# CIawevy/FreeFine

Measured on AMD Instinct MI355X. Metric: edited images/sec/GPU @512px 50-step DDIM, higher is better.
Workload: dtype bf16x3

## Files before the change

freefine_amd/_lib.py:

```python
import ctypes as C
import os

_HERE = os.path.dirname(os.path.abspath(__file__))
LIB_PATH = os.environ.get("FREEFINE_HIP_LIB") or os.path.join(_HERE, "libfreefine_hip.so")

FFN_F32, FFN_BF16, FFN_BF16X3, FFN_FP8 = 0, 1, 2, 3
IG_OUT_SILU, IG_OUT_F32, IG_GEGLU, IG_OUT_TRANSPOSED, IG_OUT_PAIR, IG_OUT_GELU, IG_OUT_RELU, IG_OUT_KV64 = 1, 2, 4, 8, 16, 32, 64, 128
IG_OUT_QGELU = 256
ELT_RELU, ELT_ADD = 0, 1
ATT_MAXP, ATT_MAXB = 4, 16
ATT_HEAD_RULE, ATT_UNIFORM_SEL1, ATT_UNIFORM_SEL0, ATT_CAUSAL = 1, 2, 4, 8
NORM_SILU, NORM_OUT_PAIR = 1, 2


class IgemmDesc(C.Structure):
    _fields_ = [
        ("A", C.c_void_p), ("W", C.c_void_p), ("out", C.c_void_p),
        ("bias", C.c_void_p), ("rowbias", C.c_void_p), ("residual", C.c_void_p),
        ("M", C.c_int), ("N", C.c_int), ("K", C.c_int), ("Kpad", C.c_int),
        ("lda", C.c_int), ("ldo", C.c_int), ("ldr", C.c_int), ("ldrb", C.c_int),
        ("rows_per_batch", C.c_int),
        ("Hin", C.c_int), ("Win", C.c_int), ("Cin", C.c_int), ("Hout", C.c_int), ("Wout", C.c_int),
        ("stride", C.c_int), ("pad", C.c_int), ("upsample", C.c_int),
        ("flags", C.c_int), ("alpha", C.c_float), ("conv", C.c_int),
        ("splitk", C.c_int), ("ws", C.c_void_p), ("ws_bytes", C.c_long),
        ("a_lo", C.c_int), ("x3", C.c_int), ("f8", C.c_int), ("kv64_from", C.c_int),
    ]


class AttnEntry(C.Structure):
    _fields_ = [
        ("q_row", C.c_int), ("kv_row", C.c_int),
        ("w_const", C.c_float), ("w_slope", C.c_float),
        ("wq", C.c_void_p), ("kmask", C.c_void_p), ("qsel", C.c_void_p),
        ("flags", C.c_int), ("hr_row", C.c_int),
    ]


class AttnDesc(C.Structure):
    _fields_ = [
        ("q", C.c_void_p), ("k", C.c_void_p), ("vt", C.c_void_p), ("out", C.c_void_p), ("w_dev", C.c_void_p),
        ("Bo", C.c_int), ("S", C.c_int), ("Sk", C.c_int), ("heads", C.c_int), ("D", C.c_int),
        ("ldq", C.c_int), ("ldk", C.c_int), ("ldvt", C.c_int), ("ldo", C.c_int),
        ("scale", C.c_float), ("npass", C.c_int), ("out_pair", C.c_int), ("kv_pair", C.c_int),
        ("e", AttnEntry * (ATT_MAXP * ATT_MAXB)),
    ]


class CtrlStepDesc(C.Structure):
    _fields_ = [
        ("eps", C.c_void_p), ("x", C.c_void_p), ("noise", C.c_void_p), ("m", C.c_void_p), ("om", C.c_void_p),
        ("x_prev", C.c_void_p), ("pred_x0", C.c_void_p),
        ("c_bt", C.c_float), ("c_at", C.c_float), ("c_ap", C.c_float), ("c_dir", C.c_float),
        ("c_dirm", C.c_float * 8), ("stdv", C.c_float * 8), ("row_masked", C.c_int * 8),
        ("rows", C.c_int), ("CHW", C.c_int), ("HW", C.c_int),
    ]


class SplatXform(C.Structure):
    _fields_ = [("center", C.c_float * 3), ("translate", C.c_float * 3), ("rotate", C.c_float * 9), ("scale", C.c_float * 3),
                ("tan_half_fov", C.c_float)]


class PackDesc(C.Structure):
    _fields_ = [
        ("src", C.c_void_p), ("dst", C.c_void_p), ("src_row", C.c_int * 16),
        ("B", C.c_int), ("Cl", C.c_int), ("CP", C.c_int), ("HW", C.c_int),
    ]


_vp, _i, _f, _l = C.c_void_p, C.c_int, C.c_float, C.c_long
SYMBOLS = {
    "ffn_version": (_i, []),
    "ffn_last_error": (C.c_char_p, []),
    "ffn_device_info": (_i, [_i, C.c_char_p, _i]),
    "ffn_graph_launch": (_i, [_vp, _vp]),
    "ffn_igemm": (_i, [_vp, _i, C.POINTER(IgemmDesc)]),
    "ffn_conv3x3_n4": (_i, [_vp, _i, _vp, _vp, _vp, _vp, _i, _i, _i, _i]),
    "ffn_split_pair": (_i, [_vp, _vp, _vp, _l, _i, _i]),
    "ffn_groupnorm_f8": (_i, [_vp, _vp, _vp, _vp, _vp, _i, _i, _i, _i, _i, _f, _i, _f, _vp, _vp, _vp]),
    "ffn_attn": (_i, [_vp, _i, C.POINTER(AttnDesc)]),
    "ffn_attn_kernel_name": (_i, [_i, C.POINTER(AttnDesc), C.c_char_p, _i]),
    "ffn_igemm_tune": (_i, [_vp, _i, C.POINTER(IgemmDesc)]),
    "ffn_igemm_tune_entry_ints": (_i, []),
    "ffn_igemm_tune_export": (_i, [C.POINTER(C.c_int), _i]),
    "ffn_igemm_tune_import": (_i, [C.POINTER(C.c_int), _i]),
    "ffn_igemm_tune_stamp": (_i, []),
    "ffn_igemm_tune_clear": (_i, []),
    "ffn_igemm_tune_enable": (_i, [_i]),
    "ffn_igemm_num_configs": (_i, []),
    "ffn_igemm_force_config": (_i, [_i]),
    "ffn_igemm_variant": (_i, [C.POINTER(IgemmDesc), C.POINTER(C.c_int), C.POINTER(C.c_int)]),
    "ffn_igemm_kernel_name": (_i, [_i, C.POINTER(IgemmDesc), C.c_char_p, _i]),
    "ffn_attn_presplit": (_i, [_vp, _vp, _vp, _vp, _vp, _i, _i, _i, _i, _i]),
    "ffn_attn_variant": (_i, [_i, _i, C.POINTER(C.c_int), C.POINTER(C.c_int)]),
    "ffn_gn_nchunk": (_i, [_i]),
    "ffn_gn_fused": (_i, [_i, _i, _i, _i]),
    "ffn_gn_stats": (_i, [_vp, _i, _vp, _vp, _vp, _i, _i, _i, _i, _f, _vp, _vp, _vp]),
    "ffn_gn_apply": (_i, [_vp, _i, _vp, _vp, _vp, _vp, _i, _i, _i, _i]),
    "ffn_groupnorm": (_i, [_vp, _i, _vp, _vp, _vp, _vp, _i, _i, _i, _i, _f, _i, _vp, _vp, _vp]),
    "ffn_groupnorm_pair_raw": (_i, [_vp, _vp, _vp, _vp, _vp, _vp, _i, _i, _i, _i, _f, _i, _vp, _vp, _vp]),
    "ffn_layernorm": (_i, [_vp, _i, _vp, _vp, _vp, _vp, _i, _i, _f]),
    "ffn_layernorm_pair": (_i, [_vp, _vp, _vp, _vp, _vp, _i, _i, _f]),
    "ffn_softmax_rows": (_i, [_vp, _i, _vp, _vp, _l, _i, _f]),
    "ffn_cfg_masked": (_i, [_vp, _vp, _vp, _vp, _f, _vp, _l, _i]),
    "ffn_ddim_inv_step": (_i, [_vp, _vp, _vp, _f, _f, _f, _f, _vp, _vp, _l]),
    "ffn_ddim_ctrl_step": (_i, [_vp, C.POINTER(CtrlStepDesc)]),
    "ffn_pack_nchw": (_i, [_vp, _i, C.POINTER(PackDesc)]),
    "ffn_nhwc_to_nchw_f32": (_i, [_vp, _vp, _vp, _i, _i, _i, _i]),
    "ffn_concat": (_i, [_vp, _i, _vp, _vp, _vp, _l, _i, _i]),
    "ffn_timestep_embed": (_i, [_vp, _i, _vp, _vp, _vp, _i, _i, _i]),
    "ffn_transpose": (_i, [_vp, _i, _vp, _vp, _i, _i, _i, _i, _i]),
    "ffn_cast": (_i, [_vp, _i, _i, _vp, _vp, _l]),
    "ffn_eltwise": (_i, [_vp, _i, _i, _vp, _vp, _vp, _l]),
    "ffn_resize_bilinear": (_i, [_vp, _i, _vp, _vp, _i, _i, _i, _i, _i, _i, _i]),
    "ffn_splat_lift": (_i, [_vp, _vp, _vp, _vp, _i, _i, _i, _f, _f]),
    "ffn_splat_project": (_i, [_vp, _vp, _vp, _i, C.POINTER(SplatXform)]),
    "ffn_splat_bin": (_i, [_vp, _i, _vp, _i, _f, _i, _i, _vp, _vp, _vp]),
    "ffn_splat_render": (_i, [_vp, _vp, _vp, _vp, _vp, _f, _i, _i, _i, _vp, _vp, _vp]),
    "ffn_embed_tokens": (_i, [_vp, _i, _vp, _vp, _vp, _vp, _l, _i, _i, _i]),
    "ffn_image_to_nhwc": (_i, [_vp, _i, _vp, _vp, _l, _i]),
    "ffn_nhwc_to_image": (_i, [_vp, _i, _vp, _vp, _i, _i, _i]),
}

_lib = None


class FreeFineHipError(RuntimeError):
    pass


def load():
    global _lib
    if _lib is None:
        if not os.path.exists(LIB_PATH):
            raise FreeFineHipError(
                f"{LIB_PATH} not found: build it with `python -c 'import __graft_entry__ as g; g.build()'` "
                "(hipcc --offload-arch=gfx950). There is no CPU fallback for the product path.")
        import torch
        lib = C.CDLL(LIB_PATH)
        for name, (res, args) in SYMBOLS.items():
            fn = getattr(lib, name)
            fn.restype = res
            fn.argtypes = args
        _lib = lib
    return _lib


def check(rc, what=""):
    if rc != 0:
        msg = load().ffn_last_error()
        raise FreeFineHipError(f"{what} failed rc={rc}: {msg.decode() if msg else ''}")
```

freefine_amd/csrc/capi.hip:

```cpp
#include <hip/hip_runtime.h>
#include <stdarg.h>
#include <stdio.h>
#include <mutex>
#include <unordered_map>
#include <stdlib.h>
#include <string.h>

#include "../../include/freefine_hip.h"
#include "attention.h"
#include "attention_pp.h"
#include "attention_x.h"
#include "attention_x3.h"
#include "attention_x3p.h"
#include "attention_xx3.h"
#include "conv_small.h"
#include "elementwise.h"
#include "igemm.h"
#include "igemm_p8.h"
#include "norms.h"
#include "splat.h"

static thread_local char g_err[512] = "";
static int fail(int code, const char* fmt, ...) {
    va_list ap;
    va_start(ap, fmt);
    vsnprintf(g_err, sizeof(g_err), fmt, ap);
    va_end(ap);
    return code;
}
static int check_launch(const char* what) {
    hipError_t e = hipGetLastError();
    if (e != hipSuccess) return fail(FFN_EHIP, "%s: %s", what, hipGetErrorString(e));
    return FFN_OK;
}
#define LAUNCH(...)                  \
    do {                             \
        (void)hipGetLastError();     \
        hipLaunchKernelGGL(__VA_ARGS__); \
    } while (0)
#define REQUIRE(cond, ...) \
    do {                   \
        if (!(cond)) return fail(FFN_EINVAL, __VA_ARGS__); \
    } while (0)

static inline bool aligned16(const void* p) { return (reinterpret_cast<uintptr_t>(p) & 15) == 0; }
static inline int grid_for(long n, int per_block = 256, int cap = 4096) {
    long g = (n + per_block - 1) / per_block;
    if (g < 1) g = 1;
    if (g > cap) g = cap;
    return (int)g;
}

template <typename K>
static int set_lds(K kernel, int bytes) {
    static std::mutex mu;
    static std::unordered_map<const void*, int> done;
    if (bytes > 48 * 1024) {
        std::lock_guard<std::mutex> lk(mu);
        int& have = done[reinterpret_cast<const void*>(kernel)];
        if (have >= bytes) return FFN_OK;
        have = bytes;
        hipError_t e = hipFuncSetAttribute(reinterpret_cast<const void*>(kernel), hipFuncAttributeMaxDynamicSharedMemorySize, bytes);
        if (e != hipSuccess) return fail(FFN_EHIP, "hipFuncSetAttribute(%d): %s", bytes, hipGetErrorString(e));
    }
    return FFN_OK;
}

extern "C" int ffn_version(void) { return 2; }
extern "C" const char* ffn_last_error(void) { return g_err; }
extern "C" int ffn_device_info(int device, char* name, int name_len) {
    hipDeviceProp_t prop;
    hipError_t e = hipGetDeviceProperties(&prop, device);
    if (e != hipSuccess) return fail(FFN_EHIP, "hipGetDeviceProperties: %s", hipGetErrorString(e));
    if (name && name_len > 0) {
        strncpy(name, prop.gcnArchName, name_len - 1);
        name[name_len - 1] = 0;
    }
    return prop.multiProcessorCount;
}

extern "C" int ffn_graph_launch(void* stream, void* graph_exec) {
    REQUIRE(graph_exec, "graph_launch: null graph");
    hipError_t e = hipGraphLaunch(reinterpret_cast<hipGraphExec_t>(graph_exec), reinterpret_cast<hipStream_t>(stream));
    if (e != hipSuccess) return fail(FFN_EHIP, "hipGraphLaunch: %s", hipGetErrorString(e));
    return FFN_OK;
}

static void igemm_plan_for(int dtype, const ffn_igemm_desc& d, int* bm, int* bn, int* splitk);
static int igemm_stages_env() {
    static const int v = [] {
        const char* e = getenv("FFN_IGEMM_STAGES");
        return e ? atoi(e) : 0;
    }();
    return v;
}
static int device_cus() {
    static const int n = [] {
        int dev = 0, v = 0;
        if (hipGetDevice(&dev) != hipSuccess || hipDeviceGetAttribute(&v, hipDeviceAttributeMultiprocessorCount, dev) != hipSuccess || v <= 0) v = 256;
        return v;
    }();
    return n;
}
static bool persist_enabled() {
    static const bool on = [] { const char* e = getenv("FFN_IGEMM_PERSIST"); return !(e && atoi(e) == 0); }();
    return on;
}
template <typename K>
static int launch_igemm_kernel(K kern, int lds, hipStream_t s, const ffn_igemm_desc& d, int ntiles, int splitk, int threads = 256,
                               bool persist = false) {
    int rc = set_lds(kern, lds);
    if (rc) return rc;
    int gx = ntiles;
    if (persist && persist_enabled()) {
        int per_cu = (160 * 1024) / (lds > 0 ? lds : 1);
        if (per_cu > 2048 / threads) per_cu = 2048 / threads;
        if (per_cu < 1) per_cu = 1;
        const int cap = (device_cus() * per_cu) / (splitk > 0 ? splitk : 1);
        if (gx > cap && cap >= 8) gx = cap;
    }
    LAUNCH(kern, dim3(gx, splitk), dim3(threads), lds, s, d);
// ... 124 lines not shown
    if (d.x3) {
        if (d.x3 != 2 || d.K % 96 != 0 || d.a_lo != 32) return false;
    } else if (d.K % 64 != 0) return false;
    if (nkt < 2 || d.N % bn != 0 || d.M < bm) return false;
    const int osz = d.x3 ? 4 : 2;
    if (splitk > 1) {
        if (!can_split(d) || nkt % splitk != 0 || nkt / splitk < 2 || (long)splitk * d.M * d.N * 4 > d.ws_bytes || (long)splitk * d.M * d.N * 4 >= lim) return false;
    } else {
        const int act_ok = (!d.residual && !d.x3 && !d.f8 && !(d.flags & FFN_IG_GEGLU)) ? (FFN_IG_OUT_GELU | FFN_IG_OUT_RELU) : 0;
        if ((d.alpha != 1.0f && !d.f8) || (d.flags & ~(FFN_IG_GEGLU | act_ok | (d.x3 ? (FFN_IG_OUT_F32 | FFN_IG_OUT_PAIR | FFN_IG_OUT_KV64) : 0)))) return false;
        if (d.f8 && (!d.conv || (d.flags & FFN_IG_GEGLU))) return false;
        if (d.x3 && (d.flags & FFN_IG_GEGLU) && !(d.flags & FFN_IG_OUT_PAIR)) return false;
        if ((d.flags & FFN_IG_OUT_PAIR) && !(d.flags & FFN_IG_GEGLU) && (d.N % 32 != 0 || (d.ldo / 2) % 32 != 0 || (d.flags & FFN_IG_OUT_TRANSPOSED))) return false;
        if ((d.flags & FFN_IG_GEGLU) && bn != 256) return false;
        if (d.rowbias && d.rows_per_batch < 128) return false;
    }
    long a_bytes;
    if (d.conv) {
        const int pix = d.x3 ? d.lda : d.Cin;
        const int cpt = d.x3 ? d.Cin / 32 : d.Cin / 64;
        if (d.Cin % (d.x3 ? 32 : 64) != 0 || d.K != (d.conv == 2 ? 4 : 9) * (d.x3 ? 3 : 1) * d.Cin) return false;
        if (d.x3 && d.lda != 2 * d.Cin) return false;
        if (d.conv == 2 && (d.f8 || d.stride != 1 || d.upsample)) return false;
        if ((long)cpt * 9 * cpt >= 65536) return false;
        a_bytes = (long)(d.M / (d.Hout * d.Wout)) * d.Hin * d.Win * pix * 2;
        if (2 * d.Hin + 2 >= 32768 || 2 * d.Win + 2 >= 32768) return false;
        if (a_bytes + 256l * pix * 2 >= lim) return false;
    } else {
        a_bytes = (long)d.M * d.lda * 2;
        if (a_bytes + 256l * d.lda * 2 >= lim) return false;
    }
    if ((long)d.N * d.Kpad * 2 >= lim || (long)(d.M + 256) * d.ldo * ((d.flags & FFN_IG_OUT_PAIR) ? 2 : osz) >= lim) return false;
    if (d.residual && (long)(d.M + 256) * d.ldr * osz >= lim) return false;
    return true;
}
static int halo_bytes_for(const ffn_igemm_desc& d, int bm) {
    if (!d.conv || d.stride != 1 || d.upsample || d.pad != 1 || d.Hin != d.Hout || d.Win != d.Wout) return 0;
    if (d.Cin % 64 != 0 || d.Cin > 30000 || d.K != 9 * d.Cin || d.M % bm != 0) return 0;
    const int H = d.Hin, W = d.Win;
    int tw, tr;
    if (W <= bm) {
        if (bm % W != 0 || (H * W) % bm != 0) return 0;
        tw = W; tr = bm / W;
    } else {
        if (W % bm != 0) return 0;
        tw = bm; tr = 1;
    }
    const int nq = ((tr + 2) * (tw + 2) + 7) / 8;
    if (nq > 4 * 16) return 0;
    return nq * 8 * 128;
}
static bool x3_cfg(int cfg) { return cfg == CFG_64x64 || cfg == CFG_128x64 || cfg == CFG_128x128_8 || is_pp_cfg(cfg); }
template <int AMODE, bool X3 = false, bool F8 = false>
static int launch_bf16_cfg(hipStream_t s, const ffn_igemm_desc& d, IgChoice ch) {
    const IgCfgInfo& c = kCfg[ch.cfg];
    if ((X3 || F8) && !x3_cfg(ch.cfg)) return fail(FFN_EINVAL, "igemm: configuration %d is not built for split-bf16 / fp8 problems", ch.cfg);
    const int ntiles = ((d.M + c.bm - 1) / c.bm) * ((d.N + c.bn - 1) / c.bn);
    const int lds = 2 * (c.bm + c.bn) * 128, threads = 64 * c.nwm * c.nwn;
    int rc = FFN_OK;
    const bool fastk = (d.conv ? d.Cin % 64 == 0 : d.K % 64 == 0) && (long)d.K * 2 + 256 <= (long)sizeof(g_zero_page);
#define FFN_CFG_CASE(ID, BM_, BN_, WM_, WN_)                                                                                               \
    case ID:                                                                                                                        \
        if constexpr (X3) {                                                                                                         \
            if constexpr (ID == CFG_64x64 || ID == CFG_128x64 || ID == CFG_128x128_8)                                               \
                rc = launch_igemm_kernel(igemm_glds_kernel<bf16, BM_, BN_, AMODE, true, 2, WM_, WN_, false, true>, lds, s, d, ntiles, ch.splitk, threads, true); \
        } else if constexpr (F8) {                                                                                                  \
            if constexpr (AMODE == AMODE_CONV3 && (ID == CFG_64x64 || ID == CFG_128x64 || ID == CFG_128x128_8))                     \
                rc = launch_igemm_kernel(igemm_glds_kernel<bf16, BM_, BN_, AMODE, true, 2, WM_, WN_, false, false, true>, lds, s, d, ntiles, ch.splitk, threads, true); \
        } else {                                                                                                                    \
            rc = fastk ? launch_igemm_kernel(igemm_glds_kernel<bf16, BM_, BN_, AMODE, true, 2, WM_, WN_, true>, lds, s, d, ntiles, ch.splitk, threads, true)  \
                       : launch_igemm_kernel(igemm_glds_kernel<bf16, BM_, BN_, AMODE, true, 2, WM_, WN_, false>, lds, s, d, ntiles, ch.splitk, threads, true); \
        }                                                                                                                           \
        break;
    switch (ch.cfg) {
        FFN_CFG_CASE(CFG_64x64, 64, 64, 2, 2)
        FFN_CFG_CASE(CFG_128x64, 128, 64, 4, 2)
        FFN_CFG_CASE(CFG_128x128_8, 128, 128, 2, 4)
        FFN_CFG_CASE(CFG_128x128_16, 128, 128, 4, 4)
        FFN_CFG_CASE(CFG_256x128, 256, 128, 4, 4)
        FFN_CFG_CASE(CFG_256x256, 256, 256, 4, 4)
        FFN_CFG_CASE(CFG_128x320, 128, 320, 4, 4)
        FFN_CFG_CASE(CFG_128x160, 128, 160, 4, 2)
        FFN_CFG_CASE(CFG_192x320, 192, 320, 3, 4)
        case CFG_PP_256x320:
        case CFG_PP_256x256:
        case CFG_PP_192x320:
        case CFG_PP_192x256:
        case CFG_PP_256x128: {
            if (!pp_ok(d, c.bm, c.bn, ch.splitk)) return fail(FFN_EINVAL, "igemm: ping-pong kernel not applicable");
            const int pplds = 2 * (c.bm + c.bn) * 128 + 12288;
            const int nt = ((d.M + c.bm - 1) / c.bm) * (d.N / c.bn) * ch.splitk;
            const int grid = nt < device_cus() ? nt : device_cus();
            (void)hipGetLastError();
#define FFN_PP_LAUNCH(BM_, BN_, RES_, GEGLU_)                                              \
    do {                                                                                   \
        auto kern = igemm_pp_kernel<BM_, BN_, AMODE, RES_, (GEGLU_) && !F8, false, false, X3, F8>;      \
        if ((rc = set_lds(kern, pplds))) return rc;                                        \
        hipLaunchKernelGGL(kern, dim3(grid), dim3(512), pplds, s, d, 1);                   \
    } while (0)
#define FFN_PP_TILE(BM_)                                                                   \
    do {                                                                                   \
        if (c.bn == 320) {                                                                 \
            if (d.residual) FFN_PP_LAUNCH(BM_, 320, true, false);                          \
            else FFN_PP_LAUNCH(BM_, 320, false, false);                                    \
        } else {                                                                           \
            if constexpr (AMODE == AMODE_DENSE) {                                          \
                if (d.flags & FFN_IG_GEGLU) FFN_PP_LAUNCH(BM_, 256, false, true);          \
                else if (d.residual) FFN_PP_LAUNCH(BM_, 256, true, false);                 \
                else FFN_PP_LAUNCH(BM_, 256, false, false);                                \
            } else {                                                                       \
                if (d.residual) FFN_PP_LAUNCH(BM_, 256, true, false);                      \
                else FFN_PP_LAUNCH(BM_, 256, false, false);                                \
            }                                                                              \
        }                                                                                  \
    } while (0)
#define FFN_PP_SPLIT(BM_, BN_)                                                             \
    do {                                                                                   \
        auto kern = igemm_pp_kernel<BM_, BN_, AMODE, false, false, true, false, X3, F8>;   \
        if ((rc = set_lds(kern, pplds))) return rc;                                        \
        hipLaunchKernelGGL(kern, dim3(grid), dim3(512), pplds, s, d, ch.splitk);           \
    } while (0)
            if (c.bn == 128) {
                if constexpr (X3 && AMODE == AMODE_CONV3) {
                    if (d.residual) FFN_PP_LAUNCH(256, 128, true, false);
                    else FFN_PP_LAUNCH(256, 128, false, false);
                    return check_launch("igemm(ping-pong, 256 x 128)");
                } else {
                    return fail(FFN_EINVAL, "igemm: the 256 x 128 ping-pong tile is built for split-bf16 3x3 convolutions");
                }
            }
            if (ch.splitk > 1) {
                if (c.bm == 256 && c.bn == 320) FFN_PP_SPLIT(256, 320);
                else if (c.bm == 256) FFN_PP_SPLIT(256, 256);
                else if (c.bn == 320) FFN_PP_SPLIT(192, 320);
                else FFN_PP_SPLIT(192, 256);
                if ((rc = check_launch("igemm(ping-pong, split-K)"))) return rc;
                const long nq = (long)d.M * (d.N / 4);
                if constexpr (X3) LAUNCH(igemm_splitk_reduce_kernel<float>, dim3(grid_for(nq)), dim3(256), 0, s, d, ch.splitk);
                else LAUNCH(igemm_splitk_reduce_kernel<bf16>, dim3(grid_for(nq)), dim3(256), 0, s, d, ch.splitk);
                return check_launch("igemm_splitk_reduce");
            }
            if (c.bm == 256) FFN_PP_TILE(256);
            else FFN_PP_TILE(192);
#undef FFN_PP_SPLIT
#undef FFN_PP_TILE
#undef FFN_PP_LAUNCH
            return check_launch("igemm(ping-pong)");
        }
// ... 8 lines not shown
                const int nt = (d.M / c.bm) * ((d.N + c.bn - 1) / c.bn);
                (void)hipGetLastError();
                if (ch.cfg == CFG_H_128x320) {
                    auto kern = igemm_halo_kernel<bf16, 128, 320, 4, 4>;
                    if ((rc = set_lds(kern, hlds))) return rc;
                    hipLaunchKernelGGL(kern, dim3(nt), dim3(threads), hlds, s, d, hb);
                } else if (ch.cfg == CFG_H_256x128) {
                    auto kern = igemm_halo_kernel<bf16, 256, 128, 4, 4>;
                    if ((rc = set_lds(kern, hlds))) return rc;
                    hipLaunchKernelGGL(kern, dim3(nt), dim3(threads), hlds, s, d, hb);
                } else if (ch.cfg == CFG_H_256x256) {
                    auto kern = igemm_halo_kernel<bf16, 256, 256, 4, 4>;
                    if ((rc = set_lds(kern, hlds))) return rc;
                    hipLaunchKernelGGL(kern, dim3(nt), dim3(threads), hlds, s, d, hb);
                } else {
                    auto kern = igemm_halo_kernel<bf16, 128, 128, 4, 4>;
                    if ((rc = set_lds(kern, hlds))) return rc;
                    hipLaunchKernelGGL(kern, dim3(nt), dim3(threads), hlds, s, d, hb);
                }
                return check_launch("igemm(halo)");
            } else {
                return fail(FFN_EINVAL, "igemm: halo configurations are for 3x3 convolutions");
            }
        default: return fail(FFN_EINVAL, "igemm: bad configuration %d", ch.cfg);
    }
#undef FFN_CFG_CASE
    if (rc || ch.splitk == 1) return rc;
    const long nq = (long)d.M * (d.N / 4);
    if constexpr (X3) LAUNCH(igemm_splitk_reduce_kernel<float>, dim3(grid_for(nq)), dim3(256), 0, s, d, ch.splitk);
    else LAUNCH(igemm_splitk_reduce_kernel<bf16>, dim3(grid_for(nq)), dim3(256), 0, s, d, ch.splitk);
    return check_launch("igemm_splitk_reduce");
}

struct TuneKey {
    int M, N, K, conv, Cin, Hin, Win, stride, upsample, flags, lda, splitk, ptrs, wslabs, rpb, alpha1, ldo, pad, Hout, Wout, Kpad, ldr, dtype;
    bool operator==(const TuneKey& o) const { return memcmp(this, &o, sizeof(TuneKey)) == 0; }
};
struct TuneKeyHash {
    size_t operator()(const TuneKey& k) const {
        const int* p = reinterpret_cast<const int*>(&k);
        size_t h = 1469598103934665603ull;
        for (size_t i = 0; i < sizeof(TuneKey) / sizeof(int); ++i) h = (h ^ (size_t)(unsigned)p[i]) * 1099511628211ull;
        return h;
    }
};
static TuneKey tune_key(const ffn_igemm_desc& d) {
    TuneKey k;
    memset(&k, 0, sizeof(k));
    k.M = d.M; k.N = d.N; k.K = d.K; k.conv = d.conv; k.flags = d.flags; k.lda = d.lda; k.splitk = d.splitk;
    if (d.conv) { k.Cin = d.Cin; k.Hin = d.Hin; k.Win = d.Win; k.stride = d.stride; k.upsample = d.upsample; k.pad = d.pad; k.Hout = d.Hout; k.Wout = d.Wout; }
    k.Kpad = d.Kpad;
    k.ldr = d.residual ? d.ldr : 0;
    k.dtype = d.x3 ? (FFN_BF16X3 | (d.x3 << 8)) : (d.f8 ? FFN_FP8 : FFN_BF16);
    k.ptrs = (d.bias ? 1 : 0) | (d.rowbias ? 2 : 0) | (d.residual ? 4 : 0) | (d.ws && d.ws_bytes > 0 ? 8 : 0);
    const long per = (long)d.M * d.N * 4;
    k.wslabs = d.ws ? (int)(d.ws_bytes / per > 1024 ? 1024 : d.ws_bytes / per) : 0;
    k.rpb = d.rows_per_batch;
    k.alpha1 = d.alpha == 1.0f;
    k.ldo = d.ldo;
    return k;
}
static std::mutex g_tune_mu;
static std::unordered_map<TuneKey, TunedEntry, TuneKeyHash> g_tuned;
static int g_tune_runtime = 1;
static bool tune_enabled() {
    static const bool on = [] { const char* e = getenv("FFN_IGEMM_TUNE"); return !(e && atoi(e) == 0); }();
    return on && g_tune_runtime;
}
static IgChoice heuristic_choice(const ffn_igemm_desc& d) {
    if (d.conv == 2) {
        for (int bn : {320, 256})
            for (int h : {256, 192})
                if (d.N % bn == 0 && pp_ok(d, h, bn)) return IgChoice{bn == 320 ? (h == 256 ? CFG_PP_256x320 : CFG_PP_192x320) : (h == 256 ? CFG_PP_256x256 : CFG_PP_192x256), 1};
    }
    if (d.splitk <= 1) {
        for (int bn : {320, 256}) {
            if (d.N % bn != 0) continue;
            long best = -1;
            int bh = 0;
            for (int h : {256, 192}) {
                if (!pp_ok(d, h, bn)) continue;
                const long tiles = (long)((d.M + h - 1) / h) * (d.N / bn);
                if (tiles * 4 < (long)device_cus() * 3) continue;
                const long cost = ((tiles + device_cus() - 1) / device_cus()) * h;
                if (best < 0 || cost < best) { best = cost; bh = h; }
            }
            if (best >= 0) return IgChoice{bn == 320 ? (bh == 256 ? CFG_PP_256x320 : CFG_PP_192x320) : (bh == 256 ? CFG_PP_256x256 : CFG_PP_192x256), 1};
        }
        if (d.N % 128 == 0 && pp_ok(d, 256, 128) && (long)((d.M + 255) / 256) * (d.N / 128) * 4 >= (long)device_cus() * 3) return IgChoice{CFG_PP_256x128, 1};
    }
    int bm, bn, sk, ns, nw;
    igemm_plan_for(FFN_BF16, d, &bm, &bn, &sk);
    igemm_exec_cfg(FFN_BF16, d, bm, bn, sk, &ns, &nw);
    int cfg = CFG_64x64;
    if (bm == 128 && bn == 64) cfg = CFG_128x64;
    if (bm == 128 && bn == 128) cfg = (nw == 16 && !d.x3 && !d.f8) ? CFG_128x128_16 : CFG_128x128_8;
    return IgChoice{cfg, sk};
}
static int candidates_for(const ffn_igemm_desc& d, IgChoice* out, int cap) {
    int n = 0;
    const IgChoice h = heuristic_choice(d);
    out[n++] = h;
    const int nk = (d.K + 63) / 64;
    const long per = (long)d.M * d.N * 4;
    for (int cfg = 0; cfg < CFG_COUNT; ++cfg) {
        const IgCfgInfo& c = kCfg[cfg];
        if ((d.x3 || d.f8) && !x3_cfg(cfg)) continue;
// ... 151 lines not shown
}
extern "C" int ffn_igemm_tune_import(const int* buf, int n_entries) {
    REQUIRE(buf || n_entries == 0, "igemm_tune_import: null buffer");
    std::lock_guard<std::mutex> lk(g_tune_mu);
    int n = 0;
    for (int i = 0; i < n_entries; ++i) {
        const int* e = buf + (long)i * kTuneEntryInts;
        if (e[0] != kTuneStamp) continue;
        TuneKey k;
        memcpy(&k, e + 1, sizeof(TuneKey));
        const IgChoice ch{e[kTuneEntryInts - 2], e[kTuneEntryInts - 1]};
        if (ch.cfg < 0 || ch.cfg >= CFG_COUNT || ch.splitk < 1) continue;
        g_tuned[k] = TunedEntry{ch, false};
        ++n;
    }
    return n;
}
static bool tuned_lookup(const ffn_igemm_desc& d, IgChoice* ch) {
    std::lock_guard<std::mutex> lk(g_tune_mu);
    auto it = g_tuned.find(tune_key(d));
    if (it == g_tuned.end()) return false;
    *ch = it->second.ch;
    return true;
}

static bool pp_trans_tile(const ffn_igemm_desc& d, int* bm, int* bn);
static ffn_igemm_desc x3_view(const ffn_igemm_desc& d);
static ffn_igemm_desc f8_view(const ffn_igemm_desc& d);
extern "C" int ffn_igemm_kernel_name(int dtype, const ffn_igemm_desc* d0, char* buf, int len) {
    REQUIRE(d0 && buf && len > 0, "igemm_kernel_name: null argument");
    int bm, bn, sk, ns, nw;
    IgChoice ch;
    const bool x3 = dtype == FFN_BF16X3, f8 = dtype == FFN_FP8;
    const ffn_igemm_desc dd = x3 ? x3_view(*d0) : (f8 ? f8_view(*d0) : *d0);
    const ffn_igemm_desc* d = &dd;
    if (x3 && (d->flags & FFN_IG_OUT_TRANSPOSED)) {
        if (!d->conv && pp_trans_tile(*d, &bm, &bn)) {
            snprintf(buf, len, "void igemm_pp_kernel<%d, %d, 0, false, false, false, true, true, false>(ffn_igemm_desc, int)", bm, bn);
            return FFN_OK;
        }
        igemm_plan_for(FFN_BF16, *d, &bm, &bn, &sk);
        snprintf(buf, len, "void igemm_glds_kernel<bf16, %d, %d, 0, false, 2, 2, 2, false, true, false>(ffn_igemm_desc)", bm, bn);
        return FFN_OK;
    }
    if ((dtype == FFN_BF16 || x3 || f8) && !(d->flags & FFN_IG_OUT_TRANSPOSED)) {
        if (!tuned_lookup(*d, &ch)) ch = heuristic_choice(*d);
        const IgCfgInfo& c = kCfg[ch.cfg];
        if (is_halo_cfg(ch.cfg)) {
            snprintf(buf, len, "void igemm_halo_kernel<bf16, %d, %d, %d, %d>(ffn_igemm_desc, int)", c.bm, c.bn, c.nwm, c.nwn);
            return FFN_OK;
        }
        if (is_pp_cfg(ch.cfg)) {
            const bool split = ch.splitk > 1;
            snprintf(buf, len, "void igemm_pp_kernel<%d, %d, %d, %s, %s, %s, false, %s, %s>(ffn_igemm_desc, int)", c.bm, c.bn, d->conv ? 1 : 0,
                     (!split && d->residual) ? "true" : "false", (!split && (d->flags & FFN_IG_GEGLU)) ? "true" : "false", split ? "true" : "false",
                     x3 ? "true" : "false", f8 ? "true" : "false");
            return FFN_OK;
        }
        const bool fastk = !x3 && !f8 && (d->conv ? d->Cin % 64 == 0 : d->K % 64 == 0) && (long)d->K * 2 + 256 <= (long)sizeof(g_zero_page);
        snprintf(buf, len, "void igemm_glds_kernel<bf16, %d, %d, %d, true, 2, %d, %d, %s, %s, %s>(ffn_igemm_desc)", c.bm, c.bn, d->conv ? 1 : 0, c.nwm, c.nwn,
                 fastk ? "true" : "false", x3 ? "true" : "false", f8 ? "true" : "false");
        return FFN_OK;
    }
    if (dtype == FFN_BF16 && (d->flags & FFN_IG_OUT_TRANSPOSED) && !d->conv && pp_trans_tile(*d, &bm, &bn)) {
        snprintf(buf, len, "void igemm_pp_kernel<%d, %d, 0, false, false, false, true, false, false>(ffn_igemm_desc, int)", bm, bn);
        return FFN_OK;
    }
    igemm_plan_for(dtype, *d, &bm, &bn, &sk);
    igemm_exec_cfg(dtype, *d, bm, bn, sk, &ns, &nw);
    const char* t = dtype == FFN_F32 ? "float" : "bf16";
    const char* swap = (d->flags & FFN_IG_OUT_TRANSPOSED) ? "false" : "true";
    if (ns == 1) snprintf(buf, len, "void igemm_kernel<%s, %d, %d, %d, %s>(ffn_igemm_desc)", t, bm, bn, d->conv ? 1 : 0, swap);
    else {
        const int nwm = nw == 16 ? 4 : (nw == 8 ? (bn == 64 ? 4 : 2) : 2), nwn = nw / nwm;
        snprintf(buf, len, "void igemm_glds_kernel<%s, %d, %d, %d, %s, %d, %d, %d, false, false, false>(ffn_igemm_desc)", t, bm, bn, d->conv ? 1 : 0, swap, ns, nwm, nwn);
    }
    return FFN_OK;
}
static bool pp_trans_tile(const ffn_igemm_desc& d, int* bm, int* bn) {
    static const bool on = [] { const char* e = getenv("FFN_IGEMM_PP_TRANS"); return !(e && atoi(e) == 0); }();
    if (!on) return false;
    const long lim = (1l << 31) - 4096;
    *bn = d.N % 320 == 0 ? 320 : (d.N % 256 == 0 ? 256 : 0);
    if (!*bn || d.alpha != 1.0f || d.rows_per_batch % 16 != 0 || d.M % 4 != 0) return false;
    if (d.x3) {
        if (d.x3 != 2 || d.K % 96 != 0 || d.K < 192 || d.a_lo != 32) return false;
    } else if (d.K % 64 != 0 || d.K < 128) return false;
    if ((long)(d.M + 256) * d.lda * 2 >= lim || (long)d.N * d.Kpad * 2 >= lim) return false;
    if ((long)((d.M + d.rows_per_batch - 1) / d.rows_per_batch) * d.N * d.ldo * (d.x3 ? 4 : 2) >= lim) return false;
    long best = -1;
    for (int h : {256, 192}) {
        if (d.M < h) continue;
        const long tiles = (long)((d.M + h - 1) / h) * (d.N / *bn);
        const long cost = ((tiles + device_cus() - 1) / device_cus()) * h;
        if (best < 0 || cost < best) { best = cost; *bm = h; }
    }
    return best >= 0;
}
template <bool X3 = false>
static int launch_pp_trans(hipStream_t s, const ffn_igemm_desc& d, int bm, int bn) {
    const int pplds = 2 * (bm + bn) * 128 + 12288;
    const int nt = ((d.M + bm - 1) / bm) * (d.N / bn);
    const int grid = nt < device_cus() ? nt : device_cus();
    int rc = FFN_OK;
    (void)hipGetLastError();
#define FFN_PP_TR(BM_, BN_)                                                                         \
// ... 129 lines not shown
    REQUIRE(d->K % epc == 0, "igemm: K=%d must be a multiple of %d", d->K, epc);
    REQUIRE(d->rows_per_batch > 0, "igemm: rows_per_batch must be > 0");
    if (d->conv) {
        REQUIRE(d->Cin % epc == 0, "igemm: Cin=%d must be a multiple of %d", d->Cin, epc);
        if (d->conv == 2) {
            REQUIRE((dtype == FFN_BF16 || dtype == FFN_BF16X3) && d->K == 4 * d->Cin && d->stride == 1 && d->upsample == 0 && d->pad >= 0 && d->pad <= 3 && d->splitk <= 1,
                    "igemm: 2x2 convolution needs FFN_BF16 / FFN_BF16X3, K = 4*Cin, stride 1, no upsample, pad in 0..3, no forced split");
            const ffn_igemm_desc v = dtype == FFN_BF16X3 ? x3_view(*d) : *d;
            bool any = false;
            for (int bn : {320, 256})
                for (int h : {256, 192}) any |= d->N % bn == 0 && pp_ok(v, h, bn);
            REQUIRE(any, "igemm: 2x2 convolution M=%d N=%d Cin=%d fits no ping-pong tile (Cin %% 64 (split-bf16: 32), N %% 256 / 320, M >= 192)", d->M, d->N, d->Cin);
        } else {
            REQUIRE(d->conv == 1, "igemm: conv=%d", d->conv);
            REQUIRE(d->K == 9 * d->Cin, "igemm: conv K=%d != 9*Cin=%d", d->K, 9 * d->Cin);
        }
        REQUIRE(d->stride == 1 || d->stride == 2, "igemm: stride %d", d->stride);
        REQUIRE(d->upsample == 0 || d->upsample == 1, "igemm: upsample %d", d->upsample);
        REQUIRE(d->M % (d->Hout * d->Wout) == 0, "igemm: M=%d not a multiple of Hout*Wout", d->M);
    } else {
        REQUIRE(d->lda % epc == 0, "igemm: lda=%d must be a multiple of %d", d->lda, epc);
    }
    if (d->flags & FFN_IG_OUT_KV64) {
        REQUIRE(dtype == FFN_BF16X3 && !d->conv && !d->residual && !d->rowbias && d->splitk <= 1 &&
                    !(d->flags & (FFN_IG_GEGLU | FFN_IG_OUT_PAIR | FFN_IG_OUT_SILU | FFN_IG_OUT_GELU | FFN_IG_OUT_RELU | FFN_IG_OUT_QGELU)),
                "igemm: FFN_IG_OUT_KV64 needs FFN_BF16X3, dense A, the plain epilogue and no forced split-K");
        if (d->flags & FFN_IG_OUT_TRANSPOSED) REQUIRE(d->rows_per_batch % 64 == 0 && d->M % d->rows_per_batch == 0 && d->ldo >= d->rows_per_batch && d->ldo % 64 == 0,
                                                      "igemm: KV64 transposed output needs rows_per_batch %% 64 == 0, whole batches, ldo %% 64 == 0 (rows_per_batch=%d, ldo=%d)", d->rows_per_batch, d->ldo);
        else REQUIRE(d->kv64_from >= 0 && d->kv64_from < d->N && d->kv64_from % 64 == 0 && d->N % 64 == 0 && d->ldo % 4 == 0,
                     "igemm: KV64 output needs kv64_from and N %% 64 == 0 (kv64_from=%d, N=%d)", d->kv64_from, d->N);
    }
    if (d->flags & FFN_IG_OUT_TRANSPOSED) {
        REQUIRE(d->ldo % 4 == 0, "igemm: transposed ldo=%d must be a multiple of 4", d->ldo);
        REQUIRE(!(d->flags & (FFN_IG_GEGLU | FFN_IG_OUT_F32 | FFN_IG_OUT_SILU | FFN_IG_OUT_GELU | FFN_IG_OUT_RELU | FFN_IG_OUT_QGELU)) && !d->residual && !d->rowbias,
                "igemm: transposed output supports bias only");
    } else {
        REQUIRE(d->N % 4 == 0 && d->ldo % 4 == 0, "igemm: N=%d and ldo=%d must be multiples of 4", d->N, d->ldo);
        if (d->residual) REQUIRE(d->ldr % 4 == 0, "igemm: ldr=%d must be a multiple of 4", d->ldr);
        if (d->flags & FFN_IG_OUT_PAIR) {
            const int nout = (d->flags & FFN_IG_GEGLU) ? d->N / 2 : d->N;
            REQUIRE(dtype == FFN_BF16X3 && d->ldo % 16 == 0 && d->ldo / 2 >= nout, "igemm: pair output needs FFN_BF16X3, ldo %% 16 == 0, ldo/2 >= columns");
            REQUIRE(d->residual != d->out, "igemm: pair output cannot overwrite its fp32 residual");
            REQUIRE((d->ldo / 2) % 32 != 0 || nout % 32 == 0 || nout == d->ldo / 2, "igemm: blocked pair output (ldo/2 %% 32 == 0) needs whole 32-column blocks");
            REQUIRE(nout == d->ldo / 2 || (d->ldo / 2) % 32 == 0, "igemm: pair output into a wider row needs ldo/2 %% 32 == 0 (ldo=%d, columns=%d)", d->ldo, nout);
        }
        if (d->flags & FFN_IG_GEGLU) {
            REQUIRE(d->N % 64 == 0, "igemm: GEGLU needs N %% 64 == 0 (N=%d)", d->N);
            REQUIRE(!d->residual && !d->rowbias && !(d->flags & (FFN_IG_OUT_F32 | FFN_IG_OUT_SILU | FFN_IG_OUT_GELU | FFN_IG_OUT_RELU | FFN_IG_OUT_QGELU)), "igemm: GEGLU epilogue is exclusive");
        }
    }
    {
        const int act = d->flags & (FFN_IG_OUT_SILU | FFN_IG_OUT_GELU | FFN_IG_OUT_RELU | FFN_IG_OUT_QGELU);
        REQUIRE((act & (act - 1)) == 0, "igemm: SILU / GELU / QGELU / RELU are mutually exclusive");
    }
    if (d->ws) REQUIRE(aligned16(d->ws) && d->ws_bytes >= 0, "igemm: workspace must be 16-byte aligned");
    REQUIRE(d->splitk >= 0, "igemm: splitk must be >= 0");
    hipStream_t s = reinterpret_cast<hipStream_t>(stream);
    if (dtype == FFN_BF16X3) return dispatch_igemm_x3(s, x3_view(*d));
    ffn_igemm_desc plain = *d;
    plain.x3 = plain.f8 = 0;
    return dtype == FFN_F32 ? dispatch_igemm<float>(s, plain) : dispatch_igemm<bf16>(s, plain);
}

extern "C" int ffn_igemm_tune(void* stream, int dtype, const ffn_igemm_desc* d) { return ffn_igemm(stream, dtype, d); }

struct AttnTile { int dp, qf, kt, occ; };
static const AttnTile kAttnTileF32[] = {{48, 2, 64, 1}, {64, 2, 64, 1}, {80, 2, 64, 1}, {160, 1, 32, 1}};
static const AttnTile kAttnTileBf16[] = {{64, 2, 64, 2}, {96, 2, 64, 1}, {160, 1, 64, 1}};
static AttnTile attn_tile(bool f32, int D) {
    const AttnTile* t = f32 ? kAttnTileF32 : kAttnTileBf16;
    const int n = f32 ? 4 : 3;
    int i = 0;
    while (i + 1 < n && D > t[i].dp) ++i;
    return t[i];
}
extern "C" int ffn_attn_variant(int dtype, int D, int* dp, int* qf) {
    REQUIRE(dp && qf, "attn_variant: null argument");
    const AttnTile t = attn_tile(dtype == FFN_F32, D);
    *dp = t.dp;
    *qf = t.qf;
    return FFN_OK;
}
static constexpr int attn_kernel_lds(int esz, int dp, int qf, int kt) {
    return 2 * (kt * (dp * esz == 128 ? 128 : dp * esz + 16) + dp * ((dp * esz == 128 && kt * esz == 128) ? 128 : kt * esz + 16)) + 4 * (dp / 16) * qf * 64 * 16 + 2 * kt;
}
static_assert(attn_kernel_lds(4, 160, 1, 32) <= 160 * 1024 && attn_kernel_lds(2, 160, 1, 64) <= 160 * 1024, "attention tile does not fit the 160 KiB LDS");

typedef void (*attn_x3w_t)(ffn_attn_desc);
extern "C" __attribute__((visibility("hidden"))) attn_x3w_t fx3w_kernel(int masks);
extern "C" __attribute__((visibility("hidden"))) int fx3w_lds_bytes(void);
extern "C" __attribute__((visibility("hidden"))) attn_x3w_t fcausal_kernel(int dtype);
extern "C" __attribute__((visibility("hidden"))) void fembed_launch(hipStream_t s, int bf16_out, const int* ids, const float* table, const float* pos, void* out,
                                                                    long M, int S, int C, int V);

enum AttnKind { ATT_KERNEL, ATT_PP, ATT_X, ATT_X_MP, ATT_X3, ATT_X3P, ATT_X3W, ATT_XX3, ATT_CAUSAL_K };
struct AttnPlan {
    AttnKind kind;
    bool f32;
    bool masks;
    AttnTile tile;
    int nkf, nw;
    int lds;
    dim3 grid, block;
};
static int attn_plan(int dtype, const ffn_attn_desc& d, AttnPlan* p) {
    bool masks = false, uniform = false, xok = true, multi = d.npass != 1;
// ... 238 lines not shown
extern "C" int ffn_gn_fused(int B, int HW, int C, int G) {
    const long slice = (long)HW * (C / (G > 0 ? G : 1));
    if (slice > 131072) return 0;
    if (HW <= 64) return 1;
    if (HW <= 256) return B <= 32 ? 1 : 0;
    return (HW <= 1024 && (long)B * HW * C <= 3000000l) ? 1 : 0;
}
extern "C" int ffn_groupnorm(void* stream, int dtype, const void* x, void* y, const float* gamma, const float* beta, int B, int HW, int C,
                             int G, float eps, int silu, float* partial_ws, float* scale, float* shift) {
    REQUIRE(dtype == FFN_F32 || dtype == FFN_BF16, "groupnorm: bad dtype");
    REQUIRE(x && y && gamma && beta && C % G == 0 && (C / G) % 2 == 0, "groupnorm: bad arguments (C=%d, G=%d)", C, G);
    hipStream_t s = reinterpret_cast<hipStream_t>(stream);
    const long slice = (long)HW * (C / G);
    (void)slice;
    const bool fused = ffn_gn_fused(B, HW, C, G) != 0;
    const bool pair = silu & FFN_NORM_OUT_PAIR;
    REQUIRE(!pair || (dtype == FFN_F32 && C % 4 == 0), "groupnorm: pair output needs fp32 input and C %% 4 == 0");
    silu &= FFN_NORM_SILU;
    if (fused && pair) {
        dim3 grid(G, B);
        if (silu) LAUNCH((gn_fused_kernel<float, true, true>), grid, dim3(1024), 0, s, (const float*)x, (float*)y, gamma, beta, HW, C, G, eps);
        else LAUNCH((gn_fused_kernel<float, false, true>), grid, dim3(1024), 0, s, (const float*)x, (float*)y, gamma, beta, HW, C, G, eps);
        return check_launch("gn_fused(pair)");
    }
    if (fused) {
        dim3 grid(G, B);
        if (dtype == FFN_F32) {
            if (silu) LAUNCH((gn_fused_kernel<float, true>), grid, dim3(1024), 0, s, (const float*)x, (float*)y, gamma, beta, HW, C, G, eps);
            else LAUNCH((gn_fused_kernel<float, false>), grid, dim3(1024), 0, s, (const float*)x, (float*)y, gamma, beta, HW, C, G, eps);
        } else {
            if (silu) LAUNCH((gn_fused_kernel<bf16, true>), grid, dim3(1024), 0, s, (const bf16*)x, (bf16*)y, gamma, beta, HW, C, G, eps);
            else LAUNCH((gn_fused_kernel<bf16, false>), grid, dim3(1024), 0, s, (const bf16*)x, (bf16*)y, gamma, beta, HW, C, G, eps);
        }
        return check_launch("gn_fused");
    }
    REQUIRE(partial_ws && scale && shift, "groupnorm: workspace required beyond 32x32 positions");
    int rc = ffn_gn_stats(stream, dtype, x, gamma, beta, B, HW, C, G, eps, partial_ws, scale, shift);
    if (rc) return rc;
    return ffn_gn_apply(stream, dtype, x, y, scale, shift, B, HW, C, silu | (pair ? FFN_NORM_OUT_PAIR : 0));
}
extern "C" int ffn_groupnorm_pair_raw(void* stream, const void* x, void* y, void* yraw, const float* gamma, const float* beta, int B, int HW, int C, int G,
                                      float eps, int silu, float* partial_ws, float* scale, float* shift) {
    REQUIRE(x && y && yraw && gamma && beta && partial_ws && scale && shift, "groupnorm_pair_raw: null pointer (the workspace is always needed)");
    REQUIRE(C % 8 == 0 && C % G == 0 && (C / G) % 2 == 0 && aligned16(x) && aligned16(y) && aligned16(yraw), "groupnorm_pair_raw: bad arguments (C=%d, G=%d)", C, G);
    REQUIRE(y != yraw && yraw != x && y != x, "groupnorm_pair_raw: x, y and yraw must be distinct buffers");
    int rc = ffn_gn_stats(stream, FFN_F32, x, gamma, beta, B, HW, C, G, eps, partial_ws, scale, shift);
    if (rc) return rc;
    hipStream_t s = reinterpret_cast<hipStream_t>(stream);
    const long n8 = (long)B * HW * (C / 8);
    if (silu & FFN_NORM_SILU) LAUNCH((gn_apply_pair8_kernel<true, true>), dim3(grid_for(n8)), dim3(256), 0, s, (const float*)x, (bf16*)y, scale, shift, n8, HW, C, (bf16*)yraw);
    else LAUNCH((gn_apply_pair8_kernel<false, true>), dim3(grid_for(n8)), dim3(256), 0, s, (const float*)x, (bf16*)y, scale, shift, n8, HW, C, (bf16*)yraw);
    return check_launch("gn_apply(pair + raw pair)");
}
extern "C" int ffn_groupnorm_f8(void* stream, const void* x, void* y, const float* gamma, const float* beta, int B, int HW, int C, int Cp, int G,
                                float eps, int silu, float qscale, float* partial_ws, float* scale, float* shift) {
    REQUIRE(x && y && gamma && beta && partial_ws && scale && shift, "groupnorm_f8: null pointer (the workspace is always needed)");
    REQUIRE(C % 16 == 0 && C % G == 0 && Cp >= C && Cp % 16 == 0 && aligned16(x) && aligned16(y) && qscale > 0.f, "groupnorm_f8: bad arguments (C=%d, Cp=%d)", C, Cp);
    int rc = ffn_gn_stats(stream, FFN_BF16, x, gamma, beta, B, HW, C, G, eps, partial_ws, scale, shift);
    if (rc) return rc;
    hipStream_t s = reinterpret_cast<hipStream_t>(stream);
    const long nch = (long)B * HW * (Cp / 16);
    if (silu & FFN_NORM_SILU) LAUNCH(gn_apply_f8_kernel<true>, dim3(grid_for(nch)), dim3(256), 0, s, (const bf16*)x, (uint8_t*)y, scale, shift, nch, HW, C, Cp, qscale);
    else LAUNCH(gn_apply_f8_kernel<false>, dim3(grid_for(nch)), dim3(256), 0, s, (const bf16*)x, (uint8_t*)y, scale, shift, nch, HW, C, Cp, qscale);
    return check_launch("gn_apply_f8");
}
extern "C" int ffn_gn_stats(void* stream, int dtype, const void* x, const float* gamma, const float* beta, int B, int HW, int C,
                            int G, float eps, float* partial_ws, float* scale, float* shift) {
    REQUIRE(dtype == FFN_F32 || dtype == FFN_BF16, "gn_stats: bad dtype");
    const int epc = dtype == FFN_F32 ? 4 : 8;
    REQUIRE(x && gamma && beta && partial_ws && scale && shift, "gn_stats: null pointer");
    REQUIRE(C % epc == 0 && C % G == 0 && aligned16(x), "gn_stats: C=%d must be a multiple of %d and of G=%d", C, epc, G);
    hipStream_t s = reinterpret_cast<hipStream_t>(stream);
    const int nchunk = ffn_gn_nchunk(HW);
    const int ppc = (HW + nchunk - 1) / nchunk;
    const int epc_ = dtype == FFN_F32 ? 4 : 8;
    const int cols_ = C / epc_ < 256 ? C / epc_ : 256;
    const int lds = (256 / cols_ > 0 ? 256 / cols_ : 1) * cols_ * 2 * epc_ * (int)sizeof(float);
    if (dtype == FFN_F32)
        LAUNCH(gn_partial_kernel<float>, dim3(nchunk, B), dim3(256), lds, s, (const float*)x, partial_ws, HW, C, ppc);
    else
        LAUNCH(gn_partial_kernel<bf16>, dim3(nchunk, B), dim3(256), lds, s, (const bf16*)x, partial_ws, HW, C, ppc);
    if (int rc = check_launch("gn_partial")) return rc;
    LAUNCH(gn_finalize_kernel, dim3(G, B), dim3(64), 0, s, partial_ws, gamma, beta, scale, shift, HW, C, G, nchunk, eps);
    return check_launch("gn_stats");
}
extern "C" int ffn_gn_apply(void* stream, int dtype, const void* x, void* y, const float* scale, const float* shift, int B, int HW,
                            int C, int silu) {
    REQUIRE(dtype == FFN_F32 || dtype == FFN_BF16, "gn_apply: bad dtype");
    const int epc = dtype == FFN_F32 ? 4 : 8;
    REQUIRE(x && y && scale && shift && C % epc == 0 && aligned16(x) && aligned16(y), "gn_apply: bad arguments");
    hipStream_t s = reinterpret_cast<hipStream_t>(stream);
    const long nch = (long)B * HW * (C / epc);
    const int grid = grid_for(nch);
    if (silu & FFN_NORM_OUT_PAIR) {
        REQUIRE(dtype == FFN_F32, "gn_apply: pair output needs fp32 input");
        static const int wide = [] { const char* e = getenv("FFN_PAIR8"); return e ? atoi(e) : 1; }();
        if (wide && C % 8 == 0) {
            const long n8 = (long)B * HW * (C / 8);
            if (silu & FFN_NORM_SILU) LAUNCH(gn_apply_pair8_kernel<true>, dim3(grid_for(n8)), dim3(256), 0, s, (const float*)x, (bf16*)y, scale, shift, n8, HW, C);
            else LAUNCH(gn_apply_pair8_kernel<false>, dim3(grid_for(n8)), dim3(256), 0, s, (const float*)x, (bf16*)y, scale, shift, n8, HW, C);
            return check_launch("gn_apply(pair, 8 wide)");
        }
        if (silu & FFN_NORM_SILU) LAUNCH((gn_apply_kernel<float, true, true>), dim3(grid), dim3(256), 0, s, (const float*)x, (float*)y, scale, shift, nch, HW, C);
        else LAUNCH((gn_apply_kernel<float, false, true>), dim3(grid), dim3(256), 0, s, (const float*)x, (float*)y, scale, shift, nch, HW, C);
        return check_launch("gn_apply(pair)");
    }
// ... 176 lines not shown
```

freefine_amd/csrc/igemm_p8.h:

```cpp
#pragma once
#include <type_traits>
#include "igemm.h"

#ifndef PP_PRIO
#define PP_PRIO 1
#endif
#ifndef PP_ABL
#define PP_ABL 0
#endif
#ifndef PP_TAPINNER
#define PP_TAPINNER 1
#endif
#ifdef PP_STAMP
__device__ unsigned long long pp_stamp_out[8 * 64];
#define PP_STAMP_AT(k_) do { if (blockIdx.x == 7 && s >= 24 && s < 28) { const unsigned long long t_ = __builtin_amdgcn_s_memtime(); \
    if (lane == 0) *reinterpret_cast<unsigned long long*>(smem + CV + 12288 + (wave * 64 + (s - 24) * 16 + (k_)) * 8) = t_; } } while (0)
#else
#define PP_STAMP_AT(k_) do {} while (0)
#endif
#ifdef PP_NBE
#define X3_NBE(FN_, NA_) (PP_NBE)
#else
#define X3_NBE(FN_, NA_) ((FN_) + 2 - ((FN_) + (NA_) + 1) / 2)
#endif
template <int N>
__device__ __forceinline__ void pp_wait_vmcnt() {
    if (PP_ABL != 2) asm volatile("s_waitcnt vmcnt(%0)" ::"n"(N) : "memory");
}
__device__ __forceinline__ void pp_barrier() {
    asm volatile("" ::: "memory");
    __builtin_amdgcn_s_barrier();
    asm volatile("" ::: "memory");
}

#ifdef PP_TRACE
__device__ unsigned long long pp_trace[256 * 64];
#endif
template <int BM, int BN, int AMODE, bool RES, bool GEGLU, bool SPLIT = false, bool TRANS = false, bool X3 = false, bool F8 = false>
__global__ __launch_bounds__(512) void igemm_pp_kernel(const IgemmParams p, int splitk = 1) {
    typedef bf16 T;
    constexpr int HM = BM / 2;
    constexpr int FM = HM / 16;
    constexpr int FH = FM / 2;
    constexpr int NA = BM / 64;
    constexpr int FN = BN / 64;
    constexpr int WN = BN / 4;
    constexpr int ABYTES = BM * 128, BBYTES = BN * 128, BUF = ABYTES + BBYTES;
    constexpr int CV = 2 * BUF;
    constexpr int NB1 = (FN + 1) / 2;
    constexpr int NST = (SPLIT || TRANS || X3) ? FH * FN : (GEGLU ? FH * FN / 2 : FH * ((FN + 1) / 2));
    constexpr int OSZ = (X3 && !GEGLU) ? 4 : 2;
    constexpr int OOB = (int)0x80000000;
    static_assert((BM == 256 || BM == 192) && (BN == 256 || BN == 320 || (BN == 128 && BM == 256 && X3 && AMODE == AMODE_CONV3 && !GEGLU && !SPLIT && !TRANS)), "tiles built for this kernel");
    static_assert(!GEGLU || FN % 2 == 0, "GEGLU pairs hidden / gate column blocks inside a wave");

    extern __shared__ __attribute__((aligned(16))) char smem[];

    const int tid = threadIdx.x;
    const int lane = tid & 63, wave = __builtin_amdgcn_readfirstlane(tid >> 6);
    const int wr = wave >> 2, wc = wave & 3;
    const int l15 = lane & 15, g = lane >> 4;
    const int lrow = lane >> 3, csrc = (lane & 7) ^ lrow;

    static_assert(!SPLIT || (!RES && !GEGLU), "split-K slabs carry raw accumulators: the epilogue runs in the reduce kernel");
    static_assert(!TRANS || (!RES && !GEGLU && !SPLIT && AMODE == AMODE_DENSE), "transposed output: dense A, bias only");
    static_assert(!F8 || (!X3 && !TRANS && !GEGLU), "fp8 operands: plain / residual / split-K epilogues");
    const int ntn = p.N / BN;
    const int ntm = (p.M + BM - 1) / BM;
    const int nsl = SPLIT ? splitk : 1;
    const int ntiles = ntm * ntn * nsl;
    const int G = gridDim.x;
    const int nk = (X3 ? p.K / 96 : p.K / 64) / nsl;
    const int first = __builtin_amdgcn_readfirstlane(xcd_remap(blockIdx.x, G));
    const int my_tiles = (ntiles - first + G - 1) / G;
    const int S = my_tiles * nk;

    const int PIX = X3 ? p.lda * 2 : p.Cin * 2;
    const long a_bytes = AMODE == AMODE_DENSE ? (long)p.M * p.lda * 2 : (long)(p.M / (p.Hout * p.Wout)) * p.Hin * p.Win * PIX;
    const __amdgpu_buffer_rsrc_t rsrcA = __builtin_amdgcn_make_buffer_rsrc(const_cast<void*>(p.A), 0, (int)a_bytes, 0x00020000);
    const __amdgpu_buffer_rsrc_t rsrcB = __builtin_amdgcn_make_buffer_rsrc(const_cast<void*>(p.W), 0, (int)((long)p.N * p.Kpad * 2), 0x00020000);
    const __amdgpu_buffer_rsrc_t rsrcBias = __builtin_amdgcn_make_buffer_rsrc(const_cast<float*>(p.bias), 0, p.bias ? p.N * 4 : 0, 0x00020000);
    const int nbatch = (p.M + p.rows_per_batch - 1) / p.rows_per_batch;
    const __amdgpu_buffer_rsrc_t rsrcRb =
        __builtin_amdgcn_make_buffer_rsrc(const_cast<float*>(p.rowbias), 0, p.rowbias ? ((nbatch - 1) * p.ldrb + p.N) * 4 : 0, 0x00020000);
    const long o_bytes = TRANS ? (long)((p.M + p.rows_per_batch - 1) / p.rows_per_batch) * p.N * p.ldo * OSZ : (long)p.M * p.ldo * OSZ;
    const __amdgpu_buffer_rsrc_t rsrcO = __builtin_amdgcn_make_buffer_rsrc(p.out, 0, (int)o_bytes, 0x00020000);
    const __amdgpu_buffer_rsrc_t rsrcR = __builtin_amdgcn_make_buffer_rsrc(const_cast<void*>(p.residual), 0, RES ? (int)((long)p.M * p.ldr * OSZ) : 0, 0x00020000);

    int l_tile = first, l_kt = 0;
    int l_k0 = 0;
    int a_off[NA];
    int a_yx[NA];
    int b_voff;
    const int b_step = 64 * p.Kpad * 2;
    int apiece[NA];
    if constexpr (BM == 256) {
        apiece[0] = wave; apiece[1] = 16 + wave; apiece[2] = 8 + wave; apiece[3] = 24 + wave;
    } else {
        apiece[0] = wave < 6 ? wave : wave + 6;
        apiece[1] = wave < 4 ? 14 + wave : 2 + wave;
        apiece[2] = wave < 2 ? 10 + wave : 16 + wave;
    }
    const int cpt = AMODE == AMODE_DENSE ? 1 : (X3 ? p.Cin / 32 : p.Cin / 64);
    const int cpt_rcp = (65536 + cpt - 1) / cpt;
    constexpr bool TAPIN = X3 && AMODE != AMODE_DENSE && PP_TAPINNER;
    const int ntap = p.conv == 2 ? 4 : 9;
    auto kt_split = [&](int kt, int& tap, int& c) {
        if (TAPIN) {
            c = p.conv == 2 ? (kt >> 2) : ((kt * 7282) >> 16);
            tap = kt - c * ntap;
        } else {
            tap = (kt * cpt_rcp) >> 16;
            c = kt - tap * cpt;
        }
    };
    int ka = 0, tap_ky = 0, tap_kx = 0, tap_off = 0;
    auto k_position = [&]() {
        const int kt = l_k0 + l_kt;
        if (AMODE == AMODE_DENSE) {
            ka = kt * 128;
        } else {
            int tap, c;
            kt_split(kt, tap, c);
            ka = c * 128;
            tap_ky = p.conv == 2 ? (tap >> 1) : ((tap * 21846) >> 16);
            tap_kx = tap - (p.conv == 2 ? 2 : 3) * tap_ky;
            tap_off = (tap_ky * p.Win + tap_kx) * PIX;
        }
    };
    auto w_position = [&]() {
        const int kt = l_k0 + l_kt;
        if (!TAPIN) return kt * 128;
        int tap, c;
        kt_split(kt, tap, c);
        return (tap * cpt + c) * 128;
    };
    auto prep = [&](int wtile) {
        const int tile = wtile / nsl;
        l_k0 = (wtile - tile * nsl) * nk;
        const int mt = (tile / ntn) * BM, nt = (tile % ntn) * BN;
// ... 205 lines not shown
#pragma unroll
                for (int j = 0; j < FN; ++j) {
                    u32x4 w = __builtin_bit_cast(u32x4, acc[i][j]);
                    w[0] = perm(w[0]); w[1] = perm(w[1]); w[2] = perm(w[2]); w[3] = perm(w[3]);
                    __builtin_amdgcn_raw_buffer_store_b128(w, rsrcWs, vo, ((slice * p.M + m0 + i * 16) * p.N + n0 + j * 16) * 4, 0);
                }
            }
            return;
        }
        if constexpr (TRANS) {
            const int voff = (pr * p.ldo + 4 * pg) * OSZ;
#pragma unroll
            for (int i = i0; i < i0 + FH; ++i) {
                const int mb = m0 + i * 16;
                const int bb = mb / p.rows_per_batch, sb = mb - bb * p.rows_per_batch;
#pragma unroll
                for (int j = 0; j < FN; ++j) {
                    if constexpr (X3) {
                        u32x4 w4 = __builtin_bit_cast(u32x4, acc[i][j]);
                        w4[0] = perm(w4[0]); w4[1] = perm(w4[1]); w4[2] = perm(w4[2]); w4[3] = perm(w4[3]);
                        if (p.flags & FFN_IG_OUT_KV64) {
                            const float f0 = __uint_as_float(w4[0]), f1 = __uint_as_float(w4[1]), f2 = __uint_as_float(w4[2]), f3 = __uint_as_float(w4[3]);
                            u32x2 hi, lo;
                            hi[0] = pack_bf16x2(f0, f1);
                            hi[1] = pack_bf16x2(f2, f3);
                            lo[0] = pack_bf16x2(f0 - __uint_as_float(hi[0] << 16), f1 - __uint_as_float(hi[0] & 0xffff0000u));
                            lo[1] = pack_bf16x2(f2 - __uint_as_float(hi[1] << 16), f3 - __uint_as_float(hi[1] & 0xffff0000u));
                            const int vo2 = mb + 4 * pg < p.M ? (pr * p.ldo * 4 + 4 * pg * 2) : OOB;
                            const int so2 = (bb * p.N + n0 + j * 16) * p.ldo * 4 + (sb >> 6) * 256 + (sb & 63) * 2;
                            __builtin_amdgcn_raw_buffer_store_b64(hi, rsrcO, vo2, so2, 0);
                            __builtin_amdgcn_raw_buffer_store_b64(lo, rsrcO, vo2, so2 + 128, 0);
                            continue;
                        }
                        __builtin_amdgcn_raw_buffer_store_b128(w4, rsrcO, mb + 4 * pg < p.M ? voff : OOB, ((bb * p.N + n0 + j * 16) * p.ldo + sb) * 4, 0);
                        continue;
                    }
                    u32x2 w;
                    w[0] = perm(pack_bf16x2(acc[i][j][0], acc[i][j][1]));
                    w[1] = perm(pack_bf16x2(acc[i][j][2], acc[i][j][3]));
                    __builtin_amdgcn_raw_buffer_store_b64(w, rsrcO, mb + 4 * pg < p.M ? voff : OOB, ((bb * p.N + n0 + j * 16) * p.ldo + sb) * 2, 0);
                }
            }
            return;
        }
        if (PP_ABL == 4) {
#pragma unroll
            for (int i = i0; i < i0 + FH; ++i)
#pragma unroll
                for (int j = 0; j < FN; ++j) asm volatile("" ::"v"(acc[i][j]));
            return;
        }
        if constexpr (X3) {
            const int voff = (pr * p.ldo + 4 * pg) * 4;
#pragma unroll
            for (int i = i0; i < i0 + FH; ++i) {
                const int vo = m0 + i * 16 + pr < p.M ? voff : OOB;
                if constexpr (GEGLU) {
                    const int vo2 = m0 + i * 16 + pr < p.M ? (pr * p.ldo + 4 * pg) * 2 : OOB;
#pragma unroll
                    for (int j = 0; j + 1 < FN; j += 2) {
                        const f32x2_t g01 = (PP_ABL == 3 ? f32x2_t{acc[i][j + 1][0], acc[i][j + 1][1]} : gelu_erf26_2(f32x2_t{acc[i][j + 1][0], acc[i][j + 1][1]})) * f32x2_t{acc[i][j][0], acc[i][j][1]};
                        const f32x2_t g23 = (PP_ABL == 3 ? f32x2_t{acc[i][j + 1][2], acc[i][j + 1][3]} : gelu_erf26_2(f32x2_t{acc[i][j + 1][2], acc[i][j + 1][3]})) * f32x2_t{acc[i][j][2], acc[i][j][3]};
                        const float v[4] = {g01[0], g01[1], g23[0], g23[1]};
                        u32x2 hi, lo;
                        hi[0] = pack_bf16x2(v[0], v[1]);
                        hi[1] = pack_bf16x2(v[2], v[3]);
                        lo[0] = pack_bf16x2(v[0] - __uint_as_float(hi[0] << 16), v[1] - __uint_as_float(hi[0] & 0xffff0000u));
                        lo[1] = pack_bf16x2(v[2] - __uint_as_float(hi[1] << 16), v[3] - __uint_as_float(hi[1] & 0xffff0000u));
                        hi[0] = perm(hi[0]); hi[1] = perm(hi[1]); lo[0] = perm(lo[0]); lo[1] = perm(lo[1]);
                        const int so = ((m0 + i * 16) * p.ldo + n0 + (j / 2) * 16) * 2;
                        __builtin_amdgcn_raw_buffer_store_b64(hi, rsrcO, vo2, so, 0);
                        __builtin_amdgcn_raw_buffer_store_b64(lo, rsrcO, vo2, so + 64, 0);
                    }
                } else {
#pragma unroll
                    for (int j = 0; j < FN; ++j) {
                        u32x4 w = __builtin_bit_cast(u32x4, acc[i][j]);
                        w[0] = perm(w[0]); w[1] = perm(w[1]); w[2] = perm(w[2]); w[3] = perm(w[3]);
                        const int nf = n0 + j * 16;
                        if (p.flags & FFN_IG_OUT_PAIR) {
                            const float f0 = __uint_as_float(w[0]), f1 = __uint_as_float(w[1]), f2 = __uint_as_float(w[2]), f3 = __uint_as_float(w[3]);
                            u32x2 hi, lo;
                            hi[0] = pack_bf16x2(f0, f1);
                            hi[1] = pack_bf16x2(f2, f3);
                            lo[0] = pack_bf16x2(f0 - __uint_as_float(hi[0] << 16), f1 - __uint_as_float(hi[0] & 0xffff0000u));
                            lo[1] = pack_bf16x2(f2 - __uint_as_float(hi[1] << 16), f3 - __uint_as_float(hi[1] & 0xffff0000u));
                            const int vo2 = m0 + i * 16 + pr < p.M ? (pr * p.ldo + 4 * pg) * 2 : OOB;
                            const int so2 = (m0 + i * 16) * p.ldo * 2 + (nf >> 5) * 128 + (nf & 31) * 2;
                            __builtin_amdgcn_raw_buffer_store_b64(hi, rsrcO, vo2, so2, 0);
                            __builtin_amdgcn_raw_buffer_store_b64(lo, rsrcO, vo2, so2 + 64, 0);
                            continue;
                        }
                        if ((p.flags & FFN_IG_OUT_KV64) && nf >= p.kv64_from) {
                            const float f0 = __uint_as_float(w[0]), f1 = __uint_as_float(w[1]), f2 = __uint_as_float(w[2]), f3 = __uint_as_float(w[3]);
                            u32x2 hi, lo;
                            hi[0] = pack_bf16x2(f0, f1);
                            hi[1] = pack_bf16x2(f2, f3);
                            lo[0] = pack_bf16x2(f0 - __uint_as_float(hi[0] << 16), f1 - __uint_as_float(hi[0] & 0xffff0000u));
                            lo[1] = pack_bf16x2(f2 - __uint_as_float(hi[1] << 16), f3 - __uint_as_float(hi[1] & 0xffff0000u));
                            const int crel = nf - p.kv64_from;
                            const int vo2 = m0 + i * 16 + pr < p.M ? (pr * p.ldo * 4 + 4 * pg * 2) : OOB;
                            const int so2 = ((m0 + i * 16) * p.ldo + p.kv64_from) * 4 + (crel >> 6) * 256 + (crel & 63) * 2;
                            __builtin_amdgcn_raw_buffer_store_b64(hi, rsrcO, vo2, so2, 0);
                            __builtin_amdgcn_raw_buffer_store_b64(lo, rsrcO, vo2, so2 + 128, 0);
                            continue;
                        }
                        __builtin_amdgcn_raw_buffer_store_b128(w, rsrcO, vo, ((m0 + i * 16) * p.ldo + n0 + j * 16) * 4, 0);
                    }
                }
            }
            return;
        }
        if constexpr (GEGLU) {
            const int voff = (l15 * p.ldo + 4 * g) * 2;
#pragma unroll
            for (int i = i0; i < i0 + FH; ++i)
#pragma unroll
                for (int j = 0; j + 1 < FN; j += 2) {
                    const f32x2_t g01 = (PP_ABL == 3 ? f32x2_t{acc[i][j + 1][0], acc[i][j + 1][1]} : gelu_erf_fast2(f32x2_t{acc[i][j + 1][0], acc[i][j + 1][1]})) * f32x2_t{acc[i][j][0], acc[i][j][1]};
                    const f32x2_t g23 = (PP_ABL == 3 ? f32x2_t{acc[i][j + 1][2], acc[i][j + 1][3]} : gelu_erf_fast2(f32x2_t{acc[i][j + 1][2], acc[i][j + 1][3]})) * f32x2_t{acc[i][j][2], acc[i][j][3]};
                    u32x2 w;
                    w[0] = pack_bf16x2(g01[0], g01[1]);
                    w[1] = pack_bf16x2(g23[0], g23[1]);
                    __builtin_amdgcn_raw_buffer_store_b64(w, rsrcO, voff, ((m0 + i * 16) * p.ldo + n0 / 2 + (j / 2) * 16) * 2, 0);
                }
            return;
        }
        if constexpr (F8) {
#pragma unroll
            for (int i = i0; i < i0 + FH; ++i)
#pragma unroll
                for (int j = 0; j < FN; ++j) {
                    acc[i][j] *= p.alpha;
                    asm volatile("" : "+v"(acc[i][j]));
                }
            __builtin_amdgcn_sched_barrier(0);
        }
        if constexpr (!RES && !F8) {
            if (p.flags & (FFN_IG_OUT_GELU | FFN_IG_OUT_RELU)) {
                const bool gelu = p.flags & FFN_IG_OUT_GELU;
#pragma unroll
                for (int i = i0; i < i0 + FH; ++i)
#pragma unroll
                    for (int j = 0; j < FN; ++j) {
#pragma unroll
                        for (int r = 0; r < 4; ++r) acc[i][j][r] = gelu ? gelu_erf_fast(acc[i][j][r]) : fmaxf(acc[i][j][r], 0.f);
                        asm volatile("" : "+v"(acc[i][j]));
                    }
                __builtin_amdgcn_sched_barrier(0);
            }
        }
        constexpr int NOF = FN;
        const int voff8 = (pr * p.ldo + 4 * pg) * 2;
        const int voff16 = pr * p.ldo * 2 + pg * 16;
        const int paddr16 = (pr + 16 * (((pg & 1) << 1) | (pg >> 1))) * 4;
        const int ncol0 = n0;
#pragma unroll
        for (int i = i0; i < i0 + FH; ++i) {
            auto outfrag = [&](int jo, unsigned& w0, unsigned& w1) {
                w0 = pack_bf16x2(acc[i][jo][0], acc[i][jo][1]);
                w1 = pack_bf16x2(acc[i][jo][2], acc[i][jo][3]);
// ... 67 lines not shown
#pragma unroll
            for (int i = 0; i < FH; ++i)
#pragma unroll
                for (int j = 0; j < FN; ++j) mm(fb[j], fa[i], acc[i0 + i][j]);
            if constexpr (KEEPA) {
#pragma unroll
                for (int i = 0; i < FH; ++i)
#pragma unroll
                    for (int j = 0; j < FN; ++j) mm(fb[j], fal[i], acc[i0 + i][j]);
#pragma unroll
                for (int i = 0; i < FH; ++i)
#pragma unroll
                    for (int j = 0; j < FN; ++j) mm(fbl[j], fa[i], acc[i0 + i][j]);
            } else {
#pragma unroll
                for (int i = 0; i < FH; ++i) {
#pragma unroll
                    for (int j = 0; j < FN; ++j) mm(fbl[j], fa[i], acc[i0 + i][j]);
                    fa[i] = *reinterpret_cast<const u32x4*>(smem + b_ * BUF + a_rd1 + (i0 + i) * 2048);
                }
#pragma unroll
                for (int i = 0; i < FH; ++i)
#pragma unroll
                    for (int j = 0; j < FN; ++j) mm(fb[j], fa[i], acc[i0 + i][j]);
            }
            if (PP_PRIO == 1) __builtin_amdgcn_s_setprio(0);
        };
        auto read_a_set = [&](int b_, int i0) {
            read_a(b_, a_rd0, i0);
            if constexpr (KEEPA) {
#pragma unroll
                for (int i = 0; i < FH; ++i) fal[i] = *reinterpret_cast<const u32x4*>(smem + b_ * BUF + a_rd1 + (i0 + i) * 2048);
            }
        };
        auto read_low_set = [&](int b_) {
            read_a_set(b_, 0);
            read_b(b_, b_rd0);
#pragma unroll
            for (int j = 0; j < FN; ++j) fbl[j] = *reinterpret_cast<const u32x4*>(smem + b_ * BUF + b_rd1 + j * 2048);
        };
        for (int s = 0; s < S; ++s) {
            const bool more = s + 1 < S;
            const int nb = buf ^ 1;

            __builtin_amdgcn_sched_barrier(0);
            PP_STAMP_AT(0);
            if (p_tile >= 0) {
                store_rows(p_tile, I4_t{});
#pragma unroll
                for (int i = NBE; i < FN; ++i) issue_b(i, nb);
                k_position();
                issue_a(0, nb);
                issue_a(1, nb);
                pp_wait_vmcnt<FN + NAL + 2 * NST>();
                init_rows(c_tile, I0_t{});
                __builtin_amdgcn_sched_barrier(0);
                read_low_set(buf);
            } else {
                read_low_set(buf);
                PP_STAMP_AT(8);
                if (more) {
#pragma unroll
                    for (int i = NBE; i < FN; ++i) issue_b(i, nb);
                    k_position();
                    issue_a(0, nb);
                    issue_a(1, nb);
                    PP_STAMP_AT(9);
                    pp_wait_vmcnt<FN + NAL>();
                } else {
                    pp_wait_vmcnt<0>();
                }
                PP_STAMP_AT(10);
            }
            if (NBE > 0) asm volatile("s_waitcnt lgkmcnt(0)" ::: "memory");
            __builtin_amdgcn_sched_barrier(0);
            PP_STAMP_AT(1);
            pp_barrier();
            PP_STAMP_AT(2);
            mfma3(I0_t{}, buf);
            __builtin_amdgcn_sched_barrier(0);
            PP_STAMP_AT(3);
            pp_barrier();
            PP_STAMP_AT(4);

            if (more) {
#pragma unroll
                for (int i = 2; i < NA; ++i) issue_a(i, nb);
                advance();
                const bool more2 = s + 2 < S;
                if (more2) {
#pragma unroll
                    for (int i = 0; i < NBE; ++i) issue_b(i, buf);
                }
                if (more2) {
                    if (switched) pp_wait_vmcnt<NAH + NBE + (SPLIT ? 0 : 6)>();
                    else pp_wait_vmcnt<NAH + NBE>();
                } else {
                    pp_wait_vmcnt<NAH>();
                }
            }
            if (p_tile >= 0) {
                init_rows(c_tile, I4_t{});
                p_tile = -1;
            }
            if (c_kt == nk - 1) store_rows(c_tile, I0_t{});
            __builtin_amdgcn_sched_barrier(0);
            read_a_set(buf, FH);
// ... 65 lines not shown
            read_a(ra, a_rd1, 0);
            read_b(rb, b_rd1);
            if (needA) {
                k_position();
                issue_a(0, la);
                issue_a(1, la);
            }
            __builtin_amdgcn_sched_barrier(0);
            pp_barrier();
            mfma_rows(I0_t{});
            __builtin_amdgcn_sched_barrier(0);
            pp_barrier();

            read_a(ra, a_rd1, FH);
            if (more) {
                if (needA) {
#pragma unroll
                    for (int i = 2; i < NA; ++i) issue_a(i, la);
                }
                advance();
                if (PP_ABL == 9 && c_kt < 2) {}
                else if (switched) pp_wait_vmcnt<NA - 2 + (SPLIT ? 0 : 6)>();
                else pp_wait_vmcnt<NA - 2>();
            }
            if (c_kt == nk - 1) {
#ifdef PP_TRACE
                if (tid == 0) pp_trace[blockIdx.x * 64 + 2 * ((c_tile - first) / G & 31)] = __builtin_amdgcn_s_memrealtime();
#endif
                store_rows(c_tile, I0_t{});
#ifdef PP_TRACE
                if (tid == 0) pp_trace[blockIdx.x * 64 + 2 * ((c_tile - first) / G & 31) + 1] = __builtin_amdgcn_s_memrealtime();
#endif
            }
            __builtin_amdgcn_sched_barrier(0);
            pp_barrier();
            mfma_rows(I4_t{});
            __builtin_amdgcn_sched_barrier(0);
            pp_barrier();

            buf = nb;
            if (++c_kt == nk) {
                p_tile = c_tile;
                c_kt = 0;
                c_tile += G;
            }
        }
    }
    if (p_tile >= 0) store_rows(p_tile, I4_t{});
    if (wr == 0) pp_barrier();
#ifdef PP_STAMP
    if (blockIdx.x == 7) pp_stamp_out[tid] = *reinterpret_cast<const unsigned long long*>(smem + CV + 12288 + tid * 8);
#endif
}
```

freefine_amd/csrc/norms.h:

```cpp
#pragma once
#include "common.h"

__device__ __forceinline__ void store_pair4(bf16* yp, long row, int C, int c, const float* f) {
    u32x2 hi, lo;
    hi[0] = pack_bf16x2(f[0], f[1]);
    hi[1] = pack_bf16x2(f[2], f[3]);
    lo[0] = pack_bf16x2(f[0] - __uint_as_float(hi[0] << 16), f[1] - __uint_as_float(hi[0] & 0xffff0000u));
    lo[1] = pack_bf16x2(f[2] - __uint_as_float(hi[1] << 16), f[3] - __uint_as_float(hi[1] & 0xffff0000u));
    bf16* q = yp + row * 2 * C + pair_pos(c, C);
    *reinterpret_cast<u32x2*>(q) = hi;
    *reinterpret_cast<u32x2*>(q + pair_lo(C)) = lo;
}

template <typename T>
__global__ __launch_bounds__(256) void gn_partial_kernel(const T* __restrict__ x, float* __restrict__ partial, int HW,
                                                         int C, int pix_per_chunk) {
    constexpr int EPC = DT<T>::EPC;
    extern __shared__ __attribute__((aligned(16))) char smem[];
    float* ls = reinterpret_cast<float*>(smem);
    const int b = blockIdx.y, chunk = blockIdx.x, nchunk = gridDim.x;
    const int cch = C / EPC;
    const int tid = threadIdx.x;
    const int p0 = chunk * pix_per_chunk;
    const int p1 = min(HW, p0 + pix_per_chunk);
// ... 29 lines not shown
                float f[EPC];
                DT<T>::unpack(v, f);
#pragma unroll
                for (int e = 0; e < EPC; ++e) {
                    s[e] += f[e];
                    ss[e] += f[e] * f[e];
                }
            }
#pragma unroll
            for (int e = 0; e < EPC; ++e) {
                ls[(pp * cols + (cc - cbase)) * 2 * EPC + 2 * e] = s[e];
                ls[(pp * cols + (cc - cbase)) * 2 * EPC + 2 * e + 1] = ss[e];
            }
        }
        __syncthreads();
        for (int i = tid; i < cols * 2 * EPC; i += 256) {
            float acc = 0.f;
            for (int r = 0; r < ppi; ++r) acc += ls[r * cols * 2 * EPC + i];
            dst[cbase * 2 * EPC + i] = acc;
        }
        __syncthreads();
    }
}

__global__ __launch_bounds__(64) void gn_finalize_kernel(const float* __restrict__ partial, const float* __restrict__ gamma,
                                                         const float* __restrict__ beta, float* __restrict__ scale,
                                                         float* __restrict__ shift, int HW, int C, int G, int nchunk,
                                                         float eps) {
    const int g = blockIdx.x, b = blockIdx.y, lane = threadIdx.x;
    const int cg = C / G;
    double s = 0.0, ss = 0.0;
    for (int i = lane; i < nchunk * cg; i += 64) {
        const int ch = i / cg, c = g * cg + (i - ch * cg);
        const float* src = partial + (((long)b * nchunk + ch) * C + c) * 2;
        s += (double)src[0];
        ss += (double)src[1];
    }
    for (int off = 32; off > 0; off >>= 1) {
        s += __shfl_xor(s, off);
        ss += __shfl_xor(ss, off);
    }
    const double n = (double)HW * cg;
    const double mean = s / n;
    double var = ss / n - mean * mean;
    if (var < 0.0) var = 0.0;
    const float rstd = (float)(1.0 / sqrt(var + (double)eps));
    const float fmean = (float)mean;
    for (int i = lane; i < cg; i += 64) {
        const int c = g * cg + i;
        const float sc = rstd * gamma[c];
        scale[(long)b * C + c] = sc;
        shift[(long)b * C + c] = beta[c] - fmean * sc;
    }
}

template <typename T, bool SILU, bool PAIR = false>
__global__ __launch_bounds__(256) void gn_apply_kernel(const T* __restrict__ x, T* __restrict__ y,
                                                       const float* __restrict__ scale, const float* __restrict__ shift,
                                                       long nchunks_total, int HW, int C) {
    constexpr int EPC = DT<T>::EPC;
    const int cch = C / EPC;
    for (long i = (long)blockIdx.x * 256 + threadIdx.x; i < nchunks_total; i += (long)gridDim.x * 256) {
        const long pix = i / cch;
        const int cc = (int)(i - pix * cch);
        const int b = (int)(pix / HW);
        const u32x4 v = *reinterpret_cast<const u32x4*>(x + i * EPC);
        float f[EPC];
        DT<T>::unpack(v, f);
        const float* sc = scale + (long)b * C + cc * EPC;
        const float* sh = shift + (long)b * C + cc * EPC;
#pragma unroll
        for (int e = 0; e < EPC; ++e) {
            float t = f[e] * sc[e] + sh[e];
            if (SILU) t = silu_for<T>(t);
            f[e] = t;
        }
        if constexpr (PAIR) store_pair4(reinterpret_cast<bf16*>(y), pix, C, cc * EPC, f);
        else *reinterpret_cast<u32x4*>(y + i * EPC) = DT<T>::pack(f);
    }
}

template <bool SILU, bool RAW = false>
__global__ __launch_bounds__(256) void gn_apply_pair8_kernel(const float* __restrict__ x, bf16* __restrict__ y, const float* __restrict__ scale,
                                                             const float* __restrict__ shift, long n8_total, int HW, int C, bf16* __restrict__ yraw = nullptr) {
    const int cch = C / 8;
    const int lo_off = pair_lo(C);
    for (long i = (long)blockIdx.x * 256 + threadIdx.x; i < n8_total; i += (long)gridDim.x * 256) {
        const long pix = i / cch;
        const int c = (int)(i - pix * cch) * 8;
        const int b = (int)(pix / HW);
        const f32x4 v0 = *reinterpret_cast<const f32x4*>(x + pix * C + c), v1 = *reinterpret_cast<const f32x4*>(x + pix * C + c + 4);
        const f32x4 s0 = *reinterpret_cast<const f32x4*>(scale + (long)b * C + c), s1 = *reinterpret_cast<const f32x4*>(scale + (long)b * C + c + 4);
        const f32x4 h0 = *reinterpret_cast<const f32x4*>(shift + (long)b * C + c), h1 = *reinterpret_cast<const f32x4*>(shift + (long)b * C + c + 4);
        float f[8];
#pragma unroll
        for (int e = 0; e < 4; ++e) {
            f[e] = v0[e] * s0[e] + h0[e];
            f[4 + e] = v1[e] * s1[e] + h1[e];
        }
        if (SILU) {
#pragma unroll
            for (int e = 0; e < 8; ++e) f[e] = silu_fast(f[e]);
        }
        u32x4 hi, lo;
#pragma unroll
        for (int w = 0; w < 4; ++w) {
// ... 191 lines not shown
```

freefine_amd/ops.py:

```python
import ctypes as CT
import math

import os

import torch

from . import _lib as L


def _dt(t):
    if t.dtype == torch.float32:
        return L.FFN_F32
    if t.dtype == torch.bfloat16:
        return L.FFN_BF16
    raise TypeError(f"unsupported dtype {t.dtype}")


def epc(dtype):
    return 4 if dtype == torch.float32 else 8


def kstage(dtype):
    return 8 * epc(dtype)

# ... 93 lines not shown
    if x3:
        assert cp % 8 == 0, f"split-bf16 conv weights need Cin % 8 == 0 (Cin={cp})"
        hi, lo = split_hi_lo(w2.reshape(cout, 9, cp))
        if cp % 32 == 0:
            return _mark_x3(torch.stack([hi.reshape(cout, 9, cp // 32, 32), lo.reshape(cout, 9, cp // 32, 32)], dim=3).reshape(cout, 18 * cp).contiguous(), 2)
        return _mark_x3(torch.cat([hi, lo, hi], dim=2).reshape(cout, 27 * cp).contiguous(), 1)
    return pack_linear(w2.reshape(cout, 9 * cp), dtype)


def pack_conv3x3_n4(w):
    assert w.shape[0] == 4 and w.shape[2:] == (3, 3)
    return w.float().permute(0, 2, 3, 1).reshape(4, -1).contiguous()


def conv3x3_n4_eligible(cout, cin):
    return cout == 4 and cin % 16 == 0 and cin <= 448 and os.environ.get("FFN_CONV_N4", "1") != "0"


def conv3x3_n4(x, w4, bias, B, H, W, Cin):
    lib = L.load()
    assert x.is_contiguous() and x.shape[-1] == Cin and x.dtype in (torch.float32, torch.bfloat16)
    out = torch.empty(B, H * W, 4, dtype=torch.float32, device=x.device)
    L.check(_timed("conv3x3_n4_kernel", 2.0 * B * H * W * 4 * 9 * Cin, x.element_size() * x.numel() + 16.0 * B * H * W,
                   lambda: lib.ffn_conv3x3_n4(_stream(), _dt(x), x.data_ptr(), w4.data_ptr(), _p(bias), out.data_ptr(), B, H, W, Cin)), "ffn_conv3x3_n4")
    return out


def up2x_eligible(cin, cout, rows):
    return cin % 64 == 0 and (cout % 256 == 0 or cout % 320 == 0) and rows >= 192


def pack_conv3x3_up2x(w, dtype, x3=False):
    assert dtype == torch.bfloat16 or x3
    cout, cin = w.shape[:2]
    wf = w.float()
    groups = {0: ((0,), (1, 2)), 1: ((0, 1), (2,))}
    out = torch.empty(4, cout, 2, 2, cin, dtype=torch.float32, device=w.device)
    for a in (0, 1):
        for b in (0, 1):
            for dy in (0, 1):
                for dx in (0, 1):
                    acc = torch.zeros(cout, cin, dtype=torch.float32, device=w.device)
                    for ky in groups[a][dy]:
                        for kx in groups[b][dx]:
                            acc += wf[:, :, ky, kx]
                    out[2 * a + b, :, dy, dx] = acc
    if x3:
        assert cin % 32 == 0
        hi, lo = split_hi_lo(out.reshape(4 * cout, 4, cin))
        return _mark_x3(torch.stack([hi.reshape(4 * cout, 4, cin // 32, 32), lo.reshape(4 * cout, 4, cin // 32, 32)], dim=3).reshape(4 * cout, 8 * cin).contiguous(), 2)
    return pack_linear(out.reshape(4 * cout, 4 * cin), dtype)


def conv3x3_up2x(x, w4, bias, B, Hin, Win, Cin, *, out=None):
    lib = L.load()
    cout = w4.shape[0] // 4
    x3 = is_x3(w4)
    per_img = Hin * Win * max(4 * cout * (4 if x3 else 2), Cin * (4 if x3 else 2))
    nb = max(1, ((1 << 30) - 1) // per_img)
    if B > nb:
        if out is None:
            out = torch.empty(B, 4 * Hin * Win, cout, dtype=torch.float32 if x3 else x.dtype, device=x.device)
        for b0 in range(0, B, nb):
            b1 = min(B, b0 + nb)
            conv3x3_up2x(x[b0:b1], w4, bias, b1 - b0, Hin, Win, Cin, out=out[b0:b1])
        return out
    if x3:
        xa = x if pair_width(x) is not None else split_pair(x, Cin)
        assert pair_width(xa) == Cin
        odt, dcode = torch.float32, L.FFN_BF16X3
    else:
        assert x.dtype == torch.bfloat16 and x.is_contiguous()
        xa, odt, dcode = x, x.dtype, L.FFN_BF16
    assert w4.shape[1] >= (8 if x3 else 4) * Cin
    y = torch.empty(B, Hin * Win, 4 * cout, dtype=odt, device=x.device)
    for c in range(4):
        a, b = c >> 1, c & 1
        d = L.IgemmDesc()
        d.A, d.W = xa.data_ptr(), w4.data_ptr() + c * cout * w4.stride(0) * w4.element_size()
        d.bias, d.rowbias, d.residual = _p(bias), None, None
        d.M, d.N, d.K, d.Kpad = B * Hin * Win, cout, 4 * Cin, w4.stride(0)
        d.lda, d.a_lo, d.x3 = (2 * Cin, 32, 2) if x3 else (Cin, 0, 0)
        d.rows_per_batch, d.ldrb = Hin * Win, 0
        d.out, d.ldo, d.ldr = y.data_ptr() + c * cout * y.element_size(), 4 * cout, 0
        d.Hin, d.Win, d.Cin, d.Hout, d.Wout = Hin, Win, Cin, Hin, Win
        d.stride, d.pad, d.upsample = 1, 2 * (1 - a) + (1 - b), 0
        d.flags, d.alpha, d.conv = 0, 1.0, 2
        d.splitk, d.ws, d.ws_bytes = 0, _workspace(x.device).data_ptr(), WS_BYTES
        if _PROF is None:
            L.check(lib.ffn_igemm(_stream(), dcode, CT.byref(d)), "ffn_igemm(conv 2x2)")
        else:
            L.check(_timed(_igemm_name(lib, dcode, d), 2.0 * d.M * cout * 4 * Cin, y.element_size() * (x.numel() + cout * 4 * Cin + d.M * cout),
                           lambda: lib.ffn_igemm(_stream(), dcode, CT.byref(d))), "ffn_igemm(conv 2x2)")
    if out is None:
        out = torch.empty(B, 4 * Hin * Win, cout, dtype=odt, device=x.device)
    out.view(B, Hin, 2, Win, 2, cout).copy_(y.view(B, Hin, Win, 2, 2, cout).permute(0, 1, 3, 2, 4, 5))
    return out


F8_ACT_SCALE = 16.0


def pack_conv3x3_f8(w, cin_pad=None):
    cout, cin = w.shape[:2]
    cp = cin_pad or (cin + 127) // 128 * 128
    w2 = torch.zeros(cout, 3, 3, cp, dtype=torch.float32, device=w.device)
    w2[..., :cin] = w.permute(0, 2, 3, 1).float()
    amax = float(w2.abs().max())
    k = math.floor(math.log2(448.0 / amax)) if amax > 0 else 0
    ws = 2.0 ** k
    q = (w2 * ws).clamp(-448.0, 448.0).to(torch.float8_e4m3fn).reshape(cout, 9 * cp).contiguous().view(torch.uint8)
    q._ffn_f8 = (cp, 1.0 / (ws * F8_ACT_SCALE))
    return q


def is_f8(w):
    return getattr(w, "_ffn_f8", None) is not None


def groupnorm_f8(x, gamma, beta, G, eps, Cp, silu=False, ws=None):
    lib = L.load()
    B, HW, Cc = x.shape
    assert x.dtype == torch.bfloat16
    out = torch.empty(B, HW, Cp, dtype=torch.uint8, device=x.device)
    out._ffn_f8_act = Cc
    partial, scale, shift = ws if ws is not None else gn_workspace(B, HW, Cc, x.device)
    call = lambda: lib.ffn_groupnorm_f8(_stream(), x.data_ptr(), out.data_ptr(), gamma.data_ptr(), beta.data_ptr(), B, HW, Cc, Cp, G, eps,
                                        L.NORM_SILU if silu else 0, F8_ACT_SCALE, partial.data_ptr(), scale.data_ptr(), shift.data_ptr())
    L.check(_timed("gn_partial+gn_finalize+gn_apply_f8", 0.0, x.numel() * 2.0 + out.numel(), call), "ffn_groupnorm_f8")
    return out


def pack_geglu(w, b, dtype, x3=False):
    f2, k = w.shape
    f = f2 // 2
    assert f % 16 == 0
    idx = torch.arange(f, device=w.device).reshape(f // 16, 16)
    order = torch.stack([idx, idx + f], dim=1).reshape(-1)
    wp = pack_linear(w[order], dtype, x3)
    bp = None if b is None else b[order].float().contiguous()
    return wp, bp


def _mark_pair(t, C):
    t._ffn_pair = C
    return t


def pair_width(x):
    return getattr(x, "_ffn_pair", None)


def split_pair(x, K=None):
    lib = L.load()
    assert x.dtype == torch.float32 and x.stride(-1) == 1
    K = K if K is not None else x.shape[-1]
    rows = x.numel() // x.shape[-1]
    ld = x.stride(-2) if x.ndim > 1 else x.shape[-1]
    out = torch.empty(*x.shape[:-1], 2 * K, dtype=torch.bfloat16, device=x.device)
    L.check(_timed("split_pair_kernel", 0.0, 8.0 * rows * K, lambda: lib.ffn_split_pair(_stream(), x.data_ptr(), out.data_ptr(), rows, K, ld)),
            "ffn_split_pair")
    return _mark_pair(out, K)


_WS = {}
WS_BYTES = 96 << 20


def _workspace(device):
    key = (device, torch.cuda.current_stream().cuda_stream)
    ws = _WS.get(key)
    if ws is None:
        ws = _WS[key] = torch.empty(WS_BYTES // 4, dtype=torch.float32, device=device)
    return ws

def linear(x, w, bias=None, *, K=None, out=None, residual=None, rowbias=None, rows_per_batch=None, silu=False,
           geglu=False, out_f32=False, transposed_ld=None, alpha=1.0, splitk=0, out_pair=False, gelu=False, relu=False, kv64_from=None, qgelu=False):
    lib = L.load()
    K = K if K is not None else x.shape[-1]
    M = x.numel() // x.shape[-1]
    N = w.shape[0]
    d = L.IgemmDesc()
    x3 = is_x3(w)
    if x3 and pair_width(x) is not None:
        K = pair_width(x)
        M = x.numel() // x.shape[-1]
        xa = x
    else:
        xa = split_pair(x, K) if x3 else x
    dcode = L.FFN_BF16X3 if x3 else _dt(x)
    d.A, d.W = xa.data_ptr(), w.data_ptr()
    d.bias, d.rowbias, d.residual = _p(bias), _p(rowbias), _p(residual)
    d.M, d.N, d.K, d.Kpad = M, N, K, w.stride(0)
    d.lda = xa.stride(-2) if xa.ndim > 1 else xa.shape[-1]
    d.x3 = int(w._ffn_x3) if x3 else 0
    d.a_lo = (32 if d.x3 == 2 else K) if x3 else 0
    odt = torch.float32 if x3 else x.dtype
    d.rows_per_batch = rows_per_batch or M
    d.ldrb = rowbias.stride(0) if rowbias is not None else 0
    flags = 0
    n_out = N
    if silu:
        flags |= L.IG_OUT_SILU
    if gelu:
        flags |= L.IG_OUT_GELU
    if relu:
        flags |= L.IG_OUT_RELU
    if qgelu:
        flags |= L.IG_OUT_QGELU
    if geglu:
        flags |= L.IG_GEGLU
        n_out = N // 2
    if out_f32:
        flags |= L.IG_OUT_F32
    if transposed_ld is not None:
        flags |= L.IG_OUT_TRANSPOSED
        nb = M // d.rows_per_batch
        if out is None:
            alloc = torch.zeros if transposed_ld > d.rows_per_batch else torch.empty
            out = alloc(nb, N, transposed_ld, dtype=odt, device=x.device)
        d.ldo = transposed_ld
    elif out_pair:
        assert x3 and out is None
        flags |= L.IG_OUT_PAIR
        out = _mark_pair(torch.empty(*x.shape[:-1], 2 * n_out, dtype=torch.bfloat16, device=x.device), n_out)
        d.ldo = 2 * n_out
    else:
        if out is None:
            out = torch.empty(*x.shape[:-1], n_out, dtype=torch.float32 if out_f32 else odt, device=x.device)
        d.ldo = out.stride(-2) if out.ndim > 1 else n_out
    d.ldr = residual.shape[-1] if residual is not None else 0
    d.out = out.data_ptr()
    if kv64_from is not None:
        assert x3 and residual is None and rowbias is None and not (silu or gelu or relu or qgelu or geglu or out_pair)
        flags |= L.IG_OUT_KV64
        d.kv64_from = int(kv64_from)
        splitk = 1
    d.flags, d.alpha, d.conv = flags, alpha, 0
    d.splitk, d.ws, d.ws_bytes = splitk, _workspace(x.device).data_ptr(), WS_BYTES
    if _PROF is None:
        L.check(lib.ffn_igemm(_stream(), dcode, CT.byref(d)), "ffn_igemm")
    else:
        esz = x.element_size()
        L.check(_timed(_igemm_name(lib, dcode, d), 2.0 * M * N * K, esz * (M * K + N * K + M * n_out),
                       lambda: lib.ffn_igemm(_stream(), dcode, CT.byref(d))), "ffn_igemm")
    return out


def conv3x3(x, w, bias, B, Hin, Win, Cin, *, stride=1, pad=1, upsample=False, out=None, residual=None, rowbias=None,
            rowbias_ld=None, out_f32=False, Hout=None, Wout=None, splitk=0, relu=False):
    lib = L.load()
    He, We = (Hin * 2, Win * 2) if upsample else (Hin, Win)
    if Hout is None:
        Hout = (He + 2 * pad - 3) // stride + 1
        Wout = (We + 2 * pad - 3) // stride + 1
    N = w.shape[0]
    d = L.IgemmDesc()
    x3 = is_x3(w)
    f8 = is_f8(w)
    if f8:
        assert x.dtype == torch.uint8 and x.shape[-1] == w._ffn_f8[0] and out_f32 is False
        Cin = x.shape[-1]
        xa = x
    elif x3 and pair_width(x) is not None:
        assert pair_width(x) == Cin
        xa = x
    else:
        xa = split_pair(x, Cin) if x3 else x
    dcode = L.FFN_FP8 if f8 else (L.FFN_BF16X3 if x3 else _dt(x))
    odt = torch.float32 if x3 else (torch.bfloat16 if f8 else x.dtype)
    d.A, d.W = xa.data_ptr(), w.data_ptr()
    d.bias, d.rowbias, d.residual = _p(bias), _p(rowbias), _p(residual)
    d.M, d.N, d.K, d.Kpad = B * Hout * Wout, N, 9 * Cin, w.shape[1]
    d.lda = 2 * Cin if x3 else Cin
    d.x3 = int(w._ffn_x3) if x3 else 0
    d.a_lo = (32 if d.x3 == 2 else Cin) if x3 else 0
    d.rows_per_batch = Hout * Wout
    d.ldrb = (rowbias_ld or rowbias.stride(0)) if rowbias is not None else 0
    if out is None:
        out = torch.empty(B, Hout * Wout, N, dtype=torch.float32 if out_f32 else odt, device=x.device)
    d.out, d.ldo = out.data_ptr(), out.stride(-2)
    d.ldr = residual.shape[-1] if residual is not None else 0
    d.Hin, d.Win, d.Cin, d.Hout, d.Wout = Hin, Win, Cin, Hout, Wout
    d.stride, d.pad, d.upsample = stride, pad, 1 if upsample else 0
    d.flags, d.alpha, d.conv = (L.IG_OUT_F32 if out_f32 else 0) | (L.IG_OUT_RELU if relu else 0), (w._ffn_f8[1] if f8 else 1.0), 1
    d.splitk, d.ws, d.ws_bytes = splitk, _workspace(x.device).data_ptr(), WS_BYTES
    if _PROF is None:
        L.check(lib.ffn_igemm(_stream(), dcode, CT.byref(d)), "ffn_igemm(conv)")
    else:
        esz = x.element_size()
        k_real = 9 * getattr(x, "_ffn_f8_act", Cin)
        L.check(_timed(_igemm_name(lib, dcode, d), 2.0 * d.M * N * k_real, esz * (x.numel() + N * d.K + d.M * N),
                       lambda: lib.ffn_igemm(_stream(), dcode, CT.byref(d))), "ffn_igemm(conv)")
    return out


class AttnEntrySpec:
    __slots__ = ("q_row", "kv_row", "w_const", "w_slope", "wq", "kmask", "qsel", "flags", "hr_row")

    def __init__(self, q_row, kv_row, w_const=1.0, w_slope=0.0, wq=None, kmask=None, qsel=None, flags=0, hr_row=None):
        self.q_row, self.kv_row, self.w_const, self.w_slope = q_row, kv_row, w_const, w_slope
        self.wq, self.kmask, self.qsel, self.flags, self.hr_row = wq, kmask, qsel, flags, hr_row

    def remap(self, row_map, logical_row):
        return AttnEntrySpec(row_map[self.q_row], row_map[self.kv_row], self.w_const, self.w_slope, self.wq, self.kmask, self.qsel,
                             self.flags, logical_row if self.hr_row is None else self.hr_row)

    def pinned(self, logical_row):
        return self if self.hr_row is not None else AttnEntrySpec(self.q_row, self.kv_row, self.w_const, self.w_slope, self.wq, self.kmask, self.qsel,
                                                                  self.flags, logical_row)

    def renumber(self, ren, kv_ren=None):
        kv_ren = ren if kv_ren is None else kv_ren
        if self.q_row not in ren or self.kv_row not in kv_ren:
            raise ValueError(f"attention term (q row {self.q_row}, kv row {self.kv_row}) reaches outside the rows of this phase {sorted(ren)} / {sorted(kv_ren)}")
        return AttnEntrySpec(ren[self.q_row], kv_ren[self.kv_row], self.w_const, self.w_slope, self.wq, self.kmask, self.qsel, self.flags, self.hr_row)

    def shifted(self, base, logical_row, kv_base=None):
        return AttnEntrySpec(self.q_row + base, self.kv_row + (base if kv_base is None else kv_base), self.w_const, self.w_slope, self.wq,
                             self.kmask, self.qsel, self.flags, logical_row if self.hr_row is None else self.hr_row)


def _set_entries(d, passes, b0, nb, ptr=_p):
    for p, rows in enumerate(passes):
        for b in range(nb):
            sp = rows[b0 + b]
            e = d.e[p * L.ATT_MAXB + b]
            if sp is None:
                e.w_const = e.w_slope = 0.0
                continue
            e.q_row, e.kv_row, e.w_const, e.w_slope = sp.q_row, sp.kv_row, sp.w_const, sp.w_slope
            e.wq, e.kmask, e.qsel, e.flags = ptr(sp.wq), ptr(sp.kmask), ptr(sp.qsel), sp.flags
            hr = sp.hr_row if sp.hr_row is not None else (b0 + b if b0 else None)
            e.hr_row = 0 if hr is None else hr + 1


def _takes_kv_images(lib, d):
    probe = L.AttnDesc.from_buffer_copy(d)
    probe.kv_pair = 1
# ... 57 lines not shown
    descs = []
    chunk = L.ATT_MAXB
    if _ROWSPLIT and Bo > 1 and Dh == 64 and S >= 128 and Sk % 64 == 0 and q.is_cuda:
        di = q.device.index if q.device.index is not None else torch.cuda.current_device()
        if di not in _CUS:
            _CUS[di] = torch.cuda.get_device_properties(di).multi_processor_count
        chunk = attn_row_split(Bo, heads * -(-S // 256), L.ATT_MAXB, _CUS[di])
    for b0 in range(0, Bo, chunk):
        nb = min(chunk, Bo - b0)
        d = L.AttnDesc()
        d.q, d.k, d.vt, d.w_dev = q.data_ptr(), k.data_ptr(), vt.data_ptr(), _p(w_dev)
        d.out = out.data_ptr() + b0 * S * Cq * esz
        d.Bo, d.S, d.Sk, d.heads, d.D = nb, S, Sk, heads, Dh
        d.ldq, d.ldk, d.ldvt, d.ldo = q.stride(1), k.stride(1), vt.stride(1), (2 * Cq if out_pair else Cq)
        d.out_pair = 1 if out_pair else 0
        d.scale, d.npass = scale, len(passes)
        d.kv_pair = 1 if kv_images else 0
        _set_entries(d, passes, b0, nb)
        descs.append((b0, nb, d))
    if kv_images:
        assert dcode == L.FFN_BF16X3 and kv_images_ok(Dh, S, Sk)
    elif dcode == L.FFN_BF16X3 and _ATTN_PRESPLIT and k.stride(2) == 1 and vt.stride(2) == 1 and k.stride(0) == Sk * k.stride(1) \
            and vt.stride(0) == heads * Dh * vt.stride(1) and k.shape[0] * Sk * heads * Dh * 4 < 2 ** 31 - 65536:
        if all(_takes_kv_images(lib, d) for _, _, d in descs):
            Bk = k.shape[0]
            kp = torch.empty(Bk, Sk, 2 * heads * Dh, dtype=torch.bfloat16, device=q.device)
            vp = torch.empty(Bk, heads * Dh, 2 * Sk, dtype=torch.bfloat16, device=q.device)
            L.check(_timed("attn_presplit_kernel", 0.0, 16.0 * Bk * Sk * heads * Dh,
                           lambda: lib.ffn_attn_presplit(_stream(), k.data_ptr(), vt.data_ptr(), kp.data_ptr(), vp.data_ptr(), Bk, Sk, heads, k.stride(1), vt.stride(1))),
                    "ffn_attn_presplit")
            for _, _, d in descs:
                d.k, d.vt, d.kv_pair = kp.data_ptr(), vp.data_ptr(), 1
                d.ldk, d.ldvt = heads * Dh, Sk
    for b0, nb, d in descs:
        if _PROF is None:
            L.check(lib.ffn_attn(_stream(), dcode, CT.byref(d)), "ffn_attn")
        else:
            nterms = sum(1 for rows in passes for sp in rows[b0:b0 + nb] if sp is not None and (sp.w_const != 0.0 or sp.w_slope != 0.0))
            nbuf = CT.create_string_buffer(160)
            lib.ffn_attn_kernel_name(dcode, CT.byref(d), nbuf, 160)
            L.check(_timed(nbuf.value.decode(), 4.0 * nterms * S * Sk * Cq,
                           esz * nterms * (S * Cq + 2 * Sk * Cq) + esz * nb * S * Cq,
                           lambda: lib.ffn_attn(_stream(), dcode, CT.byref(d))), "ffn_attn")
    return out


def gn_workspace(B, HW, C, device):
    lib = L.load()
    nchunk = lib.ffn_gn_nchunk(HW)
    return (torch.empty(B * nchunk * 2 * C, dtype=torch.float32, device=device),
            torch.empty(B, C, dtype=torch.float32, device=device), torch.empty(B, C, dtype=torch.float32, device=device))


def groupnorm(x, gamma, beta, G, eps, silu=False, out=None, ws=None, pair=False):
    lib = L.load()
    B, HW, Cc = x.shape
    if pair:
        assert x.dtype == torch.float32 and out is None
        out = _mark_pair(torch.empty(B, HW, 2 * Cc, dtype=torch.bfloat16, device=x.device), Cc)
    if out is None:
        out = torch.empty_like(x)
    if lib.ffn_gn_fused(B, HW, Cc, G):
        partial = scale = shift = None
    else:
        partial, scale, shift = ws if ws is not None else gn_workspace(B, HW, Cc, x.device)
    fl = (L.NORM_SILU if silu else 0) | (L.NORM_OUT_PAIR if pair else 0)
    nb = B
    if partial is not None and _GN_CHUNK_MB > 0 and x.is_contiguous() and out.is_contiguous():
        row_bytes = HW * Cc * x.element_size()
        nb = max(1, min(B, int(_GN_CHUNK_MB * 2 ** 20) // row_bytes))
        nb = -(-B // -(-B // nb))
    def call():
        rc = 0
        for b0 in range(0, B, nb):
            n = min(nb, B - b0)
            rc = lib.ffn_groupnorm(_stream(), _dt(x), x.data_ptr() + b0 * HW * Cc * x.element_size(), out.data_ptr() + b0 * HW * out.shape[-1] * out.element_size(),
                                   gamma.data_ptr(), beta.data_ptr(), n, HW, Cc, G, eps, fl, _p(partial), _p(scale), _p(shift))
            if rc:
                break
        return rc
    if _PROF is None:
        L.check(call(), "ffn_groupnorm")
    else:
        name = f"gn_fused_kernel<{_tname(x)}>" if partial is None else f"gn_partial+gn_finalize+gn_apply<{_tname(x)}>"
        L.check(_timed(name, 0.0, 2.0 * x.numel() * x.element_size(), call), "ffn_groupnorm")
    return out


def groupnorm_pair_raw(x, gamma, beta, G, eps, silu=False, ws=None):
    lib = L.load()
    B, HW, Cc = x.shape
    if not _GN_RAW or Cc % 8 != 0 or lib.ffn_gn_fused(B, HW, Cc, G) or not x.is_contiguous():
        return groupnorm(x, gamma, beta, G, eps, silu=silu, pair=True, ws=ws), split_pair(x, Cc)
    assert x.dtype == torch.float32
    y = _mark_pair(torch.empty(B, HW, 2 * Cc, dtype=torch.bfloat16, device=x.device), Cc)
    yr = _mark_pair(torch.empty(B, HW, 2 * Cc, dtype=torch.bfloat16, device=x.device), Cc)
    partial, scale, shift = ws if ws is not None else gn_workspace(B, HW, Cc, x.device)
    call = lambda: lib.ffn_groupnorm_pair_raw(_stream(), x.data_ptr(), y.data_ptr(), yr.data_ptr(), gamma.data_ptr(), beta.data_ptr(), B, HW, Cc, G, eps,
                                              L.NORM_SILU if silu else 0, _p(partial), _p(scale), _p(shift))
    if _PROF is None:
        L.check(call(), "ffn_groupnorm_pair_raw")
    else:
        L.check(_timed("gn_partial+gn_finalize+gn_apply<float> (+ raw pair)", 0.0, 3.0 * x.numel() * x.element_size(), call), "ffn_groupnorm_pair_raw")
    return y, yr


def layernorm(x, gamma, beta, eps=1e-5, out=None, pair=False):
    lib = L.load()
    Cc = x.shape[-1]
    M = x.numel() // Cc
    if pair:
        assert x.dtype == torch.float32 and out is None
        out = _mark_pair(torch.empty(*x.shape[:-1], 2 * Cc, dtype=torch.bfloat16, device=x.device), Cc)
        call = lambda: lib.ffn_layernorm_pair(_stream(), x.data_ptr(), out.data_ptr(), gamma.data_ptr(), beta.data_ptr(), M, Cc, eps)
    else:
        if out is None:
            out = torch.empty_like(x)
        call = lambda: lib.ffn_layernorm(_stream(), _dt(x), x.data_ptr(), out.data_ptr(), gamma.data_ptr(), beta.data_ptr(), M, Cc, eps)
    if _PROF is None:
        L.check(call(), "ffn_layernorm")
    else:
        L.check(_timed(f"layernorm_kernel<{_tname(x)}>", 0.0, 2.0 * x.numel() * x.element_size(), call), "ffn_layernorm")
    return out


def softmax_rows(x, scale=1.0, out=None):
    lib = L.load()
    N = x.shape[-1]
    M = x.numel() // N
    if out is None:
        out = torch.empty_like(x)
    L.check(_timed(f"softmax_rows_kernel<{_tname(x)}>", 0.0, 2.0 * x.numel() * x.element_size(),
                   lambda: lib.ffn_softmax_rows(_stream(), _dt(x), x.data_ptr(), out.data_ptr(), M, N, scale)), "ffn_softmax_rows")
    return out


def cfg_masked(eps_u, eps_c, mask_f, cfg, out=None):
    lib = L.load()
    if out is None:
        out = torch.empty_like(eps_u)
    HW = eps_u.shape[-1] * eps_u.shape[-2]
    L.check(_timed("cfg_masked_kernel", 0.0, 12.0 * eps_u.numel(),
                   lambda: lib.ffn_cfg_masked(_stream(), eps_u.data_ptr(), eps_c.data_ptr(), _p(mask_f), float(cfg), out.data_ptr(),
                                              eps_u.numel(), HW)), "ffn_cfg_masked")
    return out


def ddim_inv_step(eps, x, c_bt, c_at, c_an, c_bn, want_pred_x0=False):
    lib = L.load()
# ... 4 lines not shown
                                                 x.numel())), "ffn_ddim_inv_step")
    return x_next, p0


def ddim_ctrl_step(eps, x, noise, m_f, om_f, c_bt, c_at, c_ap, c_dir, c_dirm, stdv, row_masked, want_pred_x0=False):
    lib = L.load()
    rows = x.shape[0]
    d = L.CtrlStepDesc()
    x_prev = torch.empty_like(x)
    p0 = torch.empty_like(x) if want_pred_x0 else None
    d.eps, d.x, d.noise, d.m, d.om = eps.data_ptr(), x.data_ptr(), _p(noise), m_f.data_ptr(), om_f.data_ptr()
    d.x_prev, d.pred_x0 = x_prev.data_ptr(), _p(p0)
    d.c_bt, d.c_at, d.c_ap, d.c_dir = c_bt, c_at, c_ap, c_dir
    for b in range(rows):
        d.c_dirm[b], d.stdv[b], d.row_masked[b] = c_dirm[b], stdv[b], int(row_masked[b])
    d.rows, d.CHW, d.HW = rows, x[0].numel(), x.shape[-1] * x.shape[-2]
    L.check(_timed("ddim_ctrl_step_kernel", 0.0, 20.0 * x.numel(), lambda: lib.ffn_ddim_ctrl_step(_stream(), CT.byref(d))), "ffn_ddim_ctrl_step")
    return x_prev, p0


def pack_nchw(src, src_rows, CP, dtype, out=None):
    lib = L.load()
    Bs, Cl, H, W = src.shape
    B = len(src_rows)
    if out is None:
        out = torch.empty(B, H * W, CP, dtype=dtype, device=src.device)
    for b0 in range(0, B, 16):
        nb = min(16, B - b0)
        d = L.PackDesc()
        d.src, d.dst = src.data_ptr(), out.data_ptr() + b0 * H * W * CP * out.element_size()
        for i in range(nb):
            d.src_row[i] = src_rows[b0 + i]
        d.B, d.Cl, d.CP, d.HW = nb, Cl, CP, H * W
        L.check(_timed(f"pack_nchw_kernel<{_tname(out)}>", 0.0, nb * H * W * (4.0 * Cl + CP * out.element_size()),
                       lambda: lib.ffn_pack_nchw(_stream(), _dt(out), CT.byref(d))), "ffn_pack_nchw")
    return out


def nhwc_to_nchw_f32(src, C_, H, W, out=None):
    lib = L.load()
    B, HW, ld = src.shape
    if out is None:
        out = torch.empty(B, C_, H, W, dtype=torch.float32, device=src.device)
    L.check(_timed("nhwc_to_nchw_f32_kernel", 0.0, 8.0 * B * HW * C_,
                   lambda: lib.ffn_nhwc_to_nchw_f32(_stream(), src.data_ptr(), out.data_ptr(), B, HW, C_, ld)), "ffn_nhwc_to_nchw_f32")
    return out


def concat(a, b, out=None):
    lib = L.load()
    C1, C2 = a.shape[-1], b.shape[-1]
    rows = a.numel() // C1
    base = getattr(a, "_ffn_cat_base", None)
    if out is None and base is not None and base.shape[-1] == C1 + C2:
        L.check(_timed(f"concat_kernel<{_tname(b)}>", 0.0, 2.0 * rows * C2 * b.element_size(),
                       lambda: lib.ffn_concat(_stream(), _dt(b), None, b.data_ptr(), base.data_ptr(), rows, C1, C2)), "ffn_concat")
        return base
    if base is not None:
        a = a.contiguous()
    if out is None:
        out = torch.empty(*a.shape[:-1], C1 + C2, dtype=a.dtype, device=a.device)
    L.check(_timed(f"concat_kernel<{_tname(a)}>", 0.0, 2.0 * rows * (C1 + C2) * a.element_size(),
                   lambda: lib.ffn_concat(_stream(), _dt(a), a.data_ptr(), b.data_ptr(), out.data_ptr(), rows, C1, C2)), "ffn_concat")
    return out


def cat_dst(shape_lead, C1, C2, dtype, device):
    base = torch.empty(*shape_lead, C1 + C2, dtype=dtype, device=device)
    view = base[..., :C1]
    view._ffn_cat_base = base
    return view


def timestep_freqs(dim, device, max_period=10000.0, shift=0.0):
    half = dim // 2
    exponent = -math.log(max_period) * torch.arange(half, dtype=torch.float32) / (half - shift)
    return torch.exp(exponent).to(device)


def timestep_embed(t_dev, freq, B, dtype, flip=True, out=None):
    lib = L.load()
    half = freq.numel()
    if out is None:
        out = torch.empty(B, 2 * half, dtype=dtype, device=freq.device)
    L.check(_timed(f"timestep_embed_kernel<{_tname(out)}>", 0.0, float(out.numel() * out.element_size()),
                   lambda: lib.ffn_timestep_embed(_stream(), _dt(out), t_dev.data_ptr(), freq.data_ptr(), out.data_ptr(), B, half,
                                                  1 if flip else 0)), "ffn_timestep_embed")
    return out


def transpose(src, ld_dst=None, out=None):
    lib = L.load()
    B, R, Cc = src.shape
    ld_dst = ld_dst or R
    if out is None:
        out = torch.zeros(B, Cc, ld_dst, dtype=src.dtype, device=src.device)
    L.check(_timed(f"transpose_kernel<{_tname(src)}>", 0.0, 2.0 * src.numel() * src.element_size(),
                   lambda: lib.ffn_transpose(_stream(), _dt(src), src.data_ptr(), out.data_ptr(), B, R, Cc, Cc, ld_dst)), "ffn_transpose")
    return out


def cast(src, dtype, out=None):
    lib = L.load()
    if out is None:
        out = torch.empty(src.shape, dtype=dtype, device=src.device)
    L.check(_timed(f"cast_kernel<{_tname(src)}, {_tname(out)}>", 0.0, float(src.numel() * (src.element_size() + out.element_size())),
                   lambda: lib.ffn_cast(_stream(), _dt(src), _dt(out), src.data_ptr(), out.data_ptr(), src.numel())), "ffn_cast")
    return out


def relu(x, out=None):
    lib = L.load()
    out = torch.empty_like(x) if out is None else out
    L.check(_timed("eltwise_kernel<relu>", 0.0, 2.0 * x.numel() * x.element_size(),
                   lambda: lib.ffn_eltwise(_stream(), _dt(x), L.ELT_RELU, x.data_ptr(), None, out.data_ptr(), x.numel())), "ffn_eltwise")
    return out

# ... 96 lines not shown
```

freefine_amd/unet.py:

```python
import ctypes as CT
import os
import weakref

import torch

from . import _lib as L
from . import ops
from .config import UNetConfig

_GRAPH_RAW = os.environ.get("FFN_GRAPH_RAW", "1") != "0"


class _Res:
    pass


class HipUNet:
    def __init__(self, cfg: UNetConfig, state, dtype=torch.bfloat16, device="cuda:0", x3=False, fp8_conv=False):
        assert not x3 or dtype == torch.float32, "split-bf16 mode keeps fp32 activations"
        assert not fp8_conv or dtype == torch.bfloat16, "fp8 convolutions are an option of the bf16 fast mode"
        self.x3 = bool(x3)
        self.fp8_conv = bool(fp8_conv)
        self.cfg, self.dtype, self.device = cfg, dtype, torch.device(device)
        self.in_channels = cfg.in_channels
# ... 423 lines not shown
            if plan["passes"] is None:
                fps.append(0)
                continue
            rows = tuple(tuple(None if e is None else (e.q_row, e.kv_row, e.w_const, e.w_slope, e.flags, e.hr_row,
                                                       0 if e.wq is None else e.wq.data_ptr(),
                                                       0 if e.kmask is None else e.kmask.data_ptr(),
                                                       0 if e.qsel is None else e.qsel.data_ptr()) for e in r) for r in plan["passes"])
            fps.append((plan["kind"], plan["needs_cg"], rows))
        self._in_phase_a = self._kv_ext = False
        return (self.hook, tuple(fps))

    def join_block_tb(self, join):
        tb = len([t for blk in self.down if blk.attn for t in blk.attn]) + 1
        for blk in self.up[:join]:
            tb += len(blk.attn) if blk.attn else 0
        return tb

    def _capture(self, sample, text_kv, sig):
        ctrls = self._ctrls()
        state = [(c.cur_att_layer, c.cur_step) for c in ctrls]
        x_static = sample.clone()
        ru = self._reuse
        ref_in = None
        if ru is not None and ru["mode"] == "replay":
            ref_in = [t.clone() for t in ru["state"]]
            ru["state_run"] = ref_in
        if ru is not None and ru["mode"] == "replay_kv":
            ref_in = ru["static"] = []
            ru["static_bufs"] = []
        self._run(x_static, text_kv)
        if ru is not None and ru["mode"] == "replay_kv":
            ru["static_ready"] = True
        for c, st in zip(ctrls, state):
            c.cur_att_layer, c.cur_step = st
        torch.cuda.synchronize()
        graph = torch.cuda.CUDAGraph()
        if self._capture_stream is None:
            self._capture_stream = torch.cuda.Stream(device=x_static.device)
        with torch.cuda.graph(graph, stream=self._capture_stream):
            out = self._run(x_static, text_kv)
        rec = ru is not None and ru["mode"] == "record"
        g = dict(graph=graph, x=x_static, out=out, ref_in=ref_in, ref_bufs=ru.get("static_bufs") if ru is not None else None,
                 boundary=self.last_boundary if rec else None, kv=self.last_kv if rec else None, device=x_static.device.index)
        if ru is not None:
            for k in ("state_run", "static", "static_bufs", "static_ready"):
                ru.pop(k, None)
        self._graphs[sig] = g
        return g

    def _gn(self, x, gb, eps, silu):
        B, HW, C = x.shape
        return ops.groupnorm(x, gb[0], gb[1], self.cfg.norm_num_groups, eps, silu=silu, pair=self.x3)

    def _gn_conv_in(self, x, gb, w):
        if ops.is_f8(w):
            return ops.groupnorm_f8(x, gb[0], gb[1], self.cfg.norm_num_groups, self.cfg.norm_eps, w._ffn_f8[0], silu=True)
        return self._gn(x, gb, self.cfg.norm_eps, True)

    def _resblock(self, r, x, B, H, W, temb_all, out=None):
        cin = x.shape[-1]
        if r.sc is not None and self.x3 and not ops.is_f8(r.c1[0]) and ops.pair_width(x) is None and x.dtype == torch.float32:
            h, x = ops.groupnorm_pair_raw(x, r.n1[0], r.n1[1], self.cfg.norm_num_groups, self.cfg.norm_eps, silu=True)
        else:
            h = self._gn_conv_in(x, r.n1, r.c1[0])
        rb = temb_all[:, r.temb_off:r.temb_off + r.cout]
        h = ops.conv3x3(h, r.c1[0], r.c1[1], B, H, W, cin, rowbias=rb, rowbias_ld=temb_all.shape[1])
        h = self._gn_conv_in(h, r.n2, r.c2[0])
        if r.sc is not None:
            x = ops.linear(x, r.sc[0], r.sc[1], K=cin)
        return ops.conv3x3(h, r.c2[0], r.c2[1], B, H, W, r.cout, residual=x, out=out)

    def _without_ref_queries(self, plan, B):
        keep = self._reuse["idx_a_list"]
        passes = plan["passes"] if plan["passes"] is not None else [[ops.AttnEntrySpec(b, b) for b in range(B)]]
        pin = lambda e, r: e if (e is None or e.hr_row is not None) else ops.AttnEntrySpec(e.q_row, e.kv_row, e.w_const, e.w_slope, e.wq, e.kmask, e.qsel, e.flags, r)
        out = dict(plan)
        out["passes"] = [[pin(rows[r], r) for r in keep] for rows in passes]
        return out

    def _self_plan(self, t, place, B, S, drop_ref_queries=False):
        if self.controller is None:
            return dict(kind="plain", needs_cg=False, passes=[[ops.AttnEntrySpec(r, r, hr_row=r) for r in self._reuse["idx_a_list"]]]) if drop_ref_queries else None
        plan = self._plan(False, place, B, S, t.heads)
        if drop_ref_queries:
            assert plan["kind"] != "shared_kv"
            plan = self._without_ref_queries(plan, B)
        return plan

    def _attention(self, t, is_cross, place, q, k, vt, ldq_view, B, S, Sk, plan=None, kv_images=False):
        D = t.C // t.heads
        scale = D ** -0.5
        if is_cross and self.controller is not None:
            plan = self._plan(is_cross, place, B, S, t.heads)
        if plan is None:
            return ops.attention(q, k, vt, t.heads, scale, None, Sk=Sk, C=t.C, x3=self.x3, out_pair=self.x3, kv_images=kv_images)
        if plan["kind"] == "shared_kv":
            assert not kv_images
            rr = plan["ref_rows"]
            kc = k[..., :t.C] if k.shape[-1] != t.C else k
            k2 = torch.cat([kc, kc[rr]], dim=1).contiguous()
            vt2 = torch.cat([vt[..., :Sk], vt[rr][..., :Sk]], dim=2).contiguous()
            return ops.attention(q, k2, vt2, t.heads, scale, plan["passes"], Sk=2 * Sk, C=t.C, x3=self.x3, out_pair=self.x3)
        return ops.attention(q, k, vt, t.heads, scale, plan["passes"], Sk=Sk, C=t.C, w_dev=self.cg_dev if plan["needs_cg"] else None, x3=self.x3,
                             out_pair=self.x3, kv_images=kv_images)

    def _kv_buffers(self, B, S, C, ldv):
        ru = self._reuse
        i = ru["cursor"]
        ru["cursor"] = i + 1
        if ru.get("static_ready"):
            return ru["static_bufs"][i]
        k_ref, vt_ref = ru["state"][2 * i], ru["state"][2 * i + 1]
        nr = k_ref.shape[0]
        assert tuple(k_ref.shape) == (nr, S, C) and tuple(vt_ref.shape) == (nr, C, ldv), (tuple(k_ref.shape), tuple(vt_ref.shape), (S, C, ldv))
        qk = torch.empty(B + nr, S, 2 * C, dtype=self.dtype, device=self.device)
        vt = torch.empty(B + nr, C, ldv, dtype=self.dtype, device=self.device)
        qk[B:, :, C:].copy_(k_ref)
        vt[B:].copy_(vt_ref)
        if ru.get("static") is not None:
            ru["static_bufs"].append((qk, vt))
            ru["static"] += [qk[B:, :, C:], vt[B:]]
        return qk, vt

    def _transformer_block(self, t, x, B, H, W, place, kv_text, out=None, drop=None, tb=0):
        S, C = H * W, t.C
        res0 = x
        ru = self._reuse
        h = self._gn(x, t.norm, 1e-6, False)
        h = ops.linear(h, t.proj_in[0], t.proj_in[1], K=C)
        y = ops.layernorm(h, *t.ln[0], pair=self.x3)
        ldv = (S + 7) // 8 * 8
        if ru is not None and ru["mode"] == "replay_kv" and tb >= ru["kv_from"]:
            qk, vt = self._kv_buffers(B, S, C, ldv)
            ops.linear(y, t.w_qk1, None, K=C, out=qk[:B])
            ops.linear(y, t.w_v1, None, K=C, rows_per_batch=S, transposed_ld=ldv, out=vt[:B])
            self._kv_ext = True
            a = self._attention(t, False, place, qk[:B], qk[..., C:], vt, 2 * C, B, S, S, plan=self._self_plan(t, place, B, S))
            self._kv_ext = False
        else:
            plan = self._self_plan(t, place, B, S, drop_ref_queries=drop is not None)
            rec = ru is not None and ru["mode"] == "record" and ru.get("kv_from") is not None and tb >= ru["kv_from"]
            img = self.x3 and not rec and (plan is None or plan["kind"] != "shared_kv") and \
                ops.kv_images_ok(C // t.heads, S, S, None if plan is None else plan["passes"], B * max(S * 2 * C, C * ldv) * 4)
            qk = ops.linear(y, t.w_qk1, None, K=C, kv64_from=C if img else None)
            vt = ops.linear(y, t.w_v1, None, K=C, rows_per_batch=S, transposed_ld=ldv, kv64_from=0 if img else None)
            if rec:
                self.last_kv.append((qk[..., C:], vt))
            a = self._attention(t, False, place, qk, qk[..., C:], vt, 2 * C, B, S, S, plan=plan, kv_images=img)
        if drop is not None:
            idx, kv_text = drop
            h, res0, B = h.index_select(0, idx), res0.index_select(0, idx), idx.shape[0]
            self._in_phase_a = True
        h = ops.linear(a, t.o1[0], t.o1[1], K=C, residual=h)
        y = ops.layernorm(h, *t.ln[1], pair=self.x3)
        q = ops.linear(y, t.w_q2, None, K=C)
        k2, vt2 = kv_text
        a = self._attention(t, True, place, q, k2, vt2, C, B, S, k2.shape[1])
        h = ops.linear(a, t.o2[0], t.o2[1], K=C, residual=h)
        y = ops.layernorm(h, *t.ln[2], pair=self.x3)
        y = ops.linear(y, t.ff1[0], t.ff1[1], K=C, geglu=True, out_pair=self.x3)
        h = ops.linear(y, t.ff2[0], t.ff2[1], K=4 * C, residual=h, out_pair=self.x3 and C % 32 == 0)
        return ops.linear(h, t.proj_out[0], t.proj_out[1], K=C, residual=res0, out=out)

    def _run(self, sample, text_kv):
        cfg = self.cfg
        B, _, H, W = sample.shape
        dt = self.dtype
        ru = self._reuse
        replay = ru is not None and ru["mode"] == "replay"
        record = ru is not None and ru["mode"] == "record"
        replay_kv = ru is not None and ru["mode"] == "replay_kv"
        BB = B
        if replay:
            sample = sample.index_select(0, ru["idx_a"])
            B = sample.shape[0]
            text_kv = list(ru["text_kv_a"][:self.join_block_tb(ru["join"])]) + list(text_kv[self.join_block_tb(ru["join"]):])
        if replay_kv:
            sample = sample.index_select(0, ru["idx_a"])
            B = sample.shape[0]
            text_kv = ru["text_kv_a"]
            ru["cursor"] = 0
        if record and ru.get("kv_from") is not None:
            self.last_kv = []
        self._in_phase_a = replay
        ti = iter(text_kv)
        tb = 0
        te = ops.timestep_embed(self.t_dev, self.freq, BB, dt, flip=cfg.flip_sin_to_cos)
        e1 = ops.linear(te, self.te1[0], self.te1[1], K=self.te1[2], silu=True)
        e2 = ops.linear(e1, self.te2[0], self.te2[1], K=self.te2[2], silu=True)
        temb_all = ops.linear(e2, self.temb_w, self.temb_b, K=self.te2[0].shape[0], out_f32=True)
        temb_full = temb_all
        temb_all = temb_all[:B]
        x = ops.pack_nchw(sample, list(range(B)), self.cin_pad, dt)
        x = ops.conv3x3(x, self.conv_in[0], self.conv_in[1], B, H, W, self.cin_pad)
        skips = [(x, H, W)]
        n = len(self.down)
        for i, blk in enumerate(self.down):
            for j, r in enumerate(blk.res):
                x = self._resblock(r, x, B, H, W, temb_all)
                if blk.attn:
                    x = self._transformer_block(blk.attn[j], x, B, H, W, "down", next(ti), tb=tb)
                    tb += 1
                skips.append((x, H, W))
            if blk.down is not None:
                C = x.shape[-1]
                x = ops.conv3x3(x, blk.down[0], blk.down[1], B, H, W, C, stride=2)
                H, W = (H + 1) // 2, (W + 1) // 2
                skips.append((x, H, W))
        x = self._resblock(self.mid.res[0], x, B, H, W, temb_all)
        x = self._transformer_block(self.mid.attn[0], x, B, H, W, "mid", next(ti), tb=tb)
        tb += 1
        def cat_dst(C1, HW):
            return ops.cat_dst((B, HW), C1, skips[-1][0].shape[-1], dt, x.device) if skips else None
        x = self._resblock(self.mid.res[1], x, B, H, W, temb_all, out=cat_dst(self.mid.res[1].cout, H * W))
        for i, blk in enumerate(self.up):
            if ru is not None and ru.get("join") is not None and i == ru["join"]:
                if record:
                    self.last_boundary = [x] + [s for s, _, _ in reversed(skips)]
                if replay:
                    state = ru.get("state_run") or ru["state"]
                    assert len(state) == 1 + len(skips), (len(state), len(skips))
                    merge = lambda a, r: torch.cat([a, r.to(a.dtype)], 0).index_select(0, ru["perm"])
                    x = merge(x, state[0])
                    skips = [(merge(s, st), sh, sw) for (s, sh, sw), st in zip(skips, reversed(state[1:]))]
                    B, temb_all = BB, temb_full
                    self._in_phase_a = False
            for j, r in enumerate(blk.res):
                s, sh, sw = skips.pop()
                assert (sh, sw) == (H, W)
                x = ops.concat(x, s)
                dst = cat_dst(r.cout, H * W) if j + 1 < len(blk.res) else None
                x = self._resblock(r, x, B, H, W, temb_all, out=None if blk.attn else dst)
                if blk.attn:
                    last = replay and bool(ru.get("drop_tail")) and blk.attn[j] is self.transformers[-1]
                    drop = (ru["idx_a"], ru["text_kv_a"][-1]) if last else None
                    x = self._transformer_block(blk.attn[j], x, B, H, W, "up", next(ti), out=dst, drop=drop, tb=tb)
                    tb += 1
                    if last:
                        assert dst is None and i == len(self.up) - 1 and j == len(blk.res) - 1, "the last transformer block closes the network"
                        B, temb_all = x.shape[0], temb_full[:x.shape[0]]
            if blk.up is not None:
                C = x.shape[-1]
                if blk.up2 is not None and ops.up2x_eligible(C, C, B * H * W):
                    x = ops.conv3x3_up2x(x, blk.up2, blk.up[1], B, H, W, C, out=cat_dst(C, 4 * H * W))
                else:
                    x = ops.conv3x3(x, blk.up[0], blk.up[1], B, H, W, C, upsample=True, out=cat_dst(C, 4 * H * W))
                H, W = 2 * H, 2 * W
        C = x.shape[-1]
        if self.conv_out_n4 is not None:
            x = ops.groupnorm(x, self.norm_out[0], self.norm_out[1], cfg.norm_num_groups, cfg.norm_eps, silu=True)
            eps = ops.conv3x3_n4(x, self.conv_out_n4, self.conv_out[1], B, H, W, C)
        else:
            x = self._gn(x, self.norm_out, cfg.norm_eps, True)
            eps = ops.conv3x3(x, self.conv_out[0], self.conv_out[1], B, H, W, C, out_f32=True)
        eps = ops.nhwc_to_nchw_f32(eps, cfg.out_channels, H, W)
        self._in_phase_a = False
        if B != BB:
            eps = torch.zeros(BB, *eps.shape[1:], dtype=eps.dtype, device=eps.device).index_copy_(0, ru["idx_a"], eps)
        return eps
```

freefine_amd/vae.py:

```python
import os

import torch

from . import ops
from .config import VAEConfig


class _O:
    pass


class HipVAE:
    def __init__(self, cfg: VAEConfig, state, dtype=torch.bfloat16, device="cuda:0", x3=False):
        assert not x3 or dtype == torch.float32
        self.x3 = bool(x3)
        self.cfg, self.dtype, self.device = cfg, dtype, torch.device(device)
        self.G = cfg.norm_num_groups
        self._pack(state)

    def _f32(self, t):
        return t.detach().float().contiguous().to(self.device)

    def _conv(self, st, name, cin_pad=None, cout_pad=None):
        w, b = st[name + ".weight"].float().to(self.device), st[name + ".bias"].float().to(self.device)
# ... 24 lines not shown
        a.q, a.k, a.v, a.o = (self._lin(st, f"{p}.{n}") for n in ("to_q", "to_k", "to_v", "to_out.0"))
        return a

    def _mid(self, st, p):
        m = _O()
        m.r0, m.attn, m.r1 = self._res(st, p + ".resnets.0"), self._attn(st, p + ".attentions.0"), self._res(st, p + ".resnets.1")
        return m

    def _pack(self, st):
        cfg = self.cfg
        e = 8 if self.x3 else ops.epc(self.dtype)
        s = cfg.scaling_factor
        n = len(cfg.block_out_channels)
        self.img_cp = (cfg.in_channels + e - 1) // e * e
        self.enc_in = self._conv(st, "encoder.conv_in", self.img_cp)
        self.enc_down = []
        for i in range(n):
            b = _O()
            b.res = [self._res(st, f"encoder.down_blocks.{i}.resnets.{j}") for j in range(cfg.layers_per_block)]
            b.down = self._conv(st, f"encoder.down_blocks.{i}.downsamplers.0.conv") if i < n - 1 else None
            self.enc_down.append(b)
        self.enc_mid = self._mid(st, "encoder.mid_block")
        self.enc_norm = (self._f32(st["encoder.conv_norm_out.weight"]), self._f32(st["encoder.conv_norm_out.bias"]))
        self.enc_out = self._conv(st, "encoder.conv_out")
        lc = cfg.latent_channels
        self.lat_cp = (2 * lc + e - 1) // e * e
        qw, qb = st["quant_conv.weight"].float().reshape(2 * lc, 2 * lc), st["quant_conv.bias"].float()
        self.quant = (ops.pack_linear((qw[:lc] * s).to(self.device), self.dtype, self.x3), (qb[:lc] * s).to(self.device).contiguous(), 2 * lc)
        self.zin_cp = (lc + e - 1) // e * e
        pw = torch.zeros(self.zin_cp, self.zin_cp)
        pw[:lc, :lc] = st["post_quant_conv.weight"].float().reshape(lc, lc) / s
        pb = torch.zeros(self.zin_cp)
        pb[:lc] = st["post_quant_conv.bias"].float()
        self.post_quant = (ops.pack_linear(pw.to(self.device), self.dtype, self.x3), pb.to(self.device).contiguous(), self.zin_cp)
        self.dec_in = self._conv(st, "decoder.conv_in", self.zin_cp)
        self.dec_mid = self._mid(st, "decoder.mid_block")
        self.dec_up = []
        for i in range(n):
            b = _O()
            b.res = [self._res(st, f"decoder.up_blocks.{i}.resnets.{j}") for j in range(cfg.layers_per_block + 1)]
            b.up = self._conv(st, f"decoder.up_blocks.{i}.upsamplers.0.conv") if i < n - 1 else None
            b.up2 = None
            if b.up is not None and (self.dtype == torch.bfloat16 or self.x3) and os.environ.get("FFN_UP2X", "1") != "0":
                wu = st[f"decoder.up_blocks.{i}.upsamplers.0.conv.weight"].float().to(self.device)
                if ops.up2x_eligible(wu.shape[1], wu.shape[0], 192):
                    b.up2 = ops.pack_conv3x3_up2x(wu, self.dtype, x3=self.x3)
            self.dec_up.append(b)
        self.dec_norm = (self._f32(st["decoder.conv_norm_out.weight"]), self._f32(st["decoder.conv_norm_out.bias"]))
        self.dec_out = self._conv(st, "decoder.conv_out", cout_pad=4)

    def _gn(self, x, gb, silu):
        return ops.groupnorm(x, gb[0], gb[1], self.G, 1e-6, silu=silu, pair=self.x3)

    def _resblock(self, r, x, B, H, W):
        cin = x.shape[-1]
        h = self._gn(x, r.n1, True)
        h = ops.conv3x3(h, r.c1[0], r.c1[1], B, H, W, cin)
        h = self._gn(h, r.n2, True)
        if r.sc is not None:
            x = ops.linear(x, r.sc[0], r.sc[1], K=cin)
        return ops.conv3x3(h, r.c2[0], r.c2[1], B, H, W, r.cout, residual=x)

    def _attention(self, a, x, B, S):
        C = x.shape[-1]
        y = self._gn(x, a.gn, False)
        q = ops.linear(y, a.q[0], a.q[1], K=C)
        k = ops.linear(y, a.k[0], a.k[1], K=C)
        ld = (S + 7) // 8 * 8
        vt = ops.linear(y, a.v[0], a.v[1], K=C, rows_per_batch=S, transposed_ld=ld)
        o = torch.empty(B, S, C, dtype=self.dtype, device=self.device)
        for b in range(B):
            scores = ops.linear(q[b], k[b], None, K=C)
            p = ops.softmax_rows(scores, C ** -0.5)
            ops.linear(p, vt[b], None, K=S, out=o[b])
        return ops.linear(o, a.o[0], a.o[1], K=C, residual=x)

    def _midblock(self, m, x, B, H, W):
        x = self._resblock(m.r0, x, B, H, W)
        x = self._attention(m.attn, x, B, H * W)
        return self._resblock(m.r1, x, B, H, W)

    @torch.no_grad()
    def encode_mean_scaled(self, img_u8=None, x_nchw=None):
        if img_u8 is not None:
            B, H, W, _ = img_u8.shape
            x = ops.image_to_nhwc(img_u8.to(self.device).contiguous(), self.img_cp, self.dtype)
        else:
            B, _, H, W = x_nchw.shape
            x = ops.pack_nchw(x_nchw.to(self.device, torch.float32).contiguous(), list(range(B)), self.img_cp, self.dtype)
        x = ops.conv3x3(x, self.enc_in[0], self.enc_in[1], B, H, W, self.img_cp)
        for blk in self.enc_down:
            for r in blk.res:
                x = self._resblock(r, x, B, H, W)
            if blk.down is not None:
                C = x.shape[-1]
                x = ops.conv3x3(x, blk.down[0], blk.down[1], B, H, W, C, stride=2, pad=0, Hout=H // 2, Wout=W // 2)
                H, W = H // 2, W // 2
        x = self._midblock(self.enc_mid, x, B, H, W)
        C = x.shape[-1]
        x = self._gn(x, self.enc_norm, True)
        x = ops.conv3x3(x, self.enc_out[0], self.enc_out[1], B, H, W, C)
        z = ops.linear(x, self.quant[0], self.quant[1], K=self.quant[2], out_f32=True)
        return ops.nhwc_to_nchw_f32(z, self.cfg.latent_channels, H, W)

    @torch.no_grad()
    def decode_image(self, latents):
        latents = latents.to(self.device, torch.float32).contiguous()
        B, _, H, W = latents.shape
        z = ops.pack_nchw(latents, list(range(B)), self.zin_cp, self.dtype)
        x = ops.linear(z, self.post_quant[0], self.post_quant[1], K=self.zin_cp)
        x = ops.conv3x3(x, self.dec_in[0], self.dec_in[1], B, H, W, self.zin_cp)
        x = self._midblock(self.dec_mid, x, B, H, W)
        for blk in self.dec_up:
            for r in blk.res:
                x = self._resblock(r, x, B, H, W)
            if blk.up is not None:
                C = x.shape[-1]
                if blk.up2 is not None and ops.up2x_eligible(C, C, B * H * W):
                    x = ops.conv3x3_up2x(x, blk.up2, blk.up[1], B, H, W, C)
                else:
                    x = ops.conv3x3(x, blk.up[0], blk.up[1], B, H, W, C, upsample=True)
                H, W = 2 * H, 2 * W
        C = x.shape[-1]
        x = self._gn(x, self.dec_norm, True)
        x = ops.conv3x3(x, self.dec_out[0], self.dec_out[1], B, H, W, C)
        return ops.nhwc_to_image(x, H, W)
```

include/freefine_hip.h:

```cpp
#ifndef FREEFINE_HIP_H
#define FREEFINE_HIP_H
#include <stdint.h>
#ifdef __cplusplus
extern "C" {
#endif

enum { FFN_F32 = 0, FFN_BF16 = 1, FFN_BF16X3 = 2 ,
       FFN_FP8 = 3  };
enum { FFN_OK = 0, FFN_EINVAL = -22, FFN_ENOSYS = -38, FFN_EHIP = -5 };

int ffn_version(void);
const char* ffn_last_error(void);
int ffn_device_info(int device, char* name, int name_len);
int ffn_graph_launch(void* stream, void* graph_exec);

enum {
    FFN_IG_OUT_SILU = 1 << 0,
    FFN_IG_OUT_F32 = 1 << 1,
    FFN_IG_GEGLU = 1 << 2,
    FFN_IG_OUT_TRANSPOSED = 1 << 3,
    FFN_IG_OUT_PAIR = 1 << 4,
    FFN_IG_OUT_GELU = 1 << 5,
    FFN_IG_OUT_KV64 = 1 << 7,
    FFN_IG_OUT_RELU = 1 << 6,
    FFN_IG_OUT_QGELU = 1 << 8
};
typedef struct ffn_igemm_desc {
    const void* A;
    const void* W;
    void* out;
    const float* bias;
    const float* rowbias;
    const void* residual;
    int M, N, K, Kpad;
    int lda, ldo, ldr, ldrb;
    int rows_per_batch;
    int Hin, Win, Cin, Hout, Wout, stride, pad, upsample;
    int flags;
    float alpha;
    int conv;
    int splitk;
    void* ws;
    long ws_bytes;
    int a_lo;
    int x3;
    int f8;
    int kv64_from;
} ffn_igemm_desc;
int ffn_igemm(void* stream, int dtype, const ffn_igemm_desc* d);
int ffn_split_pair(void* stream, const float* src, void* dst, long rows, int C, int ld_src);
int ffn_conv3x3_n4(void* stream, int dtype, const void* x, const float* w, const float* bias, float* out, int B, int H, int W, int Cin);
int ffn_groupnorm_f8(void* stream, const void* x_bf16, void* y_e4m3, const float* gamma, const float* beta, int B, int HW, int C, int Cp,
                     int G, float eps, int silu, float qscale, float* partial_ws, float* scale, float* shift);
int ffn_igemm_tune(void* stream, int dtype, const ffn_igemm_desc* d);
int ffn_igemm_tune_entry_ints(void);
int ffn_igemm_tune_export(int* buf, int max_entries);
int ffn_igemm_tune_import(const int* buf, int n_entries);
int ffn_igemm_tune_clear(void);
int ffn_igemm_tune_enable(int on);
int ffn_igemm_tune_stamp(void);
int ffn_igemm_num_configs(void);
int ffn_igemm_force_config(int cfg);
int ffn_igemm_variant(const ffn_igemm_desc* d, int* bm, int* bn);
int ffn_igemm_kernel_name(int dtype, const ffn_igemm_desc* d, char* buf, int len);

#define FFN_ATT_MAXP 4
#define FFN_ATT_MAXB 16
enum { FFN_ATT_HEAD_RULE = 1, FFN_ATT_UNIFORM_SEL1 = 2, FFN_ATT_UNIFORM_SEL0 = 4,
       FFN_ATT_CAUSAL = 8  };
typedef struct ffn_attn_entry {
    int q_row, kv_row;
    float w_const, w_slope;
    const float* wq;
    const uint8_t* kmask;
    const uint8_t* qsel;
    int flags;
    int hr_row;
} ffn_attn_entry;
typedef struct ffn_attn_desc {
    const void* q;
    const void* k;
    const void* vt;
    void* out;
    const float* w_dev;
    int Bo, S, Sk, heads, D;
    int ldq, ldk, ldvt, ldo;
    float scale;
    int npass;
    int out_pair;
    int kv_pair;
    ffn_attn_entry e[FFN_ATT_MAXP * FFN_ATT_MAXB];
} ffn_attn_desc;
int ffn_attn(void* stream, int dtype, const ffn_attn_desc* d);
int ffn_attn_presplit(void* stream, const float* k, const float* vt, void* k_pair, void* vt_pair, int rows, int Sk, int heads, int ldk, int ldvt);
int ffn_attn_variant(int dtype, int D, int* dp, int* qf);
int ffn_attn_kernel_name(int dtype, const ffn_attn_desc* d, char* buf, int len);

enum { FFN_ELT_RELU = 0, FFN_ELT_ADD = 1 };
int ffn_eltwise(void* stream, int dtype, int op, const void* a, const void* b, void* y, long n);
int ffn_resize_bilinear(void* stream, int dtype, const void* x, void* y, int B, int Hin, int Win, int Hout, int Wout, int C, int relu);

typedef struct ffn_splat_xform {
    float center[3], translate[3], rotate[9] , scale[3];
    float tan_half_fov;
} ffn_splat_xform;
int ffn_splat_lift(void* stream, const float* depth, const int* idx, float* pts, int n, int W, int H, float fx, float fy);
int ffn_splat_project(void* stream, const float* pts, float* proj, int n, const ffn_splat_xform* x);
int ffn_splat_bin(void* stream, int fill, const float* proj, int n, float radius, int W, int H, int* counts, const int* offs, int* list);
int ffn_splat_render(void* stream, const float* proj, const float* rgb, const int* offs, const int* list, float radius, int K, int W, int H,
                     float* image, int* idx_sum, uint8_t* covered);

enum { FFN_NORM_SILU = 1, FFN_NORM_OUT_PAIR = 2 };
int ffn_gn_nchunk(int HW);
int ffn_gn_fused(int B, int HW, int C, int G);
int ffn_gn_stats(void* stream, int dtype, const void* x, const float* gamma, const float* beta, int B, int HW, int C, int G,
                 float eps, float* partial_ws, float* scale, float* shift);
int ffn_gn_apply(void* stream, int dtype, const void* x, void* y, const float* scale, const float* shift, int B, int HW,
                 int C, int silu);
int ffn_groupnorm(void* stream, int dtype, const void* x, void* y, const float* gamma, const float* beta, int B, int HW, int C, int G,
                  float eps, int silu, float* partial_ws, float* scale, float* shift);
int ffn_groupnorm_pair_raw(void* stream, const void* x, void* y_pair, void* yraw_pair, const float* gamma, const float* beta, int B, int HW, int C, int G,
                           float eps, int silu, float* partial_ws, float* scale, float* shift);
int ffn_layernorm(void* stream, int dtype, const void* x, void* y, const float* gamma, const float* beta, int M, int C,
                  float eps);
int ffn_layernorm_pair(void* stream, const float* x, void* y, const float* gamma, const float* beta, int M, int C, float eps);
int ffn_softmax_rows(void* stream, int dtype, const void* x, void* y, long M, int N, float scale);

int ffn_cfg_masked(void* stream, const float* eps_u, const float* eps_c, const float* mask, float cfg, float* eps, long n,
                   int HW);
int ffn_ddim_inv_step(void* stream, const float* eps, const float* x, float c_bt, float c_at, float c_an, float c_bn,
                      float* x_next, float* pred_x0, long n);
typedef struct ffn_ctrl_step_desc {
    const float* eps;
    const float* x;
    const float* noise;
    const float* m;
    const float* om;
    float* x_prev;
    float* pred_x0;
    float c_bt, c_at, c_ap, c_dir;
    float c_dirm[8], stdv[8];
    int row_masked[8];
    int rows, CHW, HW;
} ffn_ctrl_step_desc;
int ffn_ddim_ctrl_step(void* stream, const ffn_ctrl_step_desc* d);

typedef struct ffn_pack_desc {
    const float* src;
    void* dst;
    int src_row[16];
    int B, Cl, CP, HW;
} ffn_pack_desc;
int ffn_pack_nchw(void* stream, int dtype, const ffn_pack_desc* d);
int ffn_nhwc_to_nchw_f32(void* stream, const float* src, float* dst, int B, int HW, int C, int ld);
int ffn_concat(void* stream, int dtype, const void* a, const void* b, void* out, long rows, int C1, int C2);
int ffn_timestep_embed(void* stream, int dtype, const float* t_dev, const float* freq, void* out, int B, int half, int flip);
int ffn_transpose(void* stream, int dtype, const void* src, void* dst, int B, int R, int C, int ld_src, int ld_dst);
int ffn_cast(void* stream, int src_dtype, int dst_dtype, const void* src, void* dst, long n);
int ffn_embed_tokens(void* stream, int dtype, const int* ids, const float* table, const float* pos, void* out, long M, int S, int C, int V);
int ffn_image_to_nhwc(void* stream, int dtype, const uint8_t* img, void* dst, long npix, int CP);
int ffn_nhwc_to_image(void* stream, int dtype, const void* src, float* dst, int B, int HW, int ld);

#ifdef __cplusplus
}
#endif
#endif
```

Before: 1.986.

## Fuse GroupNorm statistics into split-bf16 igemm epilogue

Adds an optional stats output to the split-bf16 pipelined igemm. The epilogue reduces per-16-row partial sums and sums of squares with DPP adds and stores them to a side buffer. A new groupnorm_stats entry finalizes the mean and variance from these partials (merging two sources across concat), so GroupNorm no longer needs its own pass over the activation to compute statistics. Non-pp configurations fall back to a separate rowstats kernel. This adds extra epilogue stores, a deeper vmcnt wait, and a double-precision finalize, and it only applies to x3 fp32 outputs that meet the alignment and shape rules.

```diff
diff --git a/freefine_amd/_lib.py b/freefine_amd/_lib.py
--- a/freefine_amd/_lib.py
+++ b/freefine_amd/_lib.py
@@ -11,6 +11,7 @@
 ATT_MAXP, ATT_MAXB = 4, 16
 ATT_HEAD_RULE, ATT_UNIFORM_SEL1, ATT_UNIFORM_SEL0, ATT_CAUSAL = 1, 2, 4, 8
 NORM_SILU, NORM_OUT_PAIR = 1, 2
+IG_STATS_ROWS = 16
 
 
 class IgemmDesc(C.Structure):
@@ -25,6 +26,7 @@
         ("flags", C.c_int), ("alpha", C.c_float), ("conv", C.c_int),
         ("splitk", C.c_int), ("ws", C.c_void_p), ("ws_bytes", C.c_long),
         ("a_lo", C.c_int), ("x3", C.c_int), ("f8", C.c_int), ("kv64_from", C.c_int),
+        ("stats", C.c_void_p), ("ld_stats", C.c_int),
     ]
 
 
@@ -100,6 +102,8 @@
     "ffn_gn_apply": (_i, [_vp, _i, _vp, _vp, _vp, _vp, _i, _i, _i, _i]),
     "ffn_groupnorm": (_i, [_vp, _i, _vp, _vp, _vp, _vp, _i, _i, _i, _i, _f, _i, _vp, _vp, _vp]),
     "ffn_groupnorm_pair_raw": (_i, [_vp, _vp, _vp, _vp, _vp, _vp, _i, _i, _i, _i, _f, _i, _vp, _vp, _vp]),
+    "ffn_groupnorm_stats": (_i, [_vp, _vp, _vp, _vp, _vp, _vp, _i, _i, _i, _i, _f, _i, _vp, _i, _i, _i, _vp, _i, _i, _vp, _vp]),
+    "ffn_gn_rowstats": (_i, [_vp, _vp, _vp, _i, _i, _i, _i]),
     "ffn_layernorm": (_i, [_vp, _i, _vp, _vp, _vp, _vp, _i, _i, _f]),
     "ffn_layernorm_pair": (_i, [_vp, _vp, _vp, _vp, _vp, _i, _i, _f]),
     "ffn_softmax_rows": (_i, [_vp, _i, _vp, _vp, _l, _i, _f]),
diff --git a/freefine_amd/csrc/capi.hip b/freefine_amd/csrc/capi.hip
--- a/freefine_amd/csrc/capi.hip
+++ b/freefine_amd/csrc/capi.hip
@@ -66,7 +66,7 @@
     return FFN_OK;
 }
 
-extern "C" int ffn_version(void) { return 2; }
+extern "C" int ffn_version(void) { return 3; }
 extern "C" const char* ffn_last_error(void) { return g_err; }
 extern "C" int ffn_device_info(int device, char* name, int name_len) {
     hipDeviceProp_t prop;
@@ -297,7 +297,16 @@
 }
 static bool x3_cfg(int cfg) { return cfg == CFG_64x64 || cfg == CFG_128x64 || cfg == CFG_128x128_8 || is_pp_cfg(cfg); }
 template <int AMODE, bool X3 = false, bool F8 = false>
+static int launch_bf16_cfg_kernels(hipStream_t s, const ffn_igemm_desc& d, IgChoice ch);
+static int launch_rowstats(hipStream_t s, const float* x, float* stats, int M, int N, int ldx, int ld_stats);
+template <int AMODE, bool X3 = false, bool F8 = false>
 static int launch_bf16_cfg(hipStream_t s, const ffn_igemm_desc& d, IgChoice ch) {
+    const int rc = launch_bf16_cfg_kernels<AMODE, X3, F8>(s, d, ch);
+    if (rc || !d.stats || (is_pp_cfg(ch.cfg) && ch.splitk == 1)) return rc;
+    return launch_rowstats(s, (const float*)d.out, d.stats, d.M, d.N, d.ldo, d.ld_stats);
+}
+template <int AMODE, bool X3, bool F8>
+static int launch_bf16_cfg_kernels(hipStream_t s, const ffn_igemm_desc& d, IgChoice ch) {
     const IgCfgInfo& c = kCfg[ch.cfg];
     if ((X3 || F8) && !x3_cfg(ch.cfg)) return fail(FFN_EINVAL, "igemm: configuration %d is not built for split-bf16 / fp8 problems", ch.cfg);
     const int ntiles = ((d.M + c.bm - 1) / c.bm) * ((d.N + c.bn - 1) / c.bn);
@@ -339,6 +348,14 @@
             (void)hipGetLastError();
 #define FFN_PP_LAUNCH(BM_, BN_, RES_, GEGLU_)                                              \
     do {                                                                                   \
+        if constexpr (X3 && !(GEGLU_)) {                                                   \
+            if (d.stats) {                                                                 \
+                auto kern = igemm_pp_stats_kernel<BM_, BN_, AMODE, RES_>;                  \
+                if ((rc = set_lds(kern, pplds))) return rc;                                \
+                hipLaunchKernelGGL(kern, dim3(grid), dim3(512), pplds, s, d, 1);           \
+                break;                                                                     \
+            }                                                                              \
+        }                                                                                  \
         auto kern = igemm_pp_kernel<BM_, BN_, AMODE, RES_, (GEGLU_) && !F8, false, false, X3, F8>;      \
         if ((rc = set_lds(kern, pplds))) return rc;                                        \
         hipLaunchKernelGGL(kern, dim3(grid), dim3(512), pplds, s, d, 1);                   \
@@ -453,7 +470,7 @@
     k.Kpad = d.Kpad;
     k.ldr = d.residual ? d.ldr : 0;
     k.dtype = d.x3 ? (FFN_BF16X3 | (d.x3 << 8)) : (d.f8 ? FFN_FP8 : FFN_BF16);
-    k.ptrs = (d.bias ? 1 : 0) | (d.rowbias ? 2 : 0) | (d.residual ? 4 : 0) | (d.ws && d.ws_bytes > 0 ? 8 : 0);
+    k.ptrs = (d.bias ? 1 : 0) | (d.rowbias ? 2 : 0) | (d.residual ? 4 : 0) | (d.ws && d.ws_bytes > 0 ? 8 : 0) | (d.stats ? 16 : 0);
     const long per = (long)d.M * d.N * 4;
     k.wslabs = d.ws ? (int)(d.ws_bytes / per > 1024 ? 1024 : d.ws_bytes / per) : 0;
     k.rpb = d.rows_per_batch;
@@ -711,6 +728,10 @@
         }
         if (is_pp_cfg(ch.cfg)) {
             const bool split = ch.splitk > 1;
+            if (x3 && !split && d->stats) {
+                snprintf(buf, len, "void igemm_pp_stats_kernel<%d, %d, %d, %s>(ffn_igemm_desc, int)", c.bm, c.bn, d->conv ? 1 : 0, d->residual ? "true" : "false");
+                return FFN_OK;
+            }
             snprintf(buf, len, "void igemm_pp_kernel<%d, %d, %d, %s, %s, %s, false, %s, %s>(ffn_igemm_desc, int)", c.bm, c.bn, d->conv ? 1 : 0,
                      (!split && d->residual) ? "true" : "false", (!split && (d->flags & FFN_IG_GEGLU)) ? "true" : "false", split ? "true" : "false",
                      x3 ? "true" : "false", f8 ? "true" : "false");
@@ -946,6 +967,11 @@
     {
         const int act = d->flags & (FFN_IG_OUT_SILU | FFN_IG_OUT_GELU | FFN_IG_OUT_RELU | FFN_IG_OUT_QGELU);
         REQUIRE((act & (act - 1)) == 0, "igemm: SILU / GELU / QGELU / RELU are mutually exclusive");
+    }
+    if (d->stats) {
+        REQUIRE(dtype == FFN_BF16X3 && !(d->flags & ~FFN_IG_OUT_F32), "igemm: stats need FFN_BF16X3 and the plain row-major fp32 output (flags=%d)", d->flags);
+        REQUIRE(d->M % FFN_IG_STATS_ROWS == 0 && d->ld_stats >= d->N && d->ld_stats % 2 == 0 && aligned16(d->stats) && (long)(d->M / FFN_IG_STATS_ROWS) * d->ld_stats * 8 < (1l << 31),
+                "igemm: stats need M %% %d == 0, an even ld_stats >= N, a 16-byte aligned buffer below 2 GiB (M=%d, N=%d, ld_stats=%d)", FFN_IG_STATS_ROWS, d->M, d->N, d->ld_stats);
     }
     if (d->ws) REQUIRE(aligned16(d->ws) && d->ws_bytes >= 0, "igemm: workspace must be 16-byte aligned");
     REQUIRE(d->splitk >= 0, "igemm: splitk must be >= 0");
@@ -1290,6 +1316,36 @@
     else LAUNCH((gn_apply_pair8_kernel<false, true>), dim3(grid_for(n8)), dim3(256), 0, s, (const float*)x, (bf16*)y, scale, shift, n8, HW, C, (bf16*)yraw);
     return check_launch("gn_apply(pair + raw pair)");
 }
+static int launch_rowstats(hipStream_t s, const float* x, float* stats, int M, int N, int ldx, int ld_stats) {
+    const long total = (long)(M / FFN_IG_STATS_ROWS) * (N / 4);
+    LAUNCH(gn_rowstats_kernel, dim3((unsigned)((total + 255) / 256)), dim3(256), 0, s, x, stats, total, N / 4, ldx, ld_stats);
+    return check_launch("gn_rowstats");
+}
+extern "C" int ffn_gn_rowstats(void* stream, const float* x, float* stats, int M, int N, int ldx, int ld_stats) {
+    REQUIRE(x && stats && aligned16(x) && aligned16(stats), "gn_rowstats: null / unaligned pointer");
+    REQUIRE(M > 0 && M % FFN_IG_STATS_ROWS == 0 && N > 0 && N % 4 == 0 && ldx >= N && ldx % 4 == 0 && ld_stats >= N && ld_stats % 2 == 0,
+            "gn_rowstats: M %% %d == 0, N %% 4 == 0, ldx %% 4 == 0, even ld_stats >= N (M=%d, N=%d, ldx=%d, ld_stats=%d)", FFN_IG_STATS_ROWS, M, N, ldx, ld_stats);
+    return launch_rowstats(reinterpret_cast<hipStream_t>(stream), x, stats, M, N, ldx, ld_stats);
+}
+extern "C" int ffn_groupnorm_stats(void* stream, const void* x, void* y, void* yraw, const float* gamma, const float* beta, int B, int HW, int C, int G, float eps,
+                                   int flags, const float* stats_a, int nchunk_a, int ld_a, int C1, const float* stats_b, int nchunk_b, int ld_b, float* scale,
+                                   float* shift) {
+    REQUIRE(x && y && gamma && beta && scale && shift && stats_a, "groupnorm_stats: null pointer");
+    REQUIRE(B > 0 && HW > 0 && G > 0 && C % G == 0 && C % 4 == 0 && C1 > 0 && C1 <= C, "groupnorm_stats: bad shape (C=%d, G=%d, C1=%d)", C, G, C1);
+    REQUIRE(nchunk_a > 0 && ld_a >= C1, "groupnorm_stats: source a: nchunk=%d, ld=%d for %d channels", nchunk_a, ld_a, C1);
+    if (C1 < C) REQUIRE(stats_b && nchunk_b > 0 && ld_b >= C - C1, "groupnorm_stats: source b: nchunk=%d, ld=%d for %d channels", nchunk_b, ld_b, C - C1);
+    REQUIRE((reinterpret_cast<uintptr_t>(stats_a) & 7) == 0 && (reinterpret_cast<uintptr_t>(stats_b) & 7) == 0, "groupnorm_stats: statistics must be 8-byte aligned");
+    hipStream_t s = reinterpret_cast<hipStream_t>(stream);
+    LAUNCH(gn_finalize_stats_kernel, dim3(G, B), dim3(256), 0, s, stats_a, nchunk_a, ld_a, C1, stats_b, nchunk_b, ld_b, gamma, beta, scale, shift, HW, C, G, eps);
+    if (int rc = check_launch("gn_finalize_stats")) return rc;
+    if (!yraw) return ffn_gn_apply(stream, FFN_F32, x, y, scale, shift, B, HW, C, flags);
+    REQUIRE((flags & FFN_NORM_OUT_PAIR) && C % 8 == 0 && aligned16(x) && aligned16(y) && aligned16(yraw) && y != yraw && yraw != x && y != x,
+            "groupnorm_stats: the raw pair output needs FFN_NORM_OUT_PAIR, C %% 8 == 0 and three distinct aligned buffers");
+    const long n8 = (long)B * HW * (C / 8);
+    if (flags & FFN_NORM_SILU) LAUNCH((gn_apply_pair8_kernel<true, true>), dim3(grid_for(n8)), dim3(256), 0, s, (const float*)x, (bf16*)y, scale, shift, n8, HW, C, (bf16*)yraw);
+    else LAUNCH((gn_apply_pair8_kernel<false, true>), dim3(grid_for(n8)), dim3(256), 0, s, (const float*)x, (bf16*)y, scale, shift, n8, HW, C, (bf16*)yraw);
+    return check_launch("gn_apply(pair + raw pair)");
+}
 extern "C" int ffn_groupnorm_f8(void* stream, const void* x, void* y, const float* gamma, const float* beta, int B, int HW, int C, int Cp, int G,
                                 float eps, int silu, float qscale, float* partial_ws, float* scale, float* shift) {
     REQUIRE(x && y && gamma && beta && partial_ws && scale && shift, "groupnorm_f8: null pointer (the workspace is always needed)");
diff --git a/freefine_amd/csrc/igemm_p8.h b/freefine_amd/csrc/igemm_p8.h
--- a/freefine_amd/csrc/igemm_p8.h
+++ b/freefine_amd/csrc/igemm_p8.h
@@ -27,6 +27,21 @@
 __device__ __forceinline__ void pp_wait_vmcnt() {
     if (PP_ABL != 2) asm volatile("s_waitcnt vmcnt(%0)" ::"n"(N) : "memory");
 }
+__device__ __forceinline__ void pp_rowsum4(const float (&x)[4], float (&o)[4]) {
+#define PP_RS_STEP(A_, B_, C_, D_, CTRL_)                                   \
+    "v_add_f32_dpp %0, " A_ ", " A_ " " CTRL_ " row_mask:0xf bank_mask:0xf\n" \
+    "v_add_f32_dpp %1, " B_ ", " B_ " " CTRL_ " row_mask:0xf bank_mask:0xf\n" \
+    "v_add_f32_dpp %2, " C_ ", " C_ " " CTRL_ " row_mask:0xf bank_mask:0xf\n" \
+    "v_add_f32_dpp %3, " D_ ", " D_ " " CTRL_ " row_mask:0xf bank_mask:0xf\n"
+    asm volatile("s_nop 1\n"
+                 PP_RS_STEP("%4", "%5", "%6", "%7", "quad_perm:[1,0,3,2]")
+                 PP_RS_STEP("%0", "%1", "%2", "%3", "quad_perm:[2,3,0,1]")
+                 PP_RS_STEP("%0", "%1", "%2", "%3", "row_half_mirror")
+                 PP_RS_STEP("%0", "%1", "%2", "%3", "row_mirror")
+                 : "=&v"(o[0]), "=&v"(o[1]), "=&v"(o[2]), "=&v"(o[3])
+                 : "v"(x[0]), "v"(x[1]), "v"(x[2]), "v"(x[3]));
+#undef PP_RS_STEP
+}
 __device__ __forceinline__ void pp_barrier() {
     asm volatile("" ::: "memory");
     __builtin_amdgcn_s_barrier();
@@ -36,9 +51,10 @@
 #ifdef PP_TRACE
 __device__ unsigned long long pp_trace[256 * 64];
 #endif
-template <int BM, int BN, int AMODE, bool RES, bool GEGLU, bool SPLIT = false, bool TRANS = false, bool X3 = false, bool F8 = false>
-__global__ __launch_bounds__(512) void igemm_pp_kernel(const IgemmParams p, int splitk = 1) {
+template <int BM, int BN, int AMODE, bool RES, bool GEGLU, bool SPLIT, bool TRANS, bool X3, bool F8, bool STATS>
+__device__ __forceinline__ void igemm_pp_body(const IgemmParams p, int splitk) {
     typedef bf16 T;
+    static_assert(!STATS || (X3 && !GEGLU && !SPLIT && !TRANS && !F8), "statistics: the fp32 row-major epilogue of the split-bf16 core");
     constexpr int HM = BM / 2;
     constexpr int FM = HM / 16;
     constexpr int FH = FM / 2;
@@ -86,6 +102,14 @@
     const long o_bytes = TRANS ? (long)((p.M + p.rows_per_batch - 1) / p.rows_per_batch) * p.N * p.ldo * OSZ : (long)p.M * p.ldo * OSZ;
     const __amdgpu_buffer_rsrc_t rsrcO = __builtin_amdgcn_make_buffer_rsrc(p.out, 0, (int)o_bytes, 0x00020000);
     const __amdgpu_buffer_rsrc_t rsrcR = __builtin_amdgcn_make_buffer_rsrc(const_cast<void*>(p.residual), 0, RES ? (int)((long)p.M * p.ldr * OSZ) : 0, 0x00020000);
+
+    auto stats_arg = [&](int& ld) -> float* {
+        typedef const char __attribute__((address_space(4)))* kptr_t;
+        kptr_t ka = (kptr_t)__builtin_amdgcn_kernarg_segment_ptr();
+        asm volatile("" : "+s"(ka));
+        ld = *reinterpret_cast<const int __attribute__((address_space(4)))*>(ka + offsetof(IgemmParams, ld_stats));
+        return *reinterpret_cast<float* const __attribute__((address_space(4)))*>(ka + offsetof(IgemmParams, stats));
+    };
 
     int l_tile = first, l_kt = 0;
     int l_k0 = 0;
@@ -397,6 +421,13 @@
         }
         if constexpr (X3) {
             const int voff = (pr * p.ldo + 4 * pg) * 4;
+            int ld_st = 0;
+            float* st_ptr = nullptr;
+            if constexpr (STATS) st_ptr = stats_arg(ld_st);
+            const __amdgpu_buffer_rsrc_t rsrcS = __builtin_amdgcn_make_buffer_rsrc(st_ptr, 0, (p.M >> 4) * ld_st * 8, 0x00020000);
+            const int st_lane = (ln & 15) < 2 ? (4 * (ln >> 4) + 2 * (ln & 15)) * 8 : OOB;
+            const int st_row = ld_st * 8;
+            int st_so = ((m0 >> 4) + i0) * st_row + n0 * 8;
 #pragma unroll
             for (int i = i0; i < i0 + FH; ++i) {
                 const int vo = m0 + i * 16 + pr < p.M ? voff : OOB;
@@ -420,6 +451,16 @@
                 } else {
 #pragma unroll
                     for (int j = 0; j < FN; ++j) {
+                        if constexpr (STATS) {
+                            const f32x4 a = acc[i][j];
+                            const float c01[4] = {a[0], a[0] * a[0], a[1], a[1] * a[1]}, c23[4] = {a[2], a[2] * a[2], a[3], a[3] * a[3]};
+                            float s01[4], s23[4];
+                            pp_rowsum4(c01, s01);
+                            pp_rowsum4(c23, s23);
+                            const bool hi2 = (ln & 15) == 1;
+                            const f32x4 sv = {hi2 ? s23[0] : s01[0], hi2 ? s23[1] : s01[1], hi2 ? s23[2] : s01[2], hi2 ? s23[3] : s01[3]};
+                            __builtin_amdgcn_raw_buffer_store_b128(__builtin_bit_cast(u32x4, sv), rsrcS, (m0 + i * 16 < p.M ? st_lane : OOB) + j * 128, st_so, 0);
+                        }
                         u32x4 w = __builtin_bit_cast(u32x4, acc[i][j]);
                         w[0] = perm(w[0]); w[1] = perm(w[1]); w[2] = perm(w[2]); w[3] = perm(w[3]);
                         const int nf = n0 + j * 16;
@@ -452,6 +493,7 @@
                         }
                         __builtin_amdgcn_raw_buffer_store_b128(w, rsrcO, vo, ((m0 + i * 16) * p.ldo + n0 + j * 16) * 4, 0);
                     }
+                    st_so += st_row;
                 }
             }
             return;
@@ -625,7 +667,8 @@
                 k_position();
                 issue_a(0, nb);
                 issue_a(1, nb);
-                pp_wait_vmcnt<FN + NAL + 2 * NST>();
+                if constexpr (STATS) pp_wait_vmcnt<(FN + NAL + 4 * NST < 63 ? FN + NAL + 4 * NST : 63)>();
+                else pp_wait_vmcnt<FN + NAL + 2 * NST>();
                 init_rows(c_tile, I0_t{});
                 __builtin_amdgcn_sched_barrier(0);
                 read_low_set(buf);
@@ -797,3 +840,12 @@
     if (blockIdx.x == 7) pp_stamp_out[tid] = *reinterpret_cast<const unsigned long long*>(smem + CV + 12288 + tid * 8);
 #endif
 }
+
+template <int BM, int BN, int AMODE, bool RES, bool GEGLU, bool SPLIT = false, bool TRANS = false, bool X3 = false, bool F8 = false>
+__global__ __launch_bounds__(512) void igemm_pp_kernel(const IgemmParams p, int splitk = 1) {
+    igemm_pp_body<BM, BN, AMODE, RES, GEGLU, SPLIT, TRANS, X3, F8, false>(p, splitk);
+}
+template <int BM, int BN, int AMODE, bool RES>
+__global__ __launch_bounds__(512) void igemm_pp_stats_kernel(const IgemmParams p, int splitk = 1) {
+    igemm_pp_body<BM, BN, AMODE, RES, false, false, false, true, false, true>(p, 1);
+}
diff --git a/freefine_amd/csrc/norms.h b/freefine_amd/csrc/norms.h
--- a/freefine_amd/csrc/norms.h
+++ b/freefine_amd/csrc/norms.h
@@ -105,6 +105,65 @@
         scale[(long)b * C + c] = sc;
         shift[(long)b * C + c] = beta[c] - fmean * sc;
     }
+}
+
+__device__ __forceinline__ void gn_sum_source(const float* __restrict__ src, int nchunk, int ld, int c0, int w, int tid, double& s, double& ss) {
+    for (int i = tid; i < nchunk * w; i += 256) {
+        const int ch = i / w;
+        const float2 v = *reinterpret_cast<const float2*>(src + ((long)ch * ld + c0 + (i - ch * w)) * 2);
+        s += (double)v.x;
+        ss += (double)v.y;
+    }
+}
+__global__ __launch_bounds__(256) void gn_finalize_stats_kernel(const float* __restrict__ sa, int nca, int lda, int C1, const float* __restrict__ sb, int ncb,
+                                                                int ldb, const float* __restrict__ gamma, const float* __restrict__ beta,
+                                                                float* __restrict__ scale, float* __restrict__ shift, int HW, int C, int G, float eps) {
+    __shared__ double red[2][4];
+    const int g = blockIdx.x, b = blockIdx.y, tid = threadIdx.x;
+    const int cg = C / G, c0 = g * cg, c1 = c0 + cg;
+    double s = 0.0, ss = 0.0;
+    if (c0 < C1) gn_sum_source(sa + (long)b * nca * lda * 2, nca, lda, c0, min(c1, C1) - c0, tid, s, ss);
+    if (c1 > C1) gn_sum_source(sb + (long)b * ncb * ldb * 2, ncb, ldb, max(c0, C1) - C1, c1 - max(c0, C1), tid, s, ss);
+    for (int off = 32; off > 0; off >>= 1) {
+        s += __shfl_xor(s, off);
+        ss += __shfl_xor(ss, off);
+    }
+    if ((tid & 63) == 0) {
+        red[0][tid >> 6] = s;
+        red[1][tid >> 6] = ss;
+    }
+    __syncthreads();
+    s = (red[0][0] + red[0][1]) + (red[0][2] + red[0][3]);
+    ss = (red[1][0] + red[1][1]) + (red[1][2] + red[1][3]);
+    const double n = (double)HW * cg;
+    const double mean = s / n;
+    double var = ss / n - mean * mean;
+    if (var < 0.0) var = 0.0;
+    const float rstd = (float)(1.0 / sqrt(var + (double)eps));
+    const float fmean = (float)mean;
+    for (int i = tid; i < cg; i += 256) {
+        const int c = c0 + i;
+        const float sc = rstd * gamma[c];
+        scale[(long)b * C + c] = sc;
+        shift[(long)b * C + c] = beta[c] - fmean * sc;
+    }
+}
+__global__ __launch_bounds__(256) void gn_rowstats_kernel(const float* __restrict__ x, float* __restrict__ stats, long total, int n4, int ldx, int ld) {
+    const long i = (long)blockIdx.x * 256 + threadIdx.x;
+    if (i >= total) return;
+    const long ck = i / n4;
+    const int c = (int)(i - ck * n4) * 4;
+    const float* src = x + ck * 16 * ldx + c;
+    f32x4 s = {0.f, 0.f, 0.f, 0.f}, q = {0.f, 0.f, 0.f, 0.f};
+#pragma unroll
+    for (int r = 0; r < 16; ++r) {
+        const f32x4 v = *reinterpret_cast<const f32x4*>(src + (long)r * ldx);
+        s += v;
+        q += v * v;
+    }
+    float* dst = stats + (ck * ld + c) * 2;
+    *reinterpret_cast<f32x4*>(dst) = f32x4{s[0], q[0], s[1], q[1]};
+    *reinterpret_cast<f32x4*>(dst + 4) = f32x4{s[2], q[2], s[3], q[3]};
 }
 
 template <typename T, bool SILU, bool PAIR = false>
diff --git a/freefine_amd/ops.py b/freefine_amd/ops.py
--- a/freefine_amd/ops.py
+++ b/freefine_amd/ops.py
@@ -169,7 +169,7 @@
     return pack_linear(out.reshape(4 * cout, 4 * cin), dtype)
 
 
-def conv3x3_up2x(x, w4, bias, B, Hin, Win, Cin, *, out=None):
+def conv3x3_up2x(x, w4, bias, B, Hin, Win, Cin, *, out=None, gn_stats=False):
     lib = L.load()
     cout = w4.shape[0] // 4
     x3 = is_x3(w4)
@@ -181,7 +181,7 @@
         for b0 in range(0, B, nb):
             b1 = min(B, b0 + nb)
             conv3x3_up2x(x[b0:b1], w4, bias, b1 - b0, Hin, Win, Cin, out=out[b0:b1])
-        return out
+        return _set_gn_stats(out, None)
     if x3:
         xa = x if pair_width(x) is not None else split_pair(x, Cin)
         assert pair_width(xa) == Cin
@@ -191,6 +191,9 @@
         xa, odt, dcode = x, x.dtype, L.FFN_BF16
     assert w4.shape[1] >= (8 if x3 else 4) * Cin
     y = torch.empty(B, Hin * Win, 4 * cout, dtype=odt, device=x.device)
+    sbuf = None
+    if gn_stats and x3 and (Hin * Win) % L.IG_STATS_ROWS == 0:
+        sbuf = torch.empty(B * Hin * Win // L.IG_STATS_ROWS, 4 * cout, 2, dtype=torch.float32, device=x.device)
     for c in range(4):
         a, b = c >> 1, c & 1
         d = L.IgemmDesc()
@@ -204,6 +207,8 @@
         d.stride, d.pad, d.upsample = 1, 2 * (1 - a) + (1 - b), 0
         d.flags, d.alpha, d.conv = 0, 1.0, 2
         d.splitk, d.ws, d.ws_bytes = 0, _workspace(x.device).data_ptr(), WS_BYTES
+        if sbuf is not None:
+            d.stats, d.ld_stats = sbuf.data_ptr() + c * cout * 8, 4 * cout
         if _PROF is None:
             L.check(lib.ffn_igemm(_stream(), dcode, CT.byref(d)), "ffn_igemm(conv 2x2)")
         else:
@@ -212,7 +217,7 @@
     if out is None:
         out = torch.empty(B, 4 * Hin * Win, cout, dtype=odt, device=x.device)
     out.view(B, Hin, 2, Win, 2, cout).copy_(y.view(B, Hin, Win, 2, 2, cout).permute(0, 1, 3, 2, 4, 5))
-    return out
+    return _set_gn_stats(out, None if sbuf is None else [(sbuf, 4 * (Hin * Win // L.IG_STATS_ROWS), cout, cout)])
 
 
 F8_ACT_SCALE = 16.0
@@ -268,6 +273,30 @@
     return getattr(x, "_ffn_pair", None)
 
 
+def gn_stats_of(x):
+    return getattr(x, "_ffn_gn_stats", None)
+
+
+def _set_gn_stats(t, st):
+    if st is not None:
+        t._ffn_gn_stats = st
+    elif hasattr(t, "_ffn_gn_stats"):
+        del t._ffn_gn_stats
+    return t
+
+
+def gn_stats_wanted(B, HW, C, G):
+    return C % G == 0 and HW % L.IG_STATS_ROWS == 0 and (B * HW + 256) * C * 4 < (1 << 31) - 4096 and not L.load().ffn_gn_fused(B, HW, C, G)
+
+
+def _stats_request(d, out, rows_per_image, N, ld=None):
+    ld = ld or N
+    nchunk = rows_per_image // L.IG_STATS_ROWS
+    buf = torch.empty(d.M // L.IG_STATS_ROWS, ld, 2, dtype=torch.float32, device=out.device)
+    d.stats, d.ld_stats = buf.data_ptr(), ld
+    return buf, nchunk
+
+
 def split_pair(x, K=None):
     lib = L.load()
     assert x.dtype == torch.float32 and x.stride(-1) == 1
@@ -292,7 +321,8 @@
     return ws
 
 def linear(x, w, bias=None, *, K=None, out=None, residual=None, rowbias=None, rows_per_batch=None, silu=False,
-           geglu=False, out_f32=False, transposed_ld=None, alpha=1.0, splitk=0, out_pair=False, gelu=False, relu=False, kv64_from=None, qgelu=False):
+           geglu=False, out_f32=False, transposed_ld=None, alpha=1.0, splitk=0, out_pair=False, gelu=False, relu=False, kv64_from=None, qgelu=False,
+           gn_stats=False):
     lib = L.load()
     K = K if K is not None else x.shape[-1]
     M = x.numel() // x.shape[-1]
@@ -355,6 +385,11 @@
         splitk = 1
     d.flags, d.alpha, d.conv = flags, alpha, 0
     d.splitk, d.ws, d.ws_bytes = splitk, _workspace(x.device).data_ptr(), WS_BYTES
+    st = None
+    if gn_stats and x3 and not (flags & ~L.IG_OUT_F32) and d.rows_per_batch % L.IG_STATS_ROWS == 0 and M % d.rows_per_batch == 0:
+        buf, nchunk = _stats_request(d, out, d.rows_per_batch, N)
+        st = [(buf, nchunk, N, N)]
+    _set_gn_stats(out, st)
     if _PROF is None:
         L.check(lib.ffn_igemm(_stream(), dcode, CT.byref(d)), "ffn_igemm")
     else:
@@ -365,7 +400,7 @@
 
 
 def conv3x3(x, w, bias, B, Hin, Win, Cin, *, stride=1, pad=1, upsample=False, out=None, residual=None, rowbias=None,
-            rowbias_ld=None, out_f32=False, Hout=None, Wout=None, splitk=0, relu=False):
+            rowbias_ld=None, out_f32=False, Hout=None, Wout=None, splitk=0, relu=False, gn_stats=False):
     lib = L.load()
     He, We = (Hin * 2, Win * 2) if upsample else (Hin, Win)
     if Hout is None:
@@ -402,6 +437,11 @@
     d.stride, d.pad, d.upsample = stride, pad, 1 if upsample else 0
     d.flags, d.alpha, d.conv = (L.IG_OUT_F32 if out_f32 else 0) | (L.IG_OUT_RELU if relu else 0), (w._ffn_f8[1] if f8 else 1.0), 1
     d.splitk, d.ws, d.ws_bytes = splitk, _workspace(x.device).data_ptr(), WS_BYTES
+    st = None
+    if gn_stats and x3 and not relu and (Hout * Wout) % L.IG_STATS_ROWS == 0:
+        buf, nchunk = _stats_request(d, out, Hout * Wout, N)
+        st = [(buf, nchunk, N, N)]
+    _set_gn_stats(out, st)
     if _PROF is None:
         L.check(lib.ffn_igemm(_stream(), dcode, CT.byref(d)), "ffn_igemm(conv)")
     else:
@@ -565,7 +605,23 @@
             torch.empty(B, C, dtype=torch.float32, device=device), torch.empty(B, C, dtype=torch.float32, device=device))
 
 
-def groupnorm(x, gamma, beta, G, eps, silu=False, out=None, ws=None, pair=False):
+def _gn_from_stats(lib, x, y, yraw, gamma, beta, G, eps, fl, st, name, nbytes):
+    B, HW, Cc = x.shape
+    (sa, nca, lda, C1), (sb, ncb, ldb, _) = st[0], (st[1] if len(st) > 1 else (None, 0, 0, 0))
+    scale, shift = (torch.empty(B, Cc, dtype=torch.float32, device=x.device) for _ in range(2))
+    call = lambda: lib.ffn_groupnorm_stats(_stream(), x.data_ptr(), y.data_ptr(), _p(yraw), gamma.data_ptr(), beta.data_ptr(), B, HW, Cc, G, eps, fl,
+                                           sa.data_ptr(), nca, lda, C1, _p(sb), ncb, ldb, scale.data_ptr(), shift.data_ptr())
+    L.check(call() if _PROF is None else _timed(name, 0.0, nbytes, call), "ffn_groupnorm_stats")
+
+
+def _usable_stats(x, use_stats):
+    st = gn_stats_of(x) if use_stats else None
+    if st is None or x.dtype != torch.float32 or not x.is_contiguous() or len(st) > 2 or sum(s[3] for s in st) != x.shape[-1]:
+        return None
+    return st
+
+
+def groupnorm(x, gamma, beta, G, eps, silu=False, out=None, ws=None, pair=False, use_stats=True):
     lib = L.load()
     B, HW, Cc = x.shape
     if pair:
@@ -573,6 +629,11 @@
         out = _mark_pair(torch.empty(B, HW, 2 * Cc, dtype=torch.bfloat16, device=x.device), Cc)
     if out is None:
         out = torch.empty_like(x)
+    st = _usable_stats(x, use_stats)
+    if st is not None and not lib.ffn_gn_fused(B, HW, Cc, G):
+        _gn_from_stats(lib, x, out, None, gamma, beta, G, eps, (L.NORM_SILU if silu else 0) | (L.NORM_OUT_PAIR if pair else 0), st,
+                       f"gn_finalize_stats+gn_apply<{_tname(x)}>", 2.0 * x.numel() * x.element_size())
+        return out
     if lib.ffn_gn_fused(B, HW, Cc, G):
         partial = scale = shift = None
     else:
@@ -600,14 +661,19 @@
     return out
 
 
-def groupnorm_pair_raw(x, gamma, beta, G, eps, silu=False, ws=None):
+def groupnorm_pair_raw(x, gamma, beta, G, eps, silu=False, ws=None, use_stats=True):
     lib = L.load()
     B, HW, Cc = x.shape
     if not _GN_RAW or Cc % 8 != 0 or lib.ffn_gn_fused(B, HW, Cc, G) or not x.is_contiguous():
-        return groupnorm(x, gamma, beta, G, eps, silu=silu, pair=True, ws=ws), split_pair(x, Cc)
+        return groupnorm(x, gamma, beta, G, eps, silu=silu, pair=True, ws=ws, use_stats=use_stats), split_pair(x, Cc)
     assert x.dtype == torch.float32
     y = _mark_pair(torch.empty(B, HW, 2 * Cc, dtype=torch.bfloat16, device=x.device), Cc)
     yr = _mark_pair(torch.empty(B, HW, 2 * Cc, dtype=torch.bfloat16, device=x.device), Cc)
+    st = _usable_stats(x, use_stats)
+    if st is not None:
+        _gn_from_stats(lib, x, y, yr, gamma, beta, G, eps, (L.NORM_SILU if silu else 0) | L.NORM_OUT_PAIR, st,
+                       "gn_finalize_stats+gn_apply<float> (+ raw pair)", 3.0 * x.numel() * x.element_size())
+        return y, yr
     partial, scale, shift = ws if ws is not None else gn_workspace(B, HW, Cc, x.device)
     call = lambda: lib.ffn_groupnorm_pair_raw(_stream(), x.data_ptr(), y.data_ptr(), yr.data_ptr(), gamma.data_ptr(), beta.data_ptr(), B, HW, Cc, G, eps,
                                               L.NORM_SILU if silu else 0, _p(partial), _p(scale), _p(shift))
@@ -718,17 +784,19 @@
     C1, C2 = a.shape[-1], b.shape[-1]
     rows = a.numel() // C1
     base = getattr(a, "_ffn_cat_base", None)
+    sa, sb = gn_stats_of(a), gn_stats_of(b)
+    cat_st = sa + sb if sa is not None and sb is not None and len(sa) == 1 and len(sb) == 1 else None
     if out is None and base is not None and base.shape[-1] == C1 + C2:
         L.check(_timed(f"concat_kernel<{_tname(b)}>", 0.0, 2.0 * rows * C2 * b.element_size(),
                        lambda: lib.ffn_concat(_stream(), _dt(b), None, b.data_ptr(), base.data_ptr(), rows, C1, C2)), "ffn_concat")
-        return base
+        return _set_gn_stats(base, cat_st)
     if base is not None:
         a = a.contiguous()
     if out is None:
         out = torch.empty(*a.shape[:-1], C1 + C2, dtype=a.dtype, device=a.device)
     L.check(_timed(f"concat_kernel<{_tname(a)}>", 0.0, 2.0 * rows * (C1 + C2) * a.element_size(),
                    lambda: lib.ffn_concat(_stream(), _dt(a), a.data_ptr(), b.data_ptr(), out.data_ptr(), rows, C1, C2)), "ffn_concat")
-    return out
+    return _set_gn_stats(out, cat_st)
 
 
 def cat_dst(shape_lead, C1, C2, dtype, device):
diff --git a/freefine_amd/unet.py b/freefine_amd/unet.py
--- a/freefine_amd/unet.py
+++ b/freefine_amd/unet.py
@@ -499,6 +499,9 @@
         B, HW, C = x.shape
         return ops.groupnorm(x, gb[0], gb[1], self.cfg.norm_num_groups, eps, silu=silu, pair=self.x3)
 
+    def _st(self, B, HW, C):
+        return self.x3 and ops.gn_stats_wanted(B, HW, C, self.cfg.norm_num_groups)
+
     def _gn_conv_in(self, x, gb, w):
         if ops.is_f8(w):
             return ops.groupnorm_f8(x, gb[0], gb[1], self.cfg.norm_num_groups, self.cfg.norm_eps, w._ffn_f8[0], silu=True)
@@ -511,11 +514,12 @@
         else:
             h = self._gn_conv_in(x, r.n1, r.c1[0])
         rb = temb_all[:, r.temb_off:r.temb_off + r.cout]
-        h = ops.conv3x3(h, r.c1[0], r.c1[1], B, H, W, cin, rowbias=rb, rowbias_ld=temb_all.shape[1])
+        st = self._st(B, H * W, r.cout)
+        h = ops.conv3x3(h, r.c1[0], r.c1[1], B, H, W, cin, rowbias=rb, rowbias_ld=temb_all.shape[1], gn_stats=st)
         h = self._gn_conv_in(h, r.n2, r.c2[0])
         if r.sc is not None:
             x = ops.linear(x, r.sc[0], r.sc[1], K=cin)
-        return ops.conv3x3(h, r.c2[0], r.c2[1], B, H, W, r.cout, residual=x, out=out)
+        return ops.conv3x3(h, r.c2[0], r.c2[1], B, H, W, r.cout, residual=x, out=out, gn_stats=st)
 
     def _without_ref_queries(self, plan, B):
         keep = self._reuse["idx_a_list"]
@@ -607,7 +611,7 @@
         y = ops.layernorm(h, *t.ln[2], pair=self.x3)
         y = ops.linear(y, t.ff1[0], t.ff1[1], K=C, geglu=True, out_pair=self.x3)
         h = ops.linear(y, t.ff2[0], t.ff2[1], K=4 * C, residual=h, out_pair=self.x3 and C % 32 == 0)
-        return ops.linear(h, t.proj_out[0], t.proj_out[1], K=C, residual=res0, out=out)
+        return ops.linear(h, t.proj_out[0], t.proj_out[1], K=C, residual=res0, out=out, rows_per_batch=S, gn_stats=self._st(B, S, C))
 
     def _run(self, sample, text_kv):
         cfg = self.cfg
@@ -639,7 +643,7 @@
         temb_full = temb_all
         temb_all = temb_all[:B]
         x = ops.pack_nchw(sample, list(range(B)), self.cin_pad, dt)
-        x = ops.conv3x3(x, self.conv_in[0], self.conv_in[1], B, H, W, self.cin_pad)
+        x = ops.conv3x3(x, self.conv_in[0], self.conv_in[1], B, H, W, self.cin_pad, gn_stats=self._st(B, H * W, self.conv_in[0].shape[0]))
         skips = [(x, H, W)]
         n = len(self.down)
         for i, blk in enumerate(self.down):
@@ -651,7 +655,7 @@
                 skips.append((x, H, W))
             if blk.down is not None:
                 C = x.shape[-1]
-                x = ops.conv3x3(x, blk.down[0], blk.down[1], B, H, W, C, stride=2)
+                x = ops.conv3x3(x, blk.down[0], blk.down[1], B, H, W, C, stride=2, gn_stats=self._st(B, ((H + 1) // 2) * ((W + 1) // 2), C))
                 H, W = (H + 1) // 2, (W + 1) // 2
                 skips.append((x, H, W))
         x = self._resblock(self.mid.res[0], x, B, H, W, temb_all)
@@ -689,9 +693,9 @@
             if blk.up is not None:
                 C = x.shape[-1]
                 if blk.up2 is not None and ops.up2x_eligible(C, C, B * H * W):
-                    x = ops.conv3x3_up2x(x, blk.up2, blk.up[1], B, H, W, C, out=cat_dst(C, 4 * H * W))
+                    x = ops.conv3x3_up2x(x, blk.up2, blk.up[1], B, H, W, C, out=cat_dst(C, 4 * H * W), gn_stats=self._st(B, 4 * H * W, C))
                 else:
-                    x = ops.conv3x3(x, blk.up[0], blk.up[1], B, H, W, C, upsample=True, out=cat_dst(C, 4 * H * W))
+                    x = ops.conv3x3(x, blk.up[0], blk.up[1], B, H, W, C, upsample=True, out=cat_dst(C, 4 * H * W), gn_stats=self._st(B, 4 * H * W, C))
                 H, W = 2 * H, 2 * W
         C = x.shape[-1]
         if self.conv_out_n4 is not None:
diff --git a/freefine_amd/vae.py b/freefine_amd/vae.py
--- a/freefine_amd/vae.py
+++ b/freefine_amd/vae.py
@@ -100,14 +100,18 @@
     def _gn(self, x, gb, silu):
         return ops.groupnorm(x, gb[0], gb[1], self.G, 1e-6, silu=silu, pair=self.x3)
 
+    def _st(self, B, HW, C):
+        return self.x3 and ops.gn_stats_wanted(B, HW, C, self.G)
+
     def _resblock(self, r, x, B, H, W):
         cin = x.shape[-1]
+        st = self._st(B, H * W, r.cout)
         h = self._gn(x, r.n1, True)
-        h = ops.conv3x3(h, r.c1[0], r.c1[1], B, H, W, cin)
+        h = ops.conv3x3(h, r.c1[0], r.c1[1], B, H, W, cin, gn_stats=st)
         h = self._gn(h, r.n2, True)
         if r.sc is not None:
             x = ops.linear(x, r.sc[0], r.sc[1], K=cin)
-        return ops.conv3x3(h, r.c2[0], r.c2[1], B, H, W, r.cout, residual=x)
+        return ops.conv3x3(h, r.c2[0], r.c2[1], B, H, W, r.cout, residual=x, gn_stats=st)
 
     def _attention(self, a, x, B, S):
         C = x.shape[-1]
@@ -121,7 +125,7 @@
             scores = ops.linear(q[b], k[b], None, K=C)
             p = ops.softmax_rows(scores, C ** -0.5)
             ops.linear(p, vt[b], None, K=S, out=o[b])
-        return ops.linear(o, a.o[0], a.o[1], K=C, residual=x)
+        return ops.linear(o, a.o[0], a.o[1], K=C, residual=x, rows_per_batch=S, gn_stats=self._st(B, S, C))
 
     def _midblock(self, m, x, B, H, W):
         x = self._resblock(m.r0, x, B, H, W)
@@ -165,9 +169,9 @@
             if blk.up is not None:
                 C = x.shape[-1]
                 if blk.up2 is not None and ops.up2x_eligible(C, C, B * H * W):
-                    x = ops.conv3x3_up2x(x, blk.up2, blk.up[1], B, H, W, C)
+                    x = ops.conv3x3_up2x(x, blk.up2, blk.up[1], B, H, W, C, gn_stats=self._st(B, 4 * H * W, C))
                 else:
-                    x = ops.conv3x3(x, blk.up[0], blk.up[1], B, H, W, C, upsample=True)
+                    x = ops.conv3x3(x, blk.up[0], blk.up[1], B, H, W, C, upsample=True, gn_stats=self._st(B, 4 * H * W, C))
                 H, W = 2 * H, 2 * W
         C = x.shape[-1]
         x = self._gn(x, self.dec_norm, True)
diff --git a/include/freefine_hip.h b/include/freefine_hip.h
--- a/include/freefine_hip.h
+++ b/include/freefine_hip.h
@@ -46,7 +46,10 @@
     int x3;
     int f8;
     int kv64_from;
+    float* stats;
+    int ld_stats;
 } ffn_igemm_desc;
+enum { FFN_IG_STATS_ROWS = 16 };
 int ffn_igemm(void* stream, int dtype, const ffn_igemm_desc* d);
 int ffn_split_pair(void* stream, const float* src, void* dst, long rows, int C, int ld_src);
 int ffn_conv3x3_n4(void* stream, int dtype, const void* x, const float* w, const float* bias, float* out, int B, int H, int W, int Cin);
@@ -121,6 +124,10 @@
                   float eps, int silu, float* partial_ws, float* scale, float* shift);
 int ffn_groupnorm_pair_raw(void* stream, const void* x, void* y_pair, void* yraw_pair, const float* gamma, const float* beta, int B, int HW, int C, int G,
                            float eps, int silu, float* partial_ws, float* scale, float* shift);
+int ffn_groupnorm_stats(void* stream, const void* x, void* y, void* yraw, const float* gamma, const float* beta, int B, int HW, int C, int G, float eps,
+                        int flags, const float* stats_a, int nchunk_a, int ld_a, int C1, const float* stats_b, int nchunk_b, int ld_b, float* scale,
+                        float* shift);
+int ffn_gn_rowstats(void* stream, const float* x, float* stats, int M, int N, int ldx, int ld_stats);
 int ffn_layernorm(void* stream, int dtype, const void* x, void* y, const float* gamma, const float* beta, int M, int C,
                   float eps);
 int ffn_layernorm_pair(void* stream, const float* x, void* y, const float* gamma, const float* beta, int M, int C, float eps);
```

Measured after the change: 1.936. 2.5% lower.
